# autonomousvision/LaRa

Measured on AMD Instinct MI355X. Metric: novel-view frames/sec @512x512 (4-view in, 2DGS fwd+bwd), higher is better.
Workload: dtype f32 raster + bf16-MFMA/f32-accumulate encoder (+ bf16-autocast coarse decoder MLP, as the reference's bf16-mixed)

## Files before the change

### include/lara2dgs.h

```cpp
#ifndef LARA2DGS_H
#define LARA2DGS_H

#include <stddef.h>
#include <stdint.h>

#ifdef __cplusplus
extern "C" {
#endif

#define LARA2DGS_ABI_VERSION 10

#define LARA2DGS_OK 0
#define LARA2DGS_E_INVALID (-1)
#define LARA2DGS_E_LAUNCH (-2)
#define LARA2DGS_E_UNSUPPORTED (-3)

typedef struct lara2dgs_view {
    int32_t P;
    int32_t sh_degree;
    int32_t sh_coeffs;
    int32_t image_height;
    int32_t image_width;
    float tanfovx;
    float tanfovy;
    float scale_modifier;
    int32_t prefiltered;
    int32_t debug;
    int32_t forward_only;
    int64_t capacity;
    const float *bg;
    const float *viewmatrix;
    const float *projmatrix;
    const float *campos;
    uint32_t *counts_out;
} lara2dgs_view;

typedef struct lara2dgs_state_layout {
    int64_t header;
    int64_t geom;
    int64_t cullbox;
    int64_t point_list;
    int64_t ranges;
    int64_t tile_order;
    int64_t pair_base;
    int64_t pair_pos;
    int64_t final_T;
    int64_t n_contrib;
    int64_t seg_base;
    int64_t seg_cnt;
    int64_t bwd_order;
    int64_t bwd_items;
    int64_t ckpt;
    int64_t pair_mask;
    int64_t tile_maxc;
    int64_t seg_cost;
    int64_t total;
} lara2dgs_state_layout;

int lara2dgs_abi_version(void);
const char *lara2dgs_error_string(int code);
int lara2dgs_last_hip_error(void);

int64_t lara2dgs_state_bytes(int32_t P, int32_t H, int32_t W, int64_t capacity, int32_t forward_only);
int64_t lara2dgs_scratch_bytes(int32_t P, int32_t H, int32_t W, int64_t capacity, int32_t forward_only);
int lara2dgs_get_state_layout(int32_t P, int32_t H, int32_t W, int64_t capacity, int32_t forward_only,
                              lara2dgs_state_layout *out);

int lara2dgs_forward(const lara2dgs_view *view, const float *means3D, const float *shs,
                     const float *colors_precomp, const float *opacities, const float *scales,
                     const float *rotations, const float *transmat_precomp, float *out_color,
                     float *out_allmap, int32_t *out_radii, void *state, void *scratch,
                     void *stream);

int lara2dgs_backward(const lara2dgs_view *view, const float *means3D, const float *shs,
                      const float *colors_precomp, const float *scales, const float *rotations,
                      const float *transmat_precomp, const int32_t *radii, const float *dL_dcolor,
                      const float *dL_dallmap, void *state, void *scratch,
                      float *dL_dmeans3D, float *dL_dmeans2D, float *dL_dshs, float *dL_dcolors,
                      float *dL_dopacities, float *dL_dscales, float *dL_drotations,
                      float *dL_dtransmat, void *stream);


int lara2dgs_forward_views(int32_t n_views, const lara2dgs_view *views, const float *means3D,
                           const float *shs, const float *colors_precomp, const float *opacities,
                           const float *scales, const float *rotations, const float *transmat_precomp,
                           float *out_color, float *out_allmap, int32_t *out_radii, void *state,
                           int64_t state_stride, void *scratch, int64_t scratch_stride, void *stream);

typedef struct lara2dgs_subset {
    const void *coarse_state;
    int64_t coarse_state_stride;
    int64_t coarse_capacity;
    int32_t coarse_P;
    int32_t coarse_forward_only;
    const int32_t *inv;
} lara2dgs_subset;
int lara2dgs_forward_views_subset(int32_t n_views, const lara2dgs_view *views, const float *means3D,
                                  const float *shs, const float *colors_precomp, const float *opacities,
                                  const float *scales, const float *rotations, const float *transmat_precomp,
                                  float *out_color, float *out_allmap, int32_t *out_radii, void *state,
                                  int64_t state_stride, void *scratch, int64_t scratch_stride,
                                  const lara2dgs_subset *subset, void *stream);

typedef struct lara2dgs_grad_layout {
    int64_t means3D, means2D, shs, colors, opacities, scales, rotations, transmat, total;
} lara2dgs_grad_layout;
int lara2dgs_get_grad_layout(int32_t P, int32_t sh_coeffs, int32_t has_shs, int32_t has_colors,
                             int32_t has_scale_rot, int32_t has_transmat, lara2dgs_grad_layout *out);

int lara2dgs_backward_views(int32_t n_views, const lara2dgs_view *views, const float *means3D,
                            const float *shs, const float *colors_precomp, const float *scales,
                            const float *rotations, const float *transmat_precomp, const int32_t *radii,
                            const float *dL_dcolor, const float *dL_dallmap, void *state,
                            int64_t state_stride, void *scratch, int64_t scratch_stride,
                            float *grad_out, void *stream);

int lara2dgs_mark_visible(int32_t P, const float *means3D, const float *viewmatrix,
                          const float *projmatrix, uint8_t *present, void *stream);

int lara2dgs_profile_enable(int on);
int lara2dgs_selftest(int which, const float *in, float *out, void *stream);
int lara2dgs_profile_collect(char *names, int names_len, float *ms, int max_entries);

#ifdef __cplusplus
}
#endif
#endif
```

### lara_amd/csrc/abi.hip

```cpp
#include <stdlib.h>
#include <string.h>

#include "common.h"

static thread_local int g_last_hip_error = 0;
void l2d_set_hip_error(hipError_t e) { g_last_hip_error = (int)e; }

#include <atomic>
#include <mutex>
#include <map>
#include <utility>
#include <vector>
namespace {
struct ProfRec { const char *name; hipEvent_t a, b; };
std::atomic<bool> g_prof_on{false};
std::mutex g_prof_mu;
std::vector<ProfRec> g_prof_log;
std::vector<hipEvent_t> g_prof_pool;
hipEvent_t prof_event() {
    if (!g_prof_pool.empty()) { hipEvent_t e = g_prof_pool.back(); g_prof_pool.pop_back(); return e; }
    hipEvent_t e = nullptr;
    (void)hipEventCreate(&e);
    return e;
}
}

L2dProfScope::L2dProfScope(const char *name, hipStream_t stream) : slot(-1), s(stream) {
    if (!g_prof_on.load(std::memory_order_relaxed)) return;
    std::lock_guard<std::mutex> lk(g_prof_mu);
    ProfRec r{name, prof_event(), prof_event()};
    (void)hipEventRecord(r.a, s);
    g_prof_log.push_back(r);
    slot = (int)g_prof_log.size() - 1;
}
L2dProfScope::~L2dProfScope() {
    if (slot < 0) return;
    std::lock_guard<std::mutex> lk(g_prof_mu);
    if (slot < (int)g_prof_log.size()) (void)hipEventRecord(g_prof_log[slot].b, s);
}

namespace {

bool make_view(const lara2dgs_view *view, ViewDev &v) {
    if (!view) return false;
    if (view->P < 0 || view->image_height <= 0 || view->image_width <= 0) return false;
    if (view->sh_degree < 0 || view->sh_degree > 3) return false;
    if (view->capacity < 0 || view->capacity > 0xffffffffll) return false;
    if (!view->bg || !view->viewmatrix || !view->projmatrix || !view->campos) return false;
    v.P = view->P;
    v.deg = view->sh_degree;
    v.M = view->sh_coeffs;
    v.H = view->image_height;
    v.W = view->image_width;
    v.gx = (v.W + TILE - 1) / TILE;
    v.gy = (v.H + TILE - 1) / TILE;
    v.tiles = v.gx * v.gy;
    if (v.gx > 65535 || v.gy > 65535) return false;
    v.scale_modifier = view->scale_modifier;
    v.cull_transparent = (view->prefiltered >> 1) & 1;
    v.cap = (unsigned)view->capacity;
    v.fwd_only = view->forward_only != 0;
    v.counts_out = view->counts_out;
    {
        static const unsigned dbg = getenv("LARA2DGS_DEBUG_FLAGS") ? (unsigned)strtoul(getenv("LARA2DGS_DEBUG_FLAGS"), nullptr, 0) : 0u;
        v.dbg = dbg;
    }
    v.bg = view->bg;
    v.viewmatrix = view->viewmatrix;
    v.projmatrix = view->projmatrix;
    v.campos = view->campos;
    return true;
}

StateView carve_state(const ViewDev &v, void *state) {
    lara2dgs_state_layout L;
    state_layout(v.P, v.H, v.W, v.cap, v.fwd_only, &L);
    char *b = (char *)state;
    StateView s;
    s.header = (uint32_t *)(b + L.header);
    s.geom = (float4 *)(b + L.geom);
    s.cullbox = (float4 *)(b + L.cullbox);
    s.point_list = (uint32_t *)(b + L.point_list);
    s.ranges = (uint2 *)(b + L.ranges);
    s.tile_order = (uint32_t *)(b + L.tile_order);
    s.pair_base = (uint32_t *)(b + L.pair_base);
    s.pair_pos = (uint32_t *)(b + L.pair_pos);
    s.final_T = (float *)(b + L.final_T);
    s.n_contrib = (uint32_t *)(b + L.n_contrib);
    s.seg_base = (uint32_t *)(b + L.seg_base);
    s.seg_cnt = (uint32_t *)(b + L.seg_cnt);
    s.bwd_order = (uint32_t *)(b + L.bwd_order);
    s.bwd_items = (uint2 *)(b + L.bwd_items);
    s.ckpt = (float *)(b + L.ckpt);
    s.pair_mask = (uint2 *)(b + L.pair_mask);
    s.tile_maxc = (uint32_t *)(b + L.tile_maxc);
    s.seg_cost = (uint32_t *)(b + L.seg_cost);
    return s;
}

ScratchView carve_scratch(const ViewDev &v, void *scratch, ScratchLayout &L) {
    scratch_layout(v.P, v.H, v.W, v.cap, v.fwd_only, &L);
    char *b = (char *)scratch;
    ScratchView s;
    s.tile_count = (uint32_t *)(b + L.tile_count);
    s.tile_fill = (uint32_t *)(b + L.tile_fill);
    s.sub_start = (uint32_t *)(b + L.sub_start);
    s.sort_parts = (uint32_t *)(b + L.sort_parts);
    s.sort_items = (uint2 *)(b + L.sort_items);
    s.rect = (uint4 *)(b + L.rect);
    s.keys = (uint64_t *)(b + L.keys);
    s.block_tot = (uint32_t *)(b + L.block_tot);
    s.pair_grad = (float4 *)(b + L.pair_grad);
    s.pair_valid = (uint32_t *)(b + L.pair_valid);
    return s;
}

}

extern "C" {

int lara2dgs_abi_version(void) { return LARA2DGS_ABI_VERSION; }

const char *lara2dgs_error_string(int code) {
    switch (code) {
    case LARA2DGS_OK: return "ok";
    case LARA2DGS_E_INVALID: return "invalid argument";
    case LARA2DGS_E_LAUNCH: return "HIP launch/API failure (see lara2dgs_last_hip_error)";
    case LARA2DGS_E_UNSUPPORTED: return "unsupported configuration";
    default: return "unknown error";
    }
}

int lara2dgs_last_hip_error(void) { return g_last_hip_error; }

int64_t lara2dgs_state_bytes(int32_t P, int32_t H, int32_t W, int64_t capacity, int32_t forward_only) {
    if (P < 0 || H <= 0 || W <= 0 || capacity < 0) return LARA2DGS_E_INVALID;
    lara2dgs_state_layout L;
    state_layout(P, H, W, capacity, forward_only != 0, &L);
    return L.total;
}

int64_t lara2dgs_scratch_bytes(int32_t P, int32_t H, int32_t W, int64_t capacity, int32_t forward_only) {
    if (P < 0 || H <= 0 || W <= 0 || capacity < 0) return LARA2DGS_E_INVALID;
    ScratchLayout L;
    scratch_layout(P, H, W, capacity, forward_only != 0, &L);
    return L.total;
}

int lara2dgs_get_state_layout(int32_t P, int32_t H, int32_t W, int64_t capacity, int32_t forward_only,
                              lara2dgs_state_layout *out) {
    if (!out || P < 0 || H <= 0 || W <= 0 || capacity < 0) return LARA2DGS_E_INVALID;
    state_layout(P, H, W, capacity, forward_only != 0, out);
    return LARA2DGS_OK;
}

int lara2dgs_mark_visible(int32_t P, const float *means3D, const float *viewmatrix,
                          const float *projmatrix, uint8_t *present, void *stream) {
    (void)projmatrix;
    if (P < 0 || (P > 0 && (!means3D || !viewmatrix || !present))) return LARA2DGS_E_INVALID;
    return launch_mark_visible(P, means3D, viewmatrix, present, (hipStream_t)stream);
}

int lara2dgs_selftest(int which, const float *in, float *out, void *stream) {
    if (which != 0 || !in || !out) return LARA2DGS_E_INVALID;
    return launch_selftest_butterfly(in, out, (hipStream_t)stream);
}

int lara2dgs_profile_enable(int on) {
    g_prof_on.store(on != 0);
    return LARA2DGS_OK;
}

int lara2dgs_profile_collect(char *names, int names_len, float *ms, int max_entries) {
    std::lock_guard<std::mutex> lk(g_prof_mu);
    int n = 0, pos = 0;
    for (size_t i = 0; i < g_prof_log.size(); i++) {
        ProfRec &r = g_prof_log[i];
        if (n < max_entries && names && ms) {
            const int len = (int)strlen(r.name) + 1;
            if (pos + len <= names_len) {
                float t = 0.f;
                (void)hipEventSynchronize(r.b);
                (void)hipEventElapsedTime(&t, r.a, r.b);
                memcpy(names + pos, r.name, len);
                pos += len;
                ms[n++] = t;
            }
        }
        g_prof_pool.push_back(r.a);
        g_prof_pool.push_back(r.b);
    }
    g_prof_log.clear();
    return n;
}

}

namespace {

bool views_agree(int n, const lara2dgs_view *views) {
    for (int i = 1; i < n; i++) {
        const lara2dgs_view &a = views[0], &b = views[i];
        if (a.P != b.P || a.sh_degree != b.sh_degree || a.sh_coeffs != b.sh_coeffs || a.image_height != b.image_height ||
            a.image_width != b.image_width || a.capacity != b.capacity || a.prefiltered != b.prefiltered ||
            a.scale_modifier != b.scale_modifier || a.debug != b.debug || a.forward_only != b.forward_only) return false;
        if (b.counts_out != (a.counts_out ? a.counts_out + 4 * i : nullptr)) return false;
    }
    return true;
}

void grad_layout(int64_t P, int M, bool sh, bool col, bool sr, bool tm, lara2dgs_grad_layout *L) {
    int64_t o = 0;
    auto sec = [&](bool on, int64_t n) { if (!on) return (int64_t)-1; const int64_t at = o; o = (o + n + 3) / 4 * 4; return at; };
    L->means3D = sec(true, P * 3);
    L->means2D = sec(true, P * 3);
    L->shs = sec(sh, P * M * 3);
    L->colors = sec(col, P * 3);
    L->opacities = sec(true, P);
    L->scales = sec(sr, P * 2);
    L->rotations = sec(sr, P * 4);
    L->transmat = sec(tm, P * 9);
    L->total = o;
}

__global__ void __launch_bounds__(256) zero_strided_kernel(char *__restrict__ base, const int64_t stride, const int64_t bytes) {
    uint4 *p = (uint4 *)(base + (int64_t)blockIdx.y * stride);
    const int64_t n = bytes / 16;
    for (int64_t i = (int64_t)blockIdx.x * 256 + threadIdx.x; i < n; i += (int64_t)gridDim.x * 256) p[i] = make_uint4(0u, 0u, 0u, 0u);
}

inline void zero_strided(void *base, int64_t stride, int64_t bytes, int n_views, hipStream_t s) {
    const int64_t n = (bytes + 15) / 16;
    const unsigned gx = (unsigned)(n < 256 * 64 ? (n + 255) / 256 : 64);
    hipLaunchKernelGGL(zero_strided_kernel, dim3(gx ? gx : 1, (unsigned)n_views), dim3(256), 0, s, (char *)base, stride, (bytes + 15) / 16 * 16);
}

bool strides_ok(const lara2dgs_view &v0, int64_t state_stride, int64_t scratch_stride) {
    return state_stride % 256 == 0 && scratch_stride % 256 == 0 &&
           state_stride >= lara2dgs_state_bytes(v0.P, v0.image_height, v0.image_width, v0.capacity, v0.forward_only) &&
           scratch_stride >= lara2dgs_scratch_bytes(v0.P, v0.image_height, v0.image_width, v0.capacity, v0.forward_only);
}

void one_view_strides(const lara2dgs_view &v, int64_t &state_stride, int64_t &scratch_stride) {
    state_stride = align_up(lara2dgs_state_bytes(v.P, v.image_height, v.image_width, v.capacity, v.forward_only), 256);
    scratch_stride = align_up(lara2dgs_scratch_bytes(v.P, v.image_height, v.image_width, v.capacity, v.forward_only), 256);
}
}

extern "C" {

int lara2dgs_get_grad_layout(int32_t P, int32_t sh_coeffs, int32_t has_shs, int32_t has_colors,
                             int32_t has_scale_rot, int32_t has_transmat, lara2dgs_grad_layout *out) {
    if (!out || P < 0 || sh_coeffs < 0) return LARA2DGS_E_INVALID;
    grad_layout(P, sh_coeffs, has_shs != 0, has_colors != 0, has_scale_rot != 0, has_transmat != 0, out);
    return LARA2DGS_OK;
}

static int forward_views_impl(int32_t n_views, const lara2dgs_view *views, const float *means3D,
                           const float *shs, const float *colors_precomp, const float *opacities,
                           const float *scales, const float *rotations, const float *transmat_precomp,
                           float *out_color, float *out_allmap, int32_t *out_radii, void *state,
                           int64_t state_stride, void *scratch, int64_t scratch_stride, void *stream,
                           const lara2dgs_subset *subset) {
    if (n_views <= 0 || !views || !state || !scratch) return LARA2DGS_E_INVALID;
    if (subset) {
        if (!subset->coarse_state || !subset->inv || subset->coarse_P < views[0].P || subset->coarse_capacity < 0 ||
            subset->coarse_capacity > 0xffffffffll || subset->coarse_state_stride % 256) return LARA2DGS_E_INVALID;
        if (!views[0].forward_only && subset->coarse_forward_only) return LARA2DGS_E_INVALID;
        if (subset->coarse_state_stride < lara2dgs_state_bytes(subset->coarse_P, views[0].image_height, views[0].image_width,
                                                                subset->coarse_capacity, subset->coarse_forward_only)) return LARA2DGS_E_INVALID;
    }
    if (!views_agree(n_views, views)) return LARA2DGS_E_INVALID;
    const lara2dgs_view &v0 = views[0];
    if (!strides_ok(v0, state_stride, scratch_stride)) return LARA2DGS_E_INVALID;
    hipStream_t caller = (hipStream_t)stream;
    const int64_t HW = (int64_t)v0.image_height * v0.image_width;
    if (!out_color || !out_allmap) return LARA2DGS_E_INVALID;
    if (v0.P > 0) {
        if (!means3D || !opacities || !out_radii) return LARA2DGS_E_INVALID;
        if ((shs == nullptr) == (colors_precomp == nullptr)) return LARA2DGS_E_INVALID;
        if ((scales && rotations) == (transmat_precomp != nullptr)) return LARA2DGS_E_INVALID;
    }
    std::vector<ViewDev> vd(n_views);
    std::vector<StateView> st(n_views);
    std::vector<ScratchView> sc(n_views);
    std::vector<int32_t *> rad(n_views);
    for (int i = 0; i < n_views; i++) {
        if (!make_view(&views[i], vd[i])) return LARA2DGS_E_INVALID;
        if (v0.P > 0 && shs && vd[i].M < (vd[i].deg + 1) * (vd[i].deg + 1)) return LARA2DGS_E_INVALID;
        st[i] = carve_state(vd[i], (char *)state + i * state_stride);
        ScratchLayout SL;
        sc[i] = carve_scratch(vd[i], (char *)scratch + i * scratch_stride, SL);
        rad[i] = out_radii + (int64_t)i * v0.P;
        if (i == 0)
            zero_strided(sc[0].tile_count, scratch_stride, SL.sub_start - SL.tile_count, n_views, caller);
    }
    int rc = LARA2DGS_OK;
    for (int i0 = 0; i0 < n_views && rc == LARA2DGS_OK; i0 += L2D_MAX_VIEWS) {
        ViewBatch vb{};
        vb.n = n_views - i0 < L2D_MAX_VIEWS ? n_views - i0 : L2D_MAX_VIEWS;
        vb.state_stride = state_stride; vb.scratch_stride = scratch_stride;
        for (int k = 0; k < vb.n; k++) vb.bg[k] = vd[i0 + k].bg;
        rc = launch_preprocess_fwd_views(vd[i0], vb.n, &vd[i0], n_views > 1, means3D, shs, colors_precomp, opacities, scales,
                                         rotations, transmat_precomp, &st[i0], &sc[i0], &rad[i0], caller);
        if (rc == LARA2DGS_OK && !subset) rc = launch_binning(vd[i0], st[i0], sc[i0], caller, vb);
        if (rc == LARA2DGS_OK && subset) {
            ViewDev cv = vd[i0];
            cv.P = subset->coarse_P; cv.cap = (unsigned)subset->coarse_capacity; cv.fwd_only = subset->coarse_forward_only != 0;
            const StateView cst = carve_state(cv, (char *)const_cast<void *>(subset->coarse_state) + (int64_t)i0 * subset->coarse_state_stride);
            rc = launch_binning_subset(vd[i0], st[i0], sc[i0], caller, vb, cst, subset->coarse_state_stride, subset->inv);
        }
        if (rc == LARA2DGS_OK)
            rc = launch_composite_fwd(vd[i0], st[i0], sc[i0], out_color + (int64_t)i0 * 3 * HW, out_allmap + (int64_t)i0 * 7 * HW,
                                      caller, vb);
    }
    return rc;
}

int lara2dgs_forward_views(int32_t n_views, const lara2dgs_view *views, const float *means3D,
                           const float *shs, const float *colors_precomp, const float *opacities,
                           const float *scales, const float *rotations, const float *transmat_precomp,
                           float *out_color, float *out_allmap, int32_t *out_radii, void *state,
                           int64_t state_stride, void *scratch, int64_t scratch_stride, void *stream) {
    return forward_views_impl(n_views, views, means3D, shs, colors_precomp, opacities, scales, rotations, transmat_precomp, out_color,
                              out_allmap, out_radii, state, state_stride, scratch, scratch_stride, stream, nullptr);
}

int lara2dgs_forward_views_subset(int32_t n_views, const lara2dgs_view *views, const float *means3D,
                                  const float *shs, const float *colors_precomp, const float *opacities,
                                  const float *scales, const float *rotations, const float *transmat_precomp,
                                  float *out_color, float *out_allmap, int32_t *out_radii, void *state,
                                  int64_t state_stride, void *scratch, int64_t scratch_stride,
                                  const lara2dgs_subset *subset, void *stream) {
    if (!subset) return LARA2DGS_E_INVALID;
    return forward_views_impl(n_views, views, means3D, shs, colors_precomp, opacities, scales, rotations, transmat_precomp, out_color,
                              out_allmap, out_radii, state, state_stride, scratch, scratch_stride, stream, subset);
}

static int backward_views_impl(int32_t n_views, const lara2dgs_view *views, const float *means3D, const float *shs,
                               const float *colors_precomp, const float *scales, const float *rotations,
                               const float *transmat_precomp, const int32_t *radii, const float *dL_dcolor,
                               const float *dL_dallmap, void *state, int64_t state_stride, void *scratch,
                               int64_t scratch_stride, float *dL_dmeans3D, float *dL_dmeans2D, float *dL_dshs,
                               float *dL_dcolors, float *dL_dopacities, float *dL_dscales, float *dL_drotations,
                               float *dL_dtransmat, void *stream) {
    const lara2dgs_view &v0 = views[0];
    hipStream_t caller = (hipStream_t)stream;
    const int64_t HW = (int64_t)v0.image_height * v0.image_width;
    std::vector<ViewDev> vd(n_views);
    std::vector<StateView> st(n_views);
    std::vector<ScratchView> sc(n_views);
    std::vector<const int32_t *> rad(n_views);
    std::vector<ScratchLayout> SL(n_views);
    for (int i = 0; i < n_views; i++) {
        if (!make_view(&views[i], vd[i])) return LARA2DGS_E_INVALID;
        st[i] = carve_state(vd[i], (char *)state + i * state_stride);
        sc[i] = carve_scratch(vd[i], (char *)scratch + i * scratch_stride, SL[i]);
        rad[i] = radii + (int64_t)i * v0.P;
    }
    int rc = LARA2DGS_OK;
    for (int i0 = 0; i0 < n_views && rc == LARA2DGS_OK; i0 += L2D_MAX_VIEWS) {
        ViewBatch vb{};
        vb.n = n_views - i0 < L2D_MAX_VIEWS ? n_views - i0 : L2D_MAX_VIEWS;
        vb.state_stride = state_stride; vb.scratch_stride = scratch_stride;
        for (int k = 0; k < vb.n; k++) vb.bg[k] = vd[i0 + k].bg;
        rc = launch_bwd_order(vd[i0], st[i0], sc[i0], caller, vb, sc[i0].pair_valid, SL[i0].total - SL[i0].pair_valid);
        if (rc == LARA2DGS_OK)
            rc = launch_composite_bwd(vd[i0], st[i0], sc[i0], dL_dcolor + (int64_t)i0 * 3 * HW, dL_dallmap ? dL_dallmap + (int64_t)i0 * 7 * HW : nullptr, caller, vb);
        if (rc == LARA2DGS_OK)
            rc = launch_preprocess_bwd_views(vd[i0], vb.n, &vd[i0], n_views > 1, i0 > 0, means3D, shs, colors_precomp, scales,
                                             rotations, transmat_precomp, &rad[i0], &st[i0], &sc[i0], dL_dmeans3D, dL_dmeans2D,
                                             dL_dshs, dL_dcolors, dL_dopacities, dL_dscales, dL_drotations, dL_dtransmat, caller);
    }
    return rc;
}

int lara2dgs_backward_views(int32_t n_views, const lara2dgs_view *views, const float *means3D,
                            const float *shs, const float *colors_precomp, const float *scales,
                            const float *rotations, const float *transmat_precomp, const int32_t *radii,
                            const float *dL_dcolor, const float *dL_dallmap, void *state,
                            int64_t state_stride, void *scratch, int64_t scratch_stride,
                            float *grad_out, void *stream) {
    if (n_views <= 0 || !views || !state || !scratch || !grad_out) return LARA2DGS_E_INVALID;
    if (!views_agree(n_views, views)) return LARA2DGS_E_INVALID;
    const lara2dgs_view &v0 = views[0];
    if (v0.forward_only) return LARA2DGS_E_INVALID;
    if (!strides_ok(v0, state_stride, scratch_stride)) return LARA2DGS_E_INVALID;
    if (!dL_dcolor) return LARA2DGS_E_INVALID;
    const bool has_sh = shs != nullptr, has_col = colors_precomp != nullptr, has_sr = scales && rotations,
               has_tm = transmat_precomp != nullptr;
    lara2dgs_grad_layout G;
    grad_layout(v0.P, v0.sh_coeffs, has_sh, has_col, has_sr, has_tm, &G);
    if (v0.P == 0 || G.total == 0) return LARA2DGS_OK;
    if (!means3D || !radii) return LARA2DGS_E_INVALID;
    if (has_sh == has_col || has_sr == has_tm) return LARA2DGS_E_INVALID;
    auto at = [&](int64_t off) { return off < 0 ? (float *)nullptr : grad_out + off; };
    return backward_views_impl(n_views, views, means3D, shs, colors_precomp, scales, rotations, transmat_precomp, radii,
                               dL_dcolor, dL_dallmap, state, state_stride, scratch, scratch_stride, at(G.means3D),
                               at(G.means2D), at(G.shs), at(G.colors), at(G.opacities), at(G.scales), at(G.rotations),
                               at(G.transmat), stream);
}

int lara2dgs_forward(const lara2dgs_view *view, const float *means3D, const float *shs,
                     const float *colors_precomp, const float *opacities, const float *scales,
                     const float *rotations, const float *transmat_precomp, float *out_color,
                     float *out_allmap, int32_t *out_radii, void *state, void *scratch,
                     void *stream) {
    ViewDev v;
    if (!make_view(view, v)) return LARA2DGS_E_INVALID;
    if (!out_color || !out_allmap || !state || !scratch) return LARA2DGS_E_INVALID;
    if (v.P > 0) {
        if (!means3D || !opacities || !out_radii) return LARA2DGS_E_INVALID;
        if ((shs == nullptr) == (colors_precomp == nullptr)) return LARA2DGS_E_INVALID;
        const bool has_sr = scales && rotations;
        if (has_sr == (transmat_precomp != nullptr)) return LARA2DGS_E_INVALID;
        if (shs && v.M < (v.deg + 1) * (v.deg + 1)) return LARA2DGS_E_INVALID;
    }
    int64_t sst, qst;
    one_view_strides(*view, sst, qst);
    return forward_views_impl(1, view, means3D, shs, colors_precomp, opacities, scales, rotations, transmat_precomp, out_color,
                              out_allmap, out_radii, state, sst, scratch, qst, stream, nullptr);
}

int lara2dgs_backward(const lara2dgs_view *view, const float *means3D, const float *shs,
                      const float *colors_precomp, const float *scales, const float *rotations,
                      const float *transmat_precomp, const int32_t *radii, const float *dL_dcolor,
                      const float *dL_dallmap, void *state, void *scratch,
                      float *dL_dmeans3D, float *dL_dmeans2D, float *dL_dshs, float *dL_dcolors,
                      float *dL_dopacities, float *dL_dscales, float *dL_drotations,
                      float *dL_dtransmat, void *stream) {
    ViewDev v;
    if (!make_view(view, v)) return LARA2DGS_E_INVALID;
    if (!dL_dcolor || !state || !scratch) return LARA2DGS_E_INVALID;
    if (v.fwd_only) return LARA2DGS_E_INVALID;
    if (v.P == 0) return LARA2DGS_OK;
    if (!means3D || !radii || !dL_dmeans3D || !dL_dmeans2D || !dL_dopacities) return LARA2DGS_E_INVALID;
    if ((shs == nullptr) == (colors_precomp == nullptr)) return LARA2DGS_E_INVALID;
    if (shs && !dL_dshs) return LARA2DGS_E_INVALID;
    if (colors_precomp && !dL_dcolors) return LARA2DGS_E_INVALID;
    const bool has_sr = scales && rotations;
    if (has_sr == (transmat_precomp != nullptr)) return LARA2DGS_E_INVALID;
    if (has_sr && (!dL_dscales || !dL_drotations)) return LARA2DGS_E_INVALID;
    if (transmat_precomp && !dL_dtransmat) return LARA2DGS_E_INVALID;
    int64_t sst, qst;
    one_view_strides(*view, sst, qst);
    return backward_views_impl(1, view, means3D, shs, colors_precomp, scales, rotations, transmat_precomp, radii, dL_dcolor,
                               dL_dallmap, state, sst, scratch, qst, dL_dmeans3D, dL_dmeans2D, dL_dshs, dL_dcolors,
                               dL_dopacities, dL_dscales, dL_drotations, dL_dtransmat, stream);
}

}
```

### lara_amd/csrc/binning.hip

```cpp
#include "common.h"

namespace {

template <typename Ptr>
__device__ __forceinline__ void bitonic_sort(Ptr a, const uint32_t n, const uint32_t m ) {
    for (uint32_t k = 2; k <= m; k <<= 1) {
        for (uint32_t j = k >> 1; j > 0; j >>= 1) {
            const bool flip = (j == (k >> 1));
            for (uint32_t t = threadIdx.x; t < (m >> 1); t += blockDim.x) {
                const uint32_t i = ((t & ~(j - 1)) << 1) | (t & (j - 1));
                const uint32_t p = flip ? (i ^ (k - 1)) : (i ^ j);
                if (p < n) {
                    const uint64_t x = a[i], y = a[p];
                    if (y < x) { a[i] = y; a[p] = x; }
                }
            }
            __syncthreads();
        }
    }
}

constexpr int L2D_SORT_PARTS = 2;
__device__ __forceinline__ uint32_t l2d_sort_parts(const uint32_t len) {
    return len <= 4096u || len > 8192u ? 1u : 2u;
}

__global__ void __launch_bounds__(1024)
tile_scan_kernel(ViewDev v, const uint32_t *__restrict__ tile_count, uint32_t *__restrict__ sub_start,
                 uint2 *__restrict__ ranges, uint32_t *__restrict__ header,
                 uint32_t *__restrict__ tile_order, uint32_t *__restrict__ block_tot,
                 uint32_t *__restrict__ seg_base, uint32_t *__restrict__ seg_cnt,
                 uint32_t *__restrict__ bwd_order, uint2 *__restrict__ bwd_items,
                 uint32_t *__restrict__ sort_parts, uint2 *__restrict__ sort_items, const long long sst, const long long qst) {
    tile_count = l2d_view_ptr(tile_count, qst); sub_start = l2d_view_ptr(sub_start, qst); block_tot = l2d_view_ptr(block_tot, qst);
    sort_parts = l2d_view_ptr(sort_parts, qst); sort_items = l2d_view_ptr(sort_items, qst);
    ranges = l2d_view_ptr(ranges, sst); header = l2d_view_ptr(header, sst); tile_order = l2d_view_ptr(tile_order, sst);
    seg_base = l2d_view_ptr(seg_base, sst); seg_cnt = l2d_view_ptr(seg_cnt, sst); bwd_order = l2d_view_ptr(bwd_order, sst);
    bwd_items = l2d_view_ptr(bwd_items, sst);
    __shared__ uint32_t wave_sums[16];
    __shared__ uint32_t carry_s, s_max;
    __shared__ uint32_t bcnt[64];
    const int tid = threadIdx.x, lane = tid & 63, wid = tid >> 6;
    if (blockIdx.x == 1) {
        if (tid == 0) carry_s = 0;
        __syncthreads();
        const int nblk = (v.P + 255) / 256;
        for (int base = 0; base < nblk; base += 1024) {
            const int i = base + tid;
            const uint32_t c = i < nblk ? block_tot[i] : 0u;
            uint32_t x = c;
#pragma unroll
            for (int d = 1; d < 64; d <<= 1) {
                const uint32_t y = __shfl_up(x, d, 64);
                if (lane >= d) x += y;
            }
            if (lane == 63) wave_sums[wid] = x;
            __syncthreads();
            uint32_t wave_off = 0;
            for (int w = 0; w < wid; w++) wave_off += wave_sums[w];
            const uint32_t incl = carry_s + wave_off + x;
            if (i < nblk) block_tot[i] = incl - c;
            __syncthreads();
            if (tid == 1023) carry_s = incl;
            __syncthreads();
        }
        return;
    }
    if (tid == 0) carry_s = 0;
    if (tid >= 4 && tid < 64) header[tid] = 0u;
    __syncthreads();
    uint32_t max_len = 0;
    for (int base = 0; base < v.tiles; base += 1024) {
        const int i = base + tid;
        uint32_t sub[L2D_SLICES];
        uint32_t c = 0;
        if (i < v.tiles) {
            const uint4 *tc = (const uint4 *)(tile_count + (size_t)i * L2D_SLICES);
#pragma unroll
            for (int q = 0; q < L2D_SLICES / 4; q++) {
                const uint4 w4 = tc[q];
                sub[4 * q] = w4.x; sub[4 * q + 1] = w4.y; sub[4 * q + 2] = w4.z; sub[4 * q + 3] = w4.w;
            }
#pragma unroll
            for (int q = 0; q < L2D_SLICES; q++) c += sub[q];
        }
        max_len = c > max_len ? c : max_len;
        uint32_t x = c;
#pragma unroll
        for (int d = 1; d < 64; d <<= 1) {
            const uint32_t y = __shfl_up(x, d, 64);
            if (lane >= d) x += y;
        }
        if (lane == 63) wave_sums[wid] = x;
        __syncthreads();
        uint32_t wave_off = 0;
        for (int w = 0; w < wid; w++) wave_off += wave_sums[w];
        const uint32_t carry = carry_s;
        const uint32_t incl = carry + wave_off + x;
        if (i < v.tiles) {
            ranges[i] = c ? make_uint2(incl - c, incl) : make_uint2(0u, 0u);
            uint32_t run = incl - c;
            uint4 *ss = (uint4 *)(sub_start + (size_t)i * L2D_SLICES);
#pragma unroll
            for (int q = 0; q < L2D_SLICES / 4; q++) {
                uint4 w4;
                w4.x = run; run += sub[4 * q];
                w4.y = run; run += sub[4 * q + 1];
                w4.z = run; run += sub[4 * q + 2];
                w4.w = run; run += sub[4 * q + 3];
                ss[q] = w4;
            }
        }
        __syncthreads();
        if (tid == 1023) carry_s = incl;
        __syncthreads();
    }
#pragma unroll
    for (int d = 32; d > 0; d >>= 1) {
        const uint32_t y = __shfl_xor(max_len, d, 64);
        max_len = y > max_len ? y : max_len;
    }
    __syncthreads();
    if (lane == 0) wave_sums[wid] = max_len;
    __syncthreads();
    if (tid == 0) {
        uint32_t m = 0;
        for (int w = 0; w < 16; w++) m = wave_sums[w] > m ? wave_sums[w] : m;
        const uint32_t total = carry_s;
        header[0] = total;
        header[1] = total > v.cap ? 1u : 0u;
        header[2] = m;
        s_max = m;
        if (v.counts_out) {
            uint32_t *c = v.counts_out + 4 * blockIdx.z;
            __hip_atomic_store(&c[0], total, __ATOMIC_RELAXED, __HIP_MEMORY_SCOPE_SYSTEM);
            __hip_atomic_store(&c[1], total > v.cap ? 1u : 0u, __ATOMIC_RELAXED, __HIP_MEMORY_SCOPE_SYSTEM);
            __hip_atomic_store(&c[2], m, __ATOMIC_RELAXED, __HIP_MEMORY_SCOPE_SYSTEM);
            __hip_atomic_store(&c[3], 1u, __ATOMIC_RELEASE, __HIP_MEMORY_SCOPE_SYSTEM);
        }
    }
    if (tid < 64) bcnt[tid] = 0;
    __syncthreads();
    const uint32_t denom = s_max + 1u;
    for (int i = tid; i < v.tiles; i += 1024) {
        const uint2 rg = ranges[i];
        const uint32_t b = 63u - (uint32_t)(((uint64_t)(rg.y - rg.x) * 64u) / denom);
        atomicAdd(&bcnt[b], 1u);
    }
    __syncthreads();
    if (tid < 64) {
        const uint32_t c = bcnt[tid];
        uint32_t x = c;
#pragma unroll
        for (int d = 1; d < 64; d <<= 1) {
            const uint32_t y = __shfl_up(x, d, 64);
            if (lane >= d) x += y;
        }
        bcnt[tid] = x - c;
    }
    __syncthreads();
    for (int i = tid; i < v.tiles; i += 1024) {
        const uint2 rg = ranges[i];
        const uint32_t b = 63u - (uint32_t)(((uint64_t)(rg.y - rg.x) * 64u) / denom);
        tile_order[atomicAdd(&bcnt[b], 1u)] = (uint32_t)i;
    }
    __syncthreads();
    if (!v.fwd_only) {
    if (tid == 0) carry_s = 0;
    if (tid < 64) bcnt[tid] = 0;
    __syncthreads();
    const bool overflow = header[1] != 0u;
    for (int base = 0; base < v.tiles; base += 1024) {
        const int i = base + tid;
        uint32_t len = 0;
        if (i < v.tiles) { const uint2 rg = ranges[i]; len = rg.y - rg.x; }
        const uint32_t nb = len ? (len - 1u) / L2D_SEG : 0u;
        uint32_t x = nb;
#pragma unroll
        for (int d = 1; d < 64; d <<= 1) {
            const uint32_t y = __shfl_up(x, d, 64);
            if (lane >= d) x += y;
        }
        if (lane == 63) wave_sums[wid] = x;
        __syncthreads();
        uint32_t wave_off = 0;
        for (int w = 0; w < wid; w++) wave_off += wave_sums[w];
        const uint32_t incl = carry_s + wave_off + x;
        if (i < v.tiles) {
            seg_base[i] = incl - nb;
            seg_cnt[i] = nb;
            if (!overflow)
                for (uint32_t q = 0; q < nb; q++) bwd_items[incl - nb + q] = make_uint2((uint32_t)i, q);
            const uint32_t pl = len - nb * L2D_SEG;
            atomicAdd(&bcnt[63u - (uint32_t)(((uint64_t)min(pl, (uint32_t)L2D_SEG) * 64u) / (L2D_SEG + 1u))], 1u);
        }
        __syncthreads();
        if (tid == 1023) carry_s = incl;
        __syncthreads();
    }
    if (tid == 0) { seg_base[v.tiles] = carry_s; header[3] = carry_s; }
    if (tid < 64) {
        const uint32_t c = bcnt[tid];
        uint32_t x = c;
#pragma unroll
        for (int d = 1; d < 64; d <<= 1) {
            const uint32_t y = __shfl_up(x, d, 64);
            if (lane >= d) x += y;
        }
        bcnt[tid] = x - c;
    }
    __syncthreads();
    for (int i = tid; i < v.tiles; i += 1024) {
        const uint2 rg = ranges[i];
        const uint32_t len = rg.y - rg.x;
        const uint32_t pl = len - seg_cnt[i] * L2D_SEG;
        bwd_order[atomicAdd(&bcnt[63u - (uint32_t)(((uint64_t)min(pl, (uint32_t)L2D_SEG) * 64u) / (L2D_SEG + 1u))], 1u)] = (uint32_t)i;
    }
    }
    __syncthreads();
    if (tid == 0) carry_s = 0;
    __syncthreads();
    for (int base = 0; base < v.tiles; base += 1024) {
        const int i = base + tid;
        uint32_t len = 0;
        if (i < v.tiles) { const uint2 rg = ranges[i]; len = rg.y - rg.x; }
        const uint32_t want = l2d_sort_parts(len) - 1u;
        uint32_t x = want;
#pragma unroll
        for (int d = 1; d < 64; d <<= 1) {
            const uint32_t y = __shfl_up(x, d, 64);
            if (lane >= d) x += y;
        }
        if (lane == 63) wave_sums[wid] = x;
        __syncthreads();
        uint32_t wave_off = 0;
        for (int w = 0; w < wid; w++) wave_off += wave_sums[w];
        const uint32_t incl = carry_s + wave_off + x, first = incl - want;
        if (i < v.tiles) {
            const uint32_t room = first < (uint32_t)v.tiles ? (uint32_t)v.tiles - first : 0u;
            const uint32_t got = want < room ? want : room;
            sort_parts[i] = 1u + got;
            for (uint32_t q = 0; q < got; q++) sort_items[first + q] = make_uint2((uint32_t)i, q + 1u);
        }
        __syncthreads();
        if (tid == 1023) carry_s = incl;
        __syncthreads();
    }
    if (tid == 0) sort_parts[v.tiles] = carry_s < (uint32_t)v.tiles ? carry_s : (uint32_t)v.tiles;
}

__global__ void __launch_bounds__(256)
scatter_kernel(ViewDev v, const uint4 *__restrict__ rect, const uint32_t *__restrict__ sub_start,
               const uint32_t *__restrict__ block_base, uint32_t *__restrict__ pair_base,
               uint32_t *__restrict__ tile_fill, uint64_t *__restrict__ keys, const int use_lds, const long long sst,
               const long long qst) {
    rect = l2d_view_ptr(rect, qst); sub_start = l2d_view_ptr(sub_start, qst); block_base = l2d_view_ptr(block_base, qst);
    tile_fill = l2d_view_ptr(tile_fill, qst); keys = l2d_view_ptr(keys, qst); pair_base = l2d_view_ptr(pair_base, sst);
    extern __shared__ __attribute__((aligned(16))) uint32_t hist[];
    const int idx = blockIdx.x * blockDim.x + threadIdx.x;
    const int slice = blockIdx.x % L2D_SLICES;
    int rx0 = 0, ry0 = 0, rx1 = 0, ry1 = 0;
    uint64_t word = 0;
    if (idx < v.P) {
        const uint4 r = rect[idx];
        rx0 = r.x & 0xffff; ry0 = r.x >> 16; rx1 = r.y & 0xffff; ry1 = r.y >> 16;
        word = ((uint64_t)r.z << 32) | (uint32_t)idx;
        if (!v.fwd_only) {
            const uint32_t pb = block_base[blockIdx.x] + r.w;
            pair_base[idx] = pb;
            if (idx == v.P - 1) pair_base[v.P] = pb + (uint32_t)(rx1 - rx0) * (uint32_t)(ry1 - ry0);
        }
    }
    if (use_lds) {
        for (int t = threadIdx.x; t < v.tiles; t += blockDim.x) hist[t] = 0;
        __syncthreads();
        for (int y = ry0; y < ry1; y++)
            for (int x = rx0; x < rx1; x++) atomicAdd(&hist[y * v.gx + x], 1u);
        __syncthreads();
        for (int t = threadIdx.x; t < v.tiles; t += blockDim.x) {
            const uint32_t c = hist[t];
            if (c) hist[t] = sub_start[t * L2D_SLICES + slice] +
                             __hip_atomic_fetch_add(&tile_fill[t * L2D_SLICES + slice], c, __ATOMIC_RELAXED,
                                                    __HIP_MEMORY_SCOPE_AGENT);
        }
        __syncthreads();
        for (int y = ry0; y < ry1; y++)
            for (int x = rx0; x < rx1; x++) {
                const uint32_t slot = atomicAdd(&hist[y * v.gx + x], 1u);
                if (slot < v.cap) keys[slot] = word;
            }
    } else {
        for (int y = ry0; y < ry1; y++)
            for (int x = rx0; x < rx1; x++) {
                const int t = (y * v.gx + x) * L2D_SLICES + slice;
                const uint32_t slot = sub_start[t] + __hip_atomic_fetch_add(&tile_fill[t], 1u, __ATOMIC_RELAXED,
                                                                          __HIP_MEMORY_SCOPE_AGENT);
                if (slot < v.cap) keys[slot] = word;
            }
    }
}

__device__ __forceinline__ uint32_t next_pow2(uint32_t n) {
    return n <= 1 ? 1u : 1u << (32 - __clz(n - 1));
}

__device__ __forceinline__ void ce(uint64_t &a, uint64_t &b) {
    const bool sw = b < a;
    const uint64_t lo = sw ? b : a, hi = sw ? a : b;
    a = lo; b = hi;
}
__device__ __forceinline__ uint64_t shfl64(uint64_t x, int src_lane) {
    const uint32_t lo = __shfl((uint32_t)x, src_lane, 64), hi = __shfl((uint32_t)(x >> 32), src_lane, 64);
    return ((uint64_t)hi << 32) | lo;
}

template <int E, int NT, bool REVERSED>
__device__ __forceinline__ void xchg(uint64_t (&x)[E], const int t, const int pt, uint64_t *lds) {
    uint64_t o[E];
    if ((t ^ pt) < 64) {
#pragma unroll
        for (int e = 0; e < E; e++) o[e] = shfl64(x[REVERSED ? E - 1 - e : e], pt & 63);
    } else {
#pragma unroll
        for (int e = 0; e < E; e++) lds[e * NT + t] = x[e];
        __syncthreads();
#pragma unroll
        for (int e = 0; e < E; e++) o[e] = lds[(REVERSED ? E - 1 - e : e) * NT + pt];
        __syncthreads();
    }
    const bool keep_min = t < pt;
#pragma unroll
    for (int e = 0; e < E; e++) {
        const bool take = keep_min ? (o[e] < x[e]) : (x[e] < o[e]);
        x[e] = take ? o[e] : x[e];
    }
}

template <int E, int NT>
__device__ __forceinline__ void block_sort(uint64_t (&x)[E], uint64_t *lds) {
    const int t = threadIdx.x;
#pragma unroll
    for (int k = 2; k <= E; k <<= 1) {
#pragma unroll
        for (int e = 0; e < E; e++) {
            const int p = e ^ (k - 1);
            if (p > e) ce(x[e], x[p]);
        }
#pragma unroll
        for (int j = k >> 2; j >= 1; j >>= 1)
#pragma unroll
            for (int e = 0; e < E; e++)
                if ((e & j) == 0) ce(x[e], x[e | j]);
    }
#pragma unroll 1
    for (int kt = 2; kt <= NT; kt <<= 1) {
        xchg<E, NT, true>(x, t, t ^ (kt - 1), lds);
#pragma unroll 1
        for (int jt = kt >> 2; jt >= 1; jt >>= 1) xchg<E, NT, false>(x, t, t ^ jt, lds);
#pragma unroll
        for (int j = E >> 1; j >= 1; j >>= 1)
#pragma unroll
            for (int e = 0; e < E; e++)
                if ((e & j) == 0) ce(x[e], x[e | j]);
    }
}

struct PairMap {
    const uint4 *rect;
    const uint32_t *pair_base;
    uint32_t *pair_pos;
    int tx, ty;
    uint32_t first;
    __device__ __forceinline__ void put(const uint32_t id, const uint32_t i) const {
        if (!pair_pos) return;
        const uint4 r = rect[id];
        const int rx0 = r.x & 0xffff, ry0 = r.x >> 16, rx1 = r.y & 0xffff;
        pair_pos[first + i] = pair_base[id] + (uint32_t)((ty - ry0) * (rx1 - rx0) + (tx - rx0));
    }
};

template <int E, int NT>
__device__ __forceinline__ void sort_tile(const uint64_t *__restrict__ seg, const uint32_t n,
                                          uint32_t *__restrict__ out, uint64_t *lds, const PairMap &pm) {
    uint64_t x[E];
    const uint32_t i0 = threadIdx.x * E;
#pragma unroll
    for (int e = 0; e < E; e++) x[e] = (i0 + e < n) ? seg[i0 + e] : ~0ull;
    block_sort<E, NT>(x, lds);
#pragma unroll
    for (int e = 0; e < E; e++)
        if (i0 + e < n) {
            out[i0 + e] = (uint32_t)x[e];
            pm.put((uint32_t)x[e], i0 + e);
        }
}

constexpr uint32_t L2D_SORT_LDS_KEYS = 4096;

constexpr int L2D_SORT_BUCKETS = 1024, L2D_SORT_BUCKET_MAX = 48;

template <int E>
__device__ __forceinline__ void sort_keys(const uint64_t *src, const uint32_t m, uint32_t *__restrict__ out,
                                          const uint32_t off, uint64_t *lds, uint32_t *bkt, uint32_t *sh, const PairMap &pm) {
    const int t = threadIdx.x, lane = t & 63;
    uint64_t x[E];
#pragma unroll
    for (int e = 0; e < E; e++) x[e] = (t + e * 512 < (int)m) ? src[t + e * 512] : ~0ull;
    if (t == 0) { sh[0] = ~0u; sh[1] = 0u; sh[2] = 0u; }
    const uint32_t B = m <= 256u ? 64u : (m <= 1024u ? 256u : (uint32_t)L2D_SORT_BUCKETS);
    for (uint32_t b = t; b < B; b += 512) bkt[b] = 0u;
    __syncthreads();
    uint32_t lo = ~0u, hi = 0u;
#pragma unroll
    for (int e = 0; e < E; e++)
        if (t + e * 512 < (int)m) {
            const uint32_t d = (uint32_t)(x[e] >> 32);
            lo = d < lo ? d : lo;
            hi = d > hi ? d : hi;
        }
#pragma unroll
    for (int k = 32; k > 0; k >>= 1) {
        const uint32_t a = __shfl_xor(lo, k, 64), b = __shfl_xor(hi, k, 64);
        lo = a < lo ? a : lo;
        hi = b > hi ? b : hi;
    }
    if (lane == 0) { atomicMin(&sh[0], lo); atomicMax(&sh[1], hi); }
    __syncthreads();
    const uint32_t dmin = sh[0];
    const uint64_t scale = ((uint64_t)B << 32) / ((uint64_t)(sh[1] - dmin) + 1ull);
    uint32_t bk[E], slot[E];
#pragma unroll
    for (int e = 0; e < E; e++) {
        bk[e] = 0u; slot[e] = 0u;
        if (t + e * 512 < (int)m) {
            const uint64_t q = (uint64_t)((uint32_t)(x[e] >> 32) - dmin) * scale;
            bk[e] = (uint32_t)(q >> 32);
            bk[e] = bk[e] < B ? bk[e] : B - 1u;
            slot[e] = atomicAdd(&bkt[bk[e]], 1u);
        }
    }
    __syncthreads();
    {
        const uint32_t c0 = 2 * t < (int)B ? bkt[2 * t] : 0u, c1 = 2 * t + 1 < (int)B ? bkt[2 * t + 1] : 0u;
        uint32_t incl = c0 + c1, big = c0 > c1 ? c0 : c1;
#pragma unroll
        for (int d = 1; d < 64; d <<= 1) {
            const uint32_t y = __shfl_up(incl, d, 64);
            if (lane >= d) incl += y;
        }
#pragma unroll
        for (int k = 32; k > 0; k >>= 1) { const uint32_t y = __shfl_xor(big, k, 64); big = y > big ? y : big; }
        if (lane == 63) sh[4 + (t >> 6)] = incl;
        if (lane == 0) atomicMax(&sh[2], big);
        __syncthreads();
        uint32_t wave_off = 0;
        for (int w = 0; w < (t >> 6); w++) wave_off += sh[4 + w];
        __syncthreads();
        if (2 * t < (int)B) bkt[2 * t] = wave_off + incl - c0 - c1;
        if (2 * t + 1 < (int)B) bkt[2 * t + 1] = wave_off + incl - c1;
        if (t == 511) bkt[B] = wave_off + incl;
    }
    __syncthreads();
    if (sh[2] > (uint32_t)L2D_SORT_BUCKET_MAX) {
        __syncthreads();
        block_sort<E, 512>(x, lds);
#pragma unroll
        for (int e = 0; e < E; e++)
            if ((uint32_t)(t * E + e) < m) {
                out[off + t * E + e] = (uint32_t)x[e];
                pm.put((uint32_t)x[e], off + t * E + e);
            }
        return;
    }
#pragma unroll
    for (int e = 0; e < E; e++)
        if (t + e * 512 < (int)m) lds[bkt[bk[e]] + slot[e]] = x[e];
    __syncthreads();
    for (uint32_t b = t; b < B; b += 512) {
        const uint32_t s0 = bkt[b], s1 = bkt[b + 1];
        for (uint32_t i = s0 + 1; i < s1; i++) {
            const uint64_t key = lds[i];
            uint32_t j = i;
            while (j > s0 && lds[j - 1] > key) { lds[j] = lds[j - 1]; j--; }
            lds[j] = key;
        }
    }
    __syncthreads();
    for (uint32_t i = t; i < m; i += 512) {
        const uint32_t id = (uint32_t)lds[i];
        out[off + i] = id;
        pm.put(id, off + i);
    }
}

template <int DUMMY = 0>
__device__ __forceinline__ void sort_dispatch(const uint64_t *src, const uint32_t m, uint32_t *__restrict__ out,
                                              const uint32_t off, uint64_t *lds, uint32_t *bkt, uint32_t *sh, const PairMap &pm) {
    if (m <= 512u) sort_keys<1>(src, m, out, off, lds, bkt, sh, pm);
    else if (m <= 1024u) sort_keys<2>(src, m, out, off, lds, bkt, sh, pm);
    else if (m <= 2048u) sort_keys<4>(src, m, out, off, lds, bkt, sh, pm);
    else sort_keys<8>(src, m, out, off, lds, bkt, sh, pm);
}

__global__ void __launch_bounds__(512)
tile_sort_kernel(ViewDev v, const uint2 *__restrict__ ranges, const uint32_t *__restrict__ header,
                 const uint32_t *__restrict__ tile_order, uint64_t *__restrict__ keys,
                 uint32_t *__restrict__ point_list, const uint4 *__restrict__ rect,
                 const uint32_t *__restrict__ pair_base, uint32_t *__restrict__ pair_pos,
                 uint32_t *__restrict__ sort_parts, const uint2 *__restrict__ sort_items, const long long sst, const long long qst) {
    ranges = l2d_view_ptr(ranges, sst); header = l2d_view_ptr(header, sst); tile_order = l2d_view_ptr(tile_order, sst);
    point_list = l2d_view_ptr(point_list, sst); pair_base = l2d_view_ptr(pair_base, sst); pair_pos = l2d_view_ptr(pair_pos, sst);
    keys = l2d_view_ptr(keys, qst); rect = l2d_view_ptr(rect, qst); sort_parts = l2d_view_ptr(sort_parts, qst);
    sort_items = l2d_view_ptr(sort_items, qst);
    __shared__ uint64_t lds[L2D_SORT_LDS_KEYS];
    __shared__ uint32_t bkt[L2D_SORT_BUCKETS + 1], sh[16];
    __shared__ uint32_t s_min, s_max, s_mine, s_ticket, s_hist[L2D_SORT_PARTS];
    int part = 0, tile;
    if ((int)blockIdx.x < v.tiles) {
        if (blockIdx.x >= sort_parts[v.tiles]) return;
        const uint2 it = sort_items[blockIdx.x];
        tile = (int)it.x; part = (int)it.y;
    } else {
        tile = (int)tile_order[(int)blockIdx.x - v.tiles];
    }
    const uint2 rg = ranges[tile];
    const uint32_t n = rg.y - rg.x;
    if (header[1]) return;
    if (n == 0) return;
    const int S = (int)(sort_parts[tile] & 0xffffu);
    uint64_t *seg = keys + rg.x;
    uint32_t *out = point_list + rg.x;
    const PairMap pm{rect, pair_base, v.fwd_only ? nullptr : pair_pos, tile % v.gx, tile / v.gx, rg.x};
    bool whole_list_in_place = S == 1 && n > L2D_SORT_LDS_KEYS;
    if (S == 1 && !whole_list_in_place) {
        sort_dispatch(seg, n, out, 0u, lds, bkt, sh, pm);
        return;
    }
    if (S > 1) {
        if (threadIdx.x == 0) { s_min = ~0u; s_max = 0u; s_mine = 0u; }
        if (threadIdx.x < L2D_SORT_PARTS) s_hist[threadIdx.x] = 0u;
        __syncthreads();
        uint32_t lo = ~0u, hi = 0u;
        for (uint32_t i = threadIdx.x; i < n; i += 512) {
            const uint32_t d = (uint32_t)(seg[i] >> 32);
            lo = d < lo ? d : lo;
            hi = d > hi ? d : hi;
        }
#pragma unroll
        for (int k = 32; k > 0; k >>= 1) {
            const uint32_t a = __shfl_xor(lo, k, 64), b = __shfl_xor(hi, k, 64);
            lo = a < lo ? a : lo;
            hi = b > hi ? b : hi;
        }
        if ((threadIdx.x & 63) == 0) { atomicMin(&s_min, lo); atomicMax(&s_max, hi); }
        __syncthreads();
        const uint32_t dmin = s_min;
        const uint64_t width = (uint64_t)(s_max - dmin) + 1ull;
        uint32_t cnt[L2D_SORT_PARTS];
#pragma unroll
        for (int b = 0; b < L2D_SORT_PARTS; b++) cnt[b] = 0u;
        for (uint32_t i = threadIdx.x; i < n; i += 512) {
            const int bin = (int)(((uint64_t)((uint32_t)(seg[i] >> 32) - dmin) * (uint64_t)S) / width);
#pragma unroll
            for (int b = 0; b < L2D_SORT_PARTS; b++) cnt[b] += bin == b ? 1u : 0u;
        }
#pragma unroll
        for (int b = 0; b < L2D_SORT_PARTS; b++) {
#pragma unroll
            for (int k = 32; k > 0; k >>= 1) cnt[b] += __shfl_xor(cnt[b], k, 64);
            if ((threadIdx.x & 63) == 0 && cnt[b]) atomicAdd(&s_hist[b], cnt[b]);
        }
        __syncthreads();
        uint32_t off = 0, biggest = 0;
        for (int b = 0; b < S; b++) {
            off += b < part ? s_hist[b] : 0u;
            biggest = s_hist[b] > biggest ? s_hist[b] : biggest;
        }
        if (biggest > L2D_SORT_LDS_KEYS) {
            if (threadIdx.x == 0) {
                __threadfence();
                s_ticket = __hip_atomic_fetch_add(&sort_parts[tile], 0x10000u, __ATOMIC_ACQ_REL, __HIP_MEMORY_SCOPE_AGENT) >> 16;
            }
            __syncthreads();
            if (s_ticket != (uint32_t)S - 1u) return;
            whole_list_in_place = true;
        } else {
            const uint32_t m = s_hist[part];
            if (m == 0) return;
            for (uint32_t i0 = 0; i0 < n; i0 += 512) {
                const uint32_t i = i0 + threadIdx.x;
                const uint64_t key = i < n ? seg[i] : 0ull;
                const int bin = i < n ? (int)(((uint64_t)((uint32_t)(key >> 32) - dmin) * (uint64_t)S) / width) : -1;
                const unsigned long long mine = __ballot(bin == part);
                uint32_t base = 0;
                if ((threadIdx.x & 63) == 0 && mine) base = atomicAdd(&s_mine, (uint32_t)__builtin_popcountll(mine));
                base = (uint32_t)__builtin_amdgcn_readfirstlane((int)base);
                if (bin == part) lds[base + (uint32_t)__builtin_popcountll(mine & ((1ull << (threadIdx.x & 63)) - 1ull))] = key;
            }
            __syncthreads();
            sort_dispatch(lds, m, out, off, lds, bkt, sh, pm);
            return;
        }
    }
    bitonic_sort(seg, n, next_pow2(n));
    for (uint32_t i = threadIdx.x; i < n; i += blockDim.x) {
        out[i] = (uint32_t)seg[i];
        pm.put((uint32_t)seg[i], i);
    }
}

__global__ void __launch_bounds__(256)
pair_base_kernel(ViewDev v, const uint4 *__restrict__ rect, const uint32_t *__restrict__ block_base, uint32_t *__restrict__ pair_base,
                 const long long sst, const long long qst) {
    rect = l2d_view_ptr(rect, qst); block_base = l2d_view_ptr(block_base, qst); pair_base = l2d_view_ptr(pair_base, sst);
    const int idx = blockIdx.x * 256 + threadIdx.x;
    if (idx >= v.P) return;
    const uint4 r = rect[idx];
    const uint32_t pb = block_base[blockIdx.x] + r.w;
    pair_base[idx] = pb;
    if (idx == v.P - 1) {
        const int rx0 = r.x & 0xffff, ry0 = r.x >> 16, rx1 = r.y & 0xffff, ry1 = r.y >> 16;
        pair_base[v.P] = pb + (uint32_t)(rx1 - rx0) * (uint32_t)(ry1 - ry0);
    }
}

__global__ void __launch_bounds__(256)
subset_compact_kernel(ViewDev v, const uint32_t *__restrict__ header, const uint2 *__restrict__ ranges, uint32_t *__restrict__ point_list,
                      const uint32_t *__restrict__ pair_base, uint32_t *__restrict__ pair_pos, const long long sst,
                      const uint2 *__restrict__ c_ranges, const uint32_t *__restrict__ c_point_list, const uint32_t *__restrict__ c_pair_base,
                      const uint32_t *__restrict__ c_pair_pos, const long long csst, const int32_t *__restrict__ inv) {
    header = l2d_view_ptr(header, sst); ranges = l2d_view_ptr(ranges, sst); point_list = l2d_view_ptr(point_list, sst);
    pair_base = l2d_view_ptr(pair_base, sst); pair_pos = l2d_view_ptr(pair_pos, sst);
    c_ranges = l2d_view_ptr(c_ranges, csst); c_point_list = l2d_view_ptr(c_point_list, csst);
    c_pair_base = l2d_view_ptr(c_pair_base, csst); c_pair_pos = l2d_view_ptr(c_pair_pos, csst);
    __shared__ uint32_t wtot[2][4];
    if (header[1]) return;
    const int tile = blockIdx.x, tid = threadIdx.x, lane = tid & 63, wave = tid >> 6;
    const uint2 cr = c_ranges[tile];
    const uint32_t n = cr.y - cr.x;
    uint32_t out = ranges[tile].x;
    uint32_t id_n = tid < n ? c_point_list[cr.x + tid] : 0u;
    int fid_n = tid < n ? inv[id_n] : -1;
    int buf = 0;
    for (uint32_t base = 0; base < n; base += 256, buf ^= 1) {
        const uint32_t i = base + tid, id = id_n;
        const int fid = fid_n;
        uint32_t off = 0, pbf = 0;
        if (fid >= 0 && !v.fwd_only) { off = c_pair_pos[cr.x + i] - c_pair_base[id]; pbf = pair_base[fid]; }
        if (base + 256 < n) {
            id_n = i + 256 < n ? c_point_list[cr.x + i + 256] : 0u;
            fid_n = i + 256 < n ? inv[id_n] : -1;
        }
        const unsigned long long kept = __ballot(fid >= 0);
        if (lane == 0) wtot[buf][wave] = (uint32_t)__builtin_popcountll(kept);
        __syncthreads();
        uint32_t before = 0, all = 0;
#pragma unroll
        for (int w = 0; w < 4; w++) { before += w < wave ? wtot[buf][w] : 0u; all += wtot[buf][w]; }
        if (fid >= 0) {
            const uint32_t pos = out + before + (uint32_t)__builtin_popcountll(kept & ((1ull << lane) - 1ull));
            point_list[pos] = (uint32_t)fid;
            if (!v.fwd_only) pair_pos[pos] = pbf + off;
        }
        out += all;
    }
}

}

int launch_binning_subset(const ViewDev &v, StateView st, ScratchView sc, hipStream_t s, const ViewBatch &vb, StateView cst,
                          long long coarse_stride, const int32_t *inv) {
    const unsigned nz = (unsigned)vb.n;
    const long long sst = vb.state_stride, qst = vb.scratch_stride;
    {
        L2D_PROF("tile_scan", s);
        hipLaunchKernelGGL(tile_scan_kernel, dim3(v.P > 0 ? 2 : 1, 1, nz), dim3(1024), 0, s, v, sc.tile_count, sc.sub_start,
                           st.ranges, st.header, st.tile_order, sc.block_tot, st.seg_base, st.seg_cnt, st.bwd_order,
                           st.bwd_items, sc.sort_parts, sc.sort_items, sst, qst);
    }
    L2D_CHECK_LAUNCH();
    if (v.P == 0) return LARA2DGS_OK;
    if (!v.fwd_only) {
        L2D_PROF("subset_pair_base", s);
        hipLaunchKernelGGL(pair_base_kernel, dim3((v.P + 255) / 256, 1, nz), dim3(256), 0, s, v, sc.rect, sc.block_tot, st.pair_base, sst, qst);
    }
    {
        L2D_PROF("subset_compact", s);
        hipLaunchKernelGGL(subset_compact_kernel, dim3(v.tiles, 1, nz), dim3(256), 0, s, v, st.header, st.ranges, st.point_list,
                           st.pair_base, st.pair_pos, sst, cst.ranges, cst.point_list, cst.pair_base, cst.pair_pos, coarse_stride, inv);
    }
    L2D_CHECK_LAUNCH();
    return LARA2DGS_OK;
}

int launch_binning(const ViewDev &v, StateView st, ScratchView sc, hipStream_t s, const ViewBatch &vb) {
    const unsigned nz = (unsigned)vb.n;
    const long long sst = vb.state_stride, qst = vb.scratch_stride;
    {
        L2D_PROF("tile_scan", s);
        hipLaunchKernelGGL(tile_scan_kernel, dim3(v.P > 0 ? 2 : 1, 1, nz), dim3(1024), 0, s, v, sc.tile_count, sc.sub_start,
                           st.ranges, st.header, st.tile_order, sc.block_tot, st.seg_base, st.seg_cnt, st.bwd_order,
                           st.bwd_items, sc.sort_parts, sc.sort_items, sst, qst);
    }
    L2D_CHECK_LAUNCH();
    if (v.P == 0) return LARA2DGS_OK;
    {
        L2D_PROF("scatter", s);
        const int use_lds = v.tiles <= L2D_LDS_HIST_TILES;
        hipLaunchKernelGGL(scatter_kernel, dim3((v.P + 255) / 256, 1, nz), dim3(256),
                           use_lds ? (size_t)v.tiles * 4 : 0, s, v, sc.rect, sc.sub_start, sc.block_tot,
                           st.pair_base, sc.tile_fill, sc.keys, use_lds, sst, qst);
    }
    L2D_CHECK_LAUNCH();
    {
        L2D_PROF("tile_sort", s);
        hipLaunchKernelGGL(tile_sort_kernel, dim3(v.tiles * 2, 1, nz), dim3(512), 0, s, v, st.ranges, st.header, st.tile_order,
                           sc.keys, st.point_list, sc.rect, st.pair_base, st.pair_pos, sc.sort_parts, sc.sort_items, sst, qst);
    }
    L2D_CHECK_LAUNCH();
    return LARA2DGS_OK;
}
```

### lara_amd/csrc/common.h

```cpp
#pragma once
#include <hip/hip_runtime.h>
#include <stdint.h>

#include "../../include/lara2dgs.h"

#define TILE 16
#define NEAR_N 0.2f
#define FAR_N 100.0f
#define FILTER_SIZE 0.707106f
#define FILTER_INV_SQUARE 2.0f
#define CUTOFF 3.0f
#define GEOM_F 20
#define L2D_SLICES 16
#define L2D_LDS_HIST_TILES 8192
#define GRAD_F 20
#ifndef L2D_SEG
#define L2D_SEG 512
#endif
#define L2D_CKPT_F 10
#define L2D_MAX_VIEWS 8

struct ViewDev {
    int P, deg, M, H, W, gx, gy, tiles;
    float scale_modifier;
    unsigned cap;
    unsigned dbg;
    int cull_transparent;
    int fwd_only;
    const float *bg, *viewmatrix, *projmatrix, *campos;
    uint32_t *counts_out;
};

struct ViewBatch {
    int n;
    long long state_stride, scratch_stride;
    const float *bg[L2D_MAX_VIEWS];
};
#ifdef __HIPCC__
template <class T>
__device__ __forceinline__ T *l2d_view_ptr(T *p, const long long stride_bytes) {
    return (T *)((const char *)p + (long long)blockIdx.z * stride_bytes);
}
#endif

struct StateView {
    uint32_t *header;
    float4 *geom;
    float4 *cullbox;
    uint32_t *point_list;
    uint2 *ranges;
    uint32_t *tile_order;
    uint32_t *pair_base;
    uint32_t *pair_pos;
    float *final_T;
    uint32_t *n_contrib;
    uint32_t *seg_base;
    uint32_t *seg_cnt;
    uint32_t *bwd_order;
    uint2 *bwd_items;
    float *ckpt;
    uint2 *pair_mask;
    uint32_t *tile_maxc;
    uint32_t *seg_cost;
};

struct ScratchView {
    uint32_t *tile_count;
    uint32_t *tile_fill;
    uint32_t *sub_start;
    uint32_t *sort_parts;
    uint2 *sort_items;
    uint4 *rect;
    uint64_t *keys;
    uint32_t *block_tot;
    float4 *pair_grad;
    uint32_t *pair_valid;
};

static inline int64_t align_up(int64_t x, int64_t a) { return (x + a - 1) / a * a; }

__host__ __device__ static inline int64_t l2d_ckpt_slots(int64_t cap) { return cap / L2D_SEG + 1; }

static inline void state_layout(int P, int H, int W, int64_t cap, int fwd_only, lara2dgs_state_layout *L) {
    const int64_t tiles = (int64_t)((W + TILE - 1) / TILE) * ((H + TILE - 1) / TILE);
    const int64_t HW = (int64_t)H * W;
    const int64_t k = fwd_only ? 0 : 1;
    int64_t o = 0;
    L->header = o;      o = align_up(o + 256, 256);
    L->geom = o;        o = align_up(o + (int64_t)P * GEOM_F * 4, 256);
    L->cullbox = o;     o = align_up(o + (int64_t)P * 16, 256);
    L->point_list = o;  o = align_up(o + cap * 4, 256);
    L->ranges = o;      o = align_up(o + tiles * 8, 256);
    L->tile_order = o;  o = align_up(o + tiles * 4, 256);
    L->pair_base = o;   o = align_up(o + k * ((int64_t)P + 1) * 4, 256);
    L->pair_pos = o;    o = align_up(o + k * cap * 4, 256);
    L->final_T = o;     o = align_up(o + k * L2D_CKPT_F * HW * 4, 256);
    L->n_contrib = o;   o = align_up(o + k * 2 * HW * 4, 256);
    const int64_t nseg = cap / L2D_SEG + 1;
    L->seg_base = o;    o = align_up(o + k * (tiles + 1) * 4, 256);
    L->seg_cnt = o;     o = align_up(o + k * tiles * 4, 256);
    L->bwd_order = o;   o = align_up(o + k * tiles * 4, 256);
    L->bwd_items = o;   o = align_up(o + k * (nseg + tiles) * 8, 256);
    L->ckpt = o;        o = align_up(o + k * l2d_ckpt_slots(cap) * L2D_CKPT_F * 256 * 4, 256);
    L->pair_mask = o;   o = align_up(o + k * cap * 8, 256);
    L->tile_maxc = o;   o = align_up(o + k * tiles * 4, 256);
    L->seg_cost = o;    o = align_up(o + k * (nseg + tiles) * 4, 256);
    L->total = o;
}

struct ScratchLayout { int64_t tile_count, tile_fill, sub_start, sort_parts, sort_items, rect, keys, block_tot, pair_grad, pair_valid, total; };
static inline void scratch_layout(int P, int H, int W, int64_t cap, int fwd_only, ScratchLayout *L) {
    const int64_t tiles = (int64_t)((W + TILE - 1) / TILE) * ((H + TILE - 1) / TILE);
    int64_t o = 0;
    L->tile_count = o;  o = align_up(o + tiles * 4 * L2D_SLICES, 256);
    L->tile_fill = o;   o = align_up(o + tiles * 4 * L2D_SLICES, 256);
    L->sub_start = o;   o = align_up(o + tiles * 4 * L2D_SLICES, 256);
    L->sort_parts = o;  o = align_up(o + (tiles + 1) * 4, 256);
    L->sort_items = o;  o = align_up(o + tiles * 8, 256);
    const int64_t fwd0 = o;
    L->rect = o;        o = align_up(o + (int64_t)P * 16, 256);
    L->keys = o;        o = align_up(o + cap * 8, 256);
    L->block_tot = o;   o = align_up(o + (((int64_t)P + 255) / 256 + 1) * 4, 256);
    const int64_t fwd_end = o;
    L->pair_grad = fwd0;
    L->pair_valid = align_up(fwd0 + cap * GRAD_F * 4, 256);
    const int64_t bwd_end = align_up(L->pair_valid + cap + 256, 256);
    L->total = (fwd_only || fwd_end > bwd_end) ? fwd_end : bwd_end;
}

int launch_preprocess_fwd_views(const ViewDev &v, int n, const ViewDev *views, bool multi, const float *means3D, const float *shs,
                                const float *colors_precomp, const float *opacities, const float *scales,
                                const float *rotations, const float *transmat_precomp, const StateView *st,
                                const ScratchView *sc, int32_t *const *radii, hipStream_t s);
int launch_binning(const ViewDev &v, StateView st, ScratchView sc, hipStream_t s, const ViewBatch &vb);
int launch_binning_subset(const ViewDev &v, StateView st, ScratchView sc, hipStream_t s, const ViewBatch &vb, StateView cst,
                          long long coarse_stride, const int32_t *inv);
int launch_composite_fwd(const ViewDev &v, StateView st, ScratchView sc, float *out_color, float *out_allmap,
                         hipStream_t s, const ViewBatch &vb);
int launch_bwd_order(const ViewDev &v, StateView st, ScratchView sc, hipStream_t s, const ViewBatch &vb, void *zero_base, int64_t zero_bytes);
int launch_composite_bwd(const ViewDev &v, StateView st, ScratchView sc, const float *dL_dcolor,
                         const float *dL_dallmap, hipStream_t s, const ViewBatch &vb);
int launch_preprocess_bwd_views(const ViewDev &v, int n, const ViewDev *views, bool multi, int accumulate, const float *means3D,
                                const float *shs, const float *colors_precomp, const float *scales, const float *rotations,
                                const float *transmat_precomp, const int32_t *const *radii, const StateView *st,
                                const ScratchView *sc, float *dL_dmeans3D, float *dL_dmeans2D, float *dL_dshs,
                                float *dL_dcolors, float *dL_dopacities, float *dL_dscales, float *dL_drotations,
                                float *dL_dtransmat, hipStream_t s);
int launch_selftest_butterfly(const float *in, float *out, hipStream_t s);
int launch_mark_visible(int P, const float *means3D, const float *viewmatrix, uint8_t *present,
                        hipStream_t s);

void l2d_set_hip_error(hipError_t e);

struct L2dProfScope {
    int slot;
    hipStream_t s;
    L2dProfScope(const char *name, hipStream_t stream);
    ~L2dProfScope();
};
#define L2D_PROF(name, stream) L2dProfScope prof_scope__(name, stream)
#define L2D_CHECK_LAUNCH()                                  \
    do {                                                    \
        hipError_t e__ = hipGetLastError();                 \
        if (e__ != hipSuccess) {                            \
            l2d_set_hip_error(e__);                         \
            return LARA2DGS_E_LAUNCH;                       \
        }                                                   \
    } while (0)
```

### lara_amd/csrc/composite.hip

```cpp
#include "common.h"

namespace {

constexpr int FWD_CHUNK = 512;
constexpr int REC4 = 6;

__device__ __forceinline__ void cross3(const float a[3], const float b[3], float o[3]) {
    o[0] = a[1] * b[2] - a[2] * b[1];
    o[1] = a[2] * b[0] - a[0] * b[2];
    o[2] = a[0] * b[1] - a[1] * b[0];
}

template <int CHUNK>
__device__ __forceinline__ uint32_t stage_entry(const float4 *__restrict__ geom, const uint32_t id,
                                                const float4 cb, const bool valid, const float X0,
                                                const float Y0, float4 *rec, uint32_t *ids,
                                                const int e = threadIdx.x, uint2 *mask_out = nullptr) {
    float4 r0 = make_float4(0.f, 0.f, 0.f, 0.f), r1 = r0, r2 = r0, r3 = r0, r4 = r0, r5 = r0;
    uint32_t mask_lo = 0, mask_hi = 0, rectpack = 0;
    int gx0 = 0, gx1 = -1, gy0 = 0, gy1 = -1;
    if (valid) {
        gx0 = (int)ceilf(fminf(fmaxf((cb.x - X0 - 1.f) * 0.5f, 0.f), 8.f));
        gx1 = (int)floorf(fminf(fmaxf((cb.y - X0) * 0.5f, -1.f), 7.f));
        gy0 = (int)ceilf(fminf(fmaxf((cb.z - Y0 - 1.f) * 0.5f, 0.f), 8.f));
        gy1 = (int)floorf(fminf(fmaxf((cb.w - Y0) * 0.5f, -1.f), 7.f));
    }
    if (gx0 <= gx1 && gy0 <= gy1) {
        const float4 *g = geom + (size_t)id * 5;
        const float4 g0 = g[0], g1 = g[1], g2 = g[2], g3 = g[3], g4 = g[4];
        const float Tu[3] = {g0.x, g0.y, g0.z}, Tv[3] = {g0.w, g1.x, g1.y}, Tw[3] = {g1.z, g1.w, g2.x};
        const float k0[3] = {X0 * Tw[0] - Tu[0], X0 * Tw[1] - Tu[1], X0 * Tw[2] - Tu[2]};
        const float l0[3] = {Y0 * Tw[0] - Tv[0], Y0 * Tw[1] - Tv[1], Y0 * Tw[2] - Tv[2]};
        float A[3], B[3], C[3];
        cross3(k0, l0, A);
        cross3(Tw, l0, B);
        cross3(k0, Tw, C);
        const float cx = g2.y - X0, cy = g2.z - Y0, opa = g2.w;
        const float tau = 2.0f * __logf(255.0f * opa) * 1.001f + 0.01f;
        const float nb = B[0] * B[0] + B[1] * B[1], qa = nb - tau * B[2] * B[2];
        const bool ellipse = qa > 1e-5f * (nb + tau * B[2] * B[2]);
        const float inv_qa = ellipse ? __builtin_amdgcn_rcpf(qa) : 0.f;
        const float bx0 = (float)(2 * gx0), bx1 = (float)(2 * gx1 + 1);
        uint32_t colsum = 0;
        for (int by = gy0; by <= gy1; by++) {
            float lo = 1e9f, hi = -1e9f;
#pragma unroll
            for (int q = 0; q < 2; q++) {
                const float y = (float)(2 * by + q);
                const float u0 = A[0] + y * C[0], u1 = A[1] + y * C[1], u2 = A[2] + y * C[2];
                const float qb = u0 * B[0] + u1 * B[1] - tau * (u2 * B[2]);
                const float qc = u0 * u0 + u1 * u1 - tau * (u2 * u2);
                const float disc = qb * qb - qa * qc + 4e-6f * (qb * qb);
                if (!ellipse) {
                    lo = bx0; hi = bx1;
                } else if (disc >= 0.f) {
                    const float sq = __builtin_amdgcn_sqrtf(disc);
                    lo = fminf(lo, (-qb - sq) * inv_qa);
                    hi = fmaxf(hi, (-qb + sq) * inv_qa);
                }
                const float h = 0.5f * tau - (y - cy) * (y - cy);
                if (h >= 0.f) {
                    const float sh = __builtin_amdgcn_sqrtf(h);
                    lo = fminf(lo, cx - sh);
                    hi = fmaxf(hi, cx + sh);
                }
            }
            const int ilo = (int)ceilf(fmaxf(lo - 0.02f, bx0)), ihi = (int)floorf(fminf(hi + 0.02f, bx1));
            if (ilo <= ihi) {
                const uint32_t cols = ((2u << (ihi >> 1)) - 1u) & ~((1u << (ilo >> 1)) - 1u);
                colsum |= cols;
                if (by < 4) mask_lo |= cols << (8 * by);
                else mask_hi |= cols << (8 * (by - 4));
            }
        }
        if (colsum) {
            const int rx0 = __builtin_ctz(colsum), rx1 = 31 - __builtin_clz(colsum);
            const int ry0 = mask_lo ? (__builtin_ctz(mask_lo) >> 3) : 4 + (__builtin_ctz(mask_hi) >> 3);
            const int ry1 = mask_hi ? 4 + ((31 - __builtin_clz(mask_hi)) >> 3) : ((31 - __builtin_clz(mask_lo)) >> 3);
            rectpack = (uint32_t)rx0 | ((uint32_t)rx1 << 4) | ((uint32_t)ry0 << 8) | ((uint32_t)ry1 << 12) | (1u << 16);
            r0 = make_float4(A[0], A[1], A[2], B[0]);
            r1 = make_float4(B[1], B[2], C[0], C[1]);
            r2 = make_float4(C[2], cx, cy, Tw[0]);
            r3 = make_float4(Tw[1], Tw[2], opa, __uint_as_float(mask_lo));
            r4 = make_float4(g3.x, g3.y, g3.z, g4.x);
            r5 = make_float4(g4.y, g4.z, __uint_as_float(mask_hi), 0.f);
        }
    }
    rec[0 * CHUNK + e] = r0; rec[1 * CHUNK + e] = r1; rec[2 * CHUNK + e] = r2;
    rec[3 * CHUNK + e] = r3; rec[4 * CHUNK + e] = r4; rec[5 * CHUNK + e] = r5;
    if (ids) ids[e] = valid ? id : 0u;
    if (mask_out && valid) *mask_out = make_uint2(mask_lo, mask_hi);
    return rectpack;
}

template <int CHUNK>
__device__ __forceinline__ void stage_entry_masked(const float4 *__restrict__ geom, const uint32_t id, const uint2 mask,
                                                   const bool valid, const float X0, const float Y0, float4 *rec,
                                                   uint32_t *ids, const int e) {
    float4 r0 = make_float4(0.f, 0.f, 0.f, 0.f), r1 = r0, r2 = r0, r3 = r0, r4 = r0, r5 = r0;
    if (valid && (mask.x | mask.y)) {
        const float4 *g = geom + (size_t)id * 5;
        const float4 g0 = g[0], g1 = g[1], g2 = g[2], g3 = g[3], g4 = g[4];
        const float Tu[3] = {g0.x, g0.y, g0.z}, Tv[3] = {g0.w, g1.x, g1.y}, Tw[3] = {g1.z, g1.w, g2.x};
        const float k0[3] = {X0 * Tw[0] - Tu[0], X0 * Tw[1] - Tu[1], X0 * Tw[2] - Tu[2]};
        const float l0[3] = {Y0 * Tw[0] - Tv[0], Y0 * Tw[1] - Tv[1], Y0 * Tw[2] - Tv[2]};
        float A[3], B[3], C[3];
        cross3(k0, l0, A);
        cross3(Tw, l0, B);
        cross3(k0, Tw, C);
        r0 = make_float4(A[0], A[1], A[2], B[0]);
        r1 = make_float4(B[1], B[2], C[0], C[1]);
        r2 = make_float4(C[2], g2.y - X0, g2.z - Y0, Tw[0]);
        r3 = make_float4(Tw[1], Tw[2], g2.w, __uint_as_float(mask.x));
        r4 = make_float4(g3.x, g3.y, g3.z, g4.x);
        r5 = make_float4(g4.y, g4.z, __uint_as_float(mask.y), 0.f);
    }
    rec[0 * CHUNK + e] = r0; rec[1 * CHUNK + e] = r1; rec[2 * CHUNK + e] = r2;
    rec[3 * CHUNK + e] = r3; rec[4 * CHUNK + e] = r4; rec[5 * CHUNK + e] = r5;
    ids[e] = valid ? id : 0u;
}

struct Hit {
    float sx, sy, rz, depth, G, alpha, ddx, ddy;
    bool use3d;
};

struct EntryRec { float4 r0, r1, r2, r3; };
template <int CHUNK>
__device__ __forceinline__ EntryRec load_entry(const float4 *rec, const int j) {
    EntryRec e;
    e.r0 = rec[0 * CHUNK + j]; e.r1 = rec[1 * CHUNK + j]; e.r2 = rec[2 * CHUNK + j]; e.r3 = rec[3 * CHUNK + j];
    return e;
}

__device__ __forceinline__ bool eval_rec(const EntryRec &e, const float lx, const float ly, Hit &h,
                                         float Tw[3], float &opa) {
    const float4 r0 = e.r0, r1 = e.r1, r2 = e.r2, r3 = e.r3;
    const float px = r0.x + lx * r0.w + ly * r1.z;
    const float py = r0.y + lx * r1.x + ly * r1.w;
    const float pz = r0.z + lx * r1.y + ly * r2.x;
    Tw[0] = r2.w; Tw[1] = r3.x; Tw[2] = r3.y; opa = r3.z;
    h.rz = __builtin_amdgcn_rcpf(pz);
    h.sx = px * h.rz; h.sy = py * h.rz;
    const float rho3d = h.sx * h.sx + h.sy * h.sy;
    h.ddx = r2.y - lx; h.ddy = r2.z - ly;
    const float rho2d = FILTER_INV_SQUARE * (h.ddx * h.ddx + h.ddy * h.ddy);
    h.use3d = rho3d <= rho2d;
    const float rho = fminf(rho3d, rho2d);
    h.depth = h.use3d ? (h.sx * Tw[0] + h.sy * Tw[1]) + Tw[2] : Tw[2];
    const float power = -0.5f * rho;
    h.G = __expf(power);
    h.alpha = fminf(0.99f, opa * h.G);
    return (pz != 0.0f) & (h.depth >= NEAR_N) & !(power > 0.0f) & !(h.alpha < 1.0f / 255.0f);
}

__device__ __forceinline__ unsigned long long quad_masks(const uint32_t bm, const int qx4, const int grp) {
    unsigned long long m = 0ull;
#pragma unroll
    for (int g = 0; g < 16; g++) {
        const int bit = (g >> 2) * 8 + qx4 + (g & 3);
        const unsigned long long b = __ballot((bm >> bit) & 1u);
        m = (grp == g) ? b : m;
    }
    return m;
}

struct FwdPixel {
    float T = 1.0f, C0 = 0.f, C1 = 0.f, C2 = 0.f, N0 = 0.f, N1 = 0.f, N2 = 0.f;
    float Dd = 0.f, M1 = 0.f, M2 = 0.f, distortion = 0.f, median_depth = 0.f;
    uint32_t last_contributor = 0, median_contributor = 0;
    bool done = false;

    template <int CHUNK>
    __device__ __forceinline__ void blend(const float4 *rec, const int j, const int base, bool valid,
                                          const Hit &h) {
        valid = valid && !done;
        const float test_T = T * (1.0f - h.alpha);
        const bool kill = valid && test_T < 0.0001f;
        done = done || kill;
        valid = valid && !kill;
        if (__ballot(valid) == 0ull) return;
        const float4 r4 = rec[4 * CHUNK + j], r5 = rec[5 * CHUNK + j];
        const float a = valid ? h.alpha : 0.f;
        const float depth = valid ? h.depth : 1.0f;
        const float w = a * T;
        const float A = 1.0f - T;
        const float mm = FAR_N / (FAR_N - NEAR_N) * (1.0f - NEAR_N * __builtin_amdgcn_rcpf(depth));
        distortion += (mm * mm * A + M2 - 2.0f * mm * M1) * w;
        Dd += depth * w;
        M1 += mm * w;
        M2 += mm * mm * w;
        const bool med = valid && T > 0.5f;
        median_depth = med ? depth : median_depth;
        median_contributor = med ? (uint32_t)(base + j + 1) : median_contributor;
        N0 += r4.x * w; N1 += r4.y * w; N2 += r4.z * w;
        C0 += r4.w * w; C1 += r5.x * w; C2 += r5.y * w;
        T = valid ? test_T : T;
        last_contributor = valid ? (uint32_t)(base + j + 1) : last_contributor;
    }

};

template <bool KEEP>
__global__ void __launch_bounds__(256)
composite_fwd_kernel(ViewDev v, const uint32_t *__restrict__ header, const uint2 *__restrict__ ranges,
                     const uint32_t *__restrict__ point_list, const float4 *__restrict__ geom,
                     const uint32_t *__restrict__ tile_order, const float4 *__restrict__ cullbox,
                     float *__restrict__ final_T, uint32_t *__restrict__ n_contrib,
                     const uint32_t *__restrict__ seg_base, const uint32_t *__restrict__ seg_cnt,
                     float *__restrict__ ckpt, uint2 *__restrict__ pair_mask, uint32_t *__restrict__ tile_maxc,
                     uint32_t *__restrict__ seg_cost,
                     float *__restrict__ out_color, float *__restrict__ out_allmap, const ViewBatch vb) {
    {
        const long long sst = vb.state_stride, HWb = (long long)v.H * v.W * 4;
        header = l2d_view_ptr(header, sst); ranges = l2d_view_ptr(ranges, sst); point_list = l2d_view_ptr(point_list, sst);
        geom = l2d_view_ptr(geom, sst); tile_order = l2d_view_ptr(tile_order, sst); cullbox = l2d_view_ptr(cullbox, sst);
        final_T = l2d_view_ptr(final_T, sst); n_contrib = l2d_view_ptr(n_contrib, sst); seg_base = l2d_view_ptr(seg_base, sst);
        seg_cnt = l2d_view_ptr(seg_cnt, sst); ckpt = l2d_view_ptr(ckpt, sst); pair_mask = l2d_view_ptr(pair_mask, sst);
        tile_maxc = l2d_view_ptr(tile_maxc, sst); seg_cost = l2d_view_ptr(seg_cost, sst);
        out_color = l2d_view_ptr(out_color, 3 * HWb); out_allmap = l2d_view_ptr(out_allmap, 7 * HWb);
        v.bg = vb.bg[blockIdx.z];
    }
    constexpr int CHUNK = FWD_CHUNK;
    static_assert(L2D_SEG % FWD_CHUNK == 0, "segment boundaries must fall on round boundaries");
    __shared__ float4 rec[REC4 * CHUNK];
    __shared__ unsigned long long qmask[4][16][CHUNK / 64];
    uint32_t &s_cost = *(uint32_t *)&rec[5 * CHUNK + 0].w;
    uint32_t &s_tmax = *(uint32_t *)&rec[5 * CHUNK + 1].w;
    uint32_t &s_ndone = *(uint32_t *)&rec[5 * CHUNK + 2].w;
    const int tile = (v.dbg & 8u) ? (int)blockIdx.x : (int)tile_order[blockIdx.x];
    const int tx = tile % v.gx, ty = tile / v.gx;
    const int wave = threadIdx.x >> 6, lane = threadIdx.x & 63;
    const int grp = lane >> 2;
    const int lxi = (wave & 1) * 8 + (grp & 3) * 2 + (lane & 1);
    const int lyi = (wave >> 1) * 8 + (grp >> 2) * 2 + ((lane >> 1) & 1);
    const int pxi = tx * TILE + lxi, pyi = ty * TILE + lyi;
    const bool inside = pxi < v.W && pyi < v.H;
    const size_t HW = (size_t)v.H * v.W;
    const size_t pix = (size_t)pyi * v.W + pxi;
    const float lx = (float)lxi, ly = (float)lyi;
    const float X0 = (float)(tx * TILE), Y0 = (float)(ty * TILE);

    if (header[1]) {
        if (inside) {
            const float qnan = __uint_as_float(0x7fc00000u);
            for (int ch = 0; ch < 3; ch++) out_color[ch * HW + pix] = qnan;
            for (int ch = 0; ch < 7; ch++) out_allmap[ch * HW + pix] = qnan;
            if (KEEP) {
                for (int ch = 0; ch < L2D_CKPT_F; ch++) final_T[pix + ch * HW] = qnan;
                n_contrib[pix] = 0; n_contrib[pix + HW] = 0;
            }
        }
        return;
    }

    const uint2 range = ranges[tile];
    const int total = (int)(range.y - range.x);
    const int lo = 0, hi = total;
    FwdPixel px;
    px.done = !inside;
    uint32_t *dbg_hdr = const_cast<uint32_t *>(header);
    const long long dbg_t0 = (v.dbg & 32u) ? (long long)__builtin_readcyclecounter() : 0ll;
    int dbg_rounds = 0;

    const int tid = threadIdx.x;
    const uint32_t cost_nb = KEEP ? seg_cnt[tile] : 0u;
    uint32_t *const cost_full = KEEP ? seg_cost + seg_base[tile] : nullptr,
             *const cost_last = KEEP ? seg_cost + (v.cap / L2D_SEG + 1u) + tile : nullptr;
    if (KEEP)
        for (uint32_t q = tid; q <= cost_nb; q += 256) *(q < cost_nb ? cost_full + q : cost_last) = 0u;
    int cost_round = -1;
    constexpr int SPT = CHUNK / 256;
    uint32_t id1[SPT], id2[SPT];
    float4 cb1[SPT];
#pragma unroll
    for (int q = 0; q < SPT; q++) {
        const int o = lo + q * 256 + tid;
        id1[q] = o < hi ? point_list[range.x + o] : 0u;
        id2[q] = CHUNK + o < hi ? point_list[range.x + CHUNK + o] : 0u;
    }
#pragma unroll
    for (int q = 0; q < SPT; q++) cb1[q] = lo + q * 256 + tid < hi ? cullbox[id1[q]] : make_float4(0.f, 0.f, 0.f, 0.f);
    if (threadIdx.x < 3) *(uint32_t *)&rec[5 * CHUNK + threadIdx.x].w = 0u;
    __syncthreads();
    for (int base = lo; base < hi; base += CHUNK) {
        {
            const bool wave_done = __ballot(px.done) == ~0ull;
            if (wave_done && lane == 0) atomicAdd(&s_ndone, 1u);
            __syncthreads();
            if (s_ndone == 4u) break;
        }
        if (KEEP && tid == 0) {
            if (cost_round >= 0) { if ((uint32_t)cost_round < cost_nb) cost_full[cost_round] = s_cost; else *cost_last += s_cost; }
            s_cost = 0u;
        }
        cost_round = (base - lo) / CHUNK;
        dbg_rounds++;
        if (KEEP && base && base % L2D_SEG == 0 && !px.done) {
            float *ck = ckpt + ((size_t)seg_base[tile] + (size_t)(base / L2D_SEG - 1)) * (L2D_CKPT_F * 256) + tid;
            ck[0 * 256] = px.T; ck[1 * 256] = px.M1; ck[2 * 256] = px.M2;
            ck[3 * 256] = px.C0; ck[4 * 256] = px.C1; ck[5 * 256] = px.C2;
            ck[6 * 256] = px.Dd; ck[7 * 256] = px.N0; ck[8 * 256] = px.N1; ck[9 * 256] = px.N2;
        }
#pragma unroll
        for (int q = 0; q < SPT; q++) {
            const int o = q * 256 + tid;
            const uint32_t id0 = id1[q];
            const float4 cb0 = cb1[q];
            id1[q] = id2[q];
            id2[q] = base + 2 * CHUNK + o < hi ? point_list[range.x + base + 2 * CHUNK + o] : 0u;
            cb1[q] = base + CHUNK + o < hi ? cullbox[id1[q]] : make_float4(0.f, 0.f, 0.f, 0.f);
            stage_entry<CHUNK>(geom, id0, cb0, base + o < hi, X0, Y0, rec, nullptr, o,
                               KEEP && base + o < hi ? pair_mask + range.x + base + o : nullptr);
        }
        __syncthreads();
        if (__ballot(!px.done) == 0ull) continue;
        const int nw = (min(CHUNK, hi - base) + 63) >> 6;
        unsigned long long *qm = &qmask[wave][grp][0];
#pragma unroll 1
        for (int w = 0; w < nw; w++) {
            const float4 *mrec = rec + ((wave >> 1) ? 5 : 3) * CHUNK + w * 64 + lane;
            const uint32_t bm = __float_as_uint((wave >> 1) ? mrec->z : mrec->w);
            unsigned long long m = 0ull;
            if (__ballot((bm & (0x0f0f0f0fu << ((wave & 1) * 4))) != 0u) != 0ull) m = quad_masks(bm, (wave & 1) * 4, grp);
            if ((lane & 3) == 0) qm[w] = m;
        }
        int w = 0;
        unsigned long long mm = qm[0];
        if (((__ballot(px.done) >> (lane & ~3)) & 0xfull) == 0xfull) { mm = 0ull; w = nw; }
        auto next = [&](bool &has, int &j) {
            while (mm == 0ull && w + 1 < nw) { w++; mm = qm[w]; }
            has = mm != 0ull;
            j = has ? 64 * w + __builtin_ctzll(mm) : 0;
            mm &= mm - 1ull;
        };
        bool hA0, hA1, hB0 = false, hB1 = false;
        int jA0, jA1, jB0 = 0, jB1 = 0;
        next(hA0, jA0);
        next(hA1, jA1);
        EntryRec rA0 = load_entry<CHUNK>(rec, jA0), rA1 = load_entry<CHUNK>(rec, jA1), rB0, rB1;
        auto trip = [&](const EntryRec &c0, const EntryRec &c1, const int j0, const int j1, const bool has0, const bool has1,
                        EntryRec &x0, EntryRec &x1, int &k0, int &k1, bool &n0, bool &n1) {
            next(n0, k0);
            next(n1, k1);
            x0 = load_entry<CHUNK>(rec, k0);
            x1 = load_entry<CHUNK>(rec, k1);
            Hit h0, h1;
            float Tw0[3], Tw1[3], opa0, opa1;
            const bool e0 = eval_rec(c0, lx, ly, h0, Tw0, opa0) && has0;
            const bool e1 = eval_rec(c1, lx, ly, h1, Tw1, opa1) && has1;
            if (v.dbg & 4u) {
                atomicAdd(&dbg_hdr[4], ((lane & 3) == 0) ? (unsigned)has0 + (unsigned)has1 : 0u);
                atomicAdd(&dbg_hdr[5], (unsigned)e0 + (unsigned)e1);
                if (lane == 0) atomicAdd(&dbg_hdr[6], 1u);
            }
            px.blend<CHUNK>(rec, j0, base, e0, h0);
            px.blend<CHUNK>(rec, j1, base, e1, h1);
            if (((__ballot(px.done) >> (lane & ~3)) & 0xfull) == 0xfull) { mm = 0ull; w = nw; n0 = false; n1 = false; }
        };
        uint32_t ntrips = 0;
        while (true) {
            if (__ballot(hA0) == 0ull) break;
            trip(rA0, rA1, jA0, jA1, hA0, hA1, rB0, rB1, jB0, jB1, hB0, hB1);
            ntrips++;
            if (__ballot(hB0) == 0ull) break;
            trip(rB0, rB1, jB0, jB1, hB0, hB1, rA0, rA1, jA0, jA1, hA0, hA1);
            ntrips++;
        }
        if (KEEP && lane == 0 && ntrips) atomicAdd(&s_cost, ntrips);
    }
    const float T = px.T;
    if (KEEP) {
        if (threadIdx.x == 0) s_tmax = 0u;
        __syncthreads();
        uint32_t m = px.last_contributor;
#pragma unroll
        for (int d = 1; d < 64; d <<= 1) m = max(m, (uint32_t)__shfl_xor((int)m, d, 64));
        if (lane == 0) atomicMax(&s_tmax, m);
        __syncthreads();
        if (threadIdx.x == 0) {
            tile_maxc[tile] = s_tmax;
            if (cost_round >= 0) { if ((uint32_t)cost_round < cost_nb) cost_full[cost_round] = s_cost; else *cost_last += s_cost; }
        }
    }
    if (inside) {
        if (KEEP) {
            final_T[pix] = T;
            final_T[pix + HW] = px.M1;
            final_T[pix + 2 * HW] = px.M2;
            final_T[pix + 3 * HW] = px.C0; final_T[pix + 4 * HW] = px.C1; final_T[pix + 5 * HW] = px.C2;
            final_T[pix + 6 * HW] = px.Dd;
            final_T[pix + 7 * HW] = px.N0; final_T[pix + 8 * HW] = px.N1; final_T[pix + 9 * HW] = px.N2;
            n_contrib[pix] = px.last_contributor;
            n_contrib[pix + HW] = px.median_contributor;
        }
        out_color[0 * HW + pix] = px.C0 + T * v.bg[0];
        out_color[1 * HW + pix] = px.C1 + T * v.bg[1];
        out_color[2 * HW + pix] = px.C2 + T * v.bg[2];
        out_allmap[0 * HW + pix] = px.Dd;
        out_allmap[1 * HW + pix] = 1.0f - T;
        out_allmap[2 * HW + pix] = px.N0;
        out_allmap[3 * HW + pix] = px.N1;
        out_allmap[4 * HW + pix] = px.N2;
        out_allmap[5 * HW + pix] = px.median_depth;
        out_allmap[6 * HW + pix] = px.distortion;
        if ((v.dbg & 32u) && lane == 0) {
            out_allmap[6 * HW + pix] = (float)((long long)__builtin_readcyclecounter() - dbg_t0);
            out_allmap[5 * HW + pix] = (float)dbg_rounds;
        }
    }
}

__device__ __forceinline__ float mul_legacy(const float a, const float b) {
    float r;
    asm("v_mul_legacy_f32 %0, %1, %2" : "=v"(r) : "v"(a), "v"(b));
    return r;
}

template <int CTRL>
__device__ __forceinline__ float dpp_full(float x) {
    return __int_as_float(__builtin_amdgcn_update_dpp(0, __float_as_int(x), CTRL, 0xf, 0xf, false));
}
struct QuadCoef { float a1, a2, a3, b1, b2, b3; };
__device__ __forceinline__ QuadCoef quad_coef(const int lane, const float lx, const float ly) {
    QuadCoef k;
    const int l = lane & 3;
    k.a1 = l == 0 ? 1.f : (l == 1 ? lx - 1.f : (l == 2 ? ly : 0.f));
    k.a2 = l == 1 ? 1.f : 0.f;
    k.a3 = l == 3 ? 1.f : 0.f;
    k.b1 = l == 0 ? ly : (l == 2 ? 1.f : (l == 3 ? lx - 1.f : 0.f));
    k.b2 = l == 3 ? 1.f : 0.f;
    k.b3 = l == 1 ? 1.f : 0.f;
    return k;
}
__device__ __forceinline__ void quad_reduce_scatter(const float dp[3], const float q[3], const float h[10], const QuadCoef &k,
                                                    float r[6], const int lane) {
    const bool b0 = lane & 1, b1 = lane & 2;
#pragma unroll
    for (int c = 0; c < 3; c++) {
        float d = dp[c];
        asm volatile("" : "+v"(d));
        const float t = d + dpp_full<0xB1>(d);
        const float tq = q[c] + dpp_full<0xB1>(q[c]);
        const float mine = k.a1 * t + (k.a2 * d + k.a3 * tq);
        const float send = k.b1 * t + (k.b2 * d + k.b3 * tq);
        r[c] = mine + dpp_full<0x4E>(send);
    }
    float v1[5];
#pragma unroll
    for (int i = 0; i < 5; i++) {
        const float mine = b0 ? h[2 * i + 1] : h[2 * i];
        const float send = b0 ? h[2 * i] : h[2 * i + 1];
        v1[i] = mine + dpp_full<0xB1>(send);
    }
#pragma unroll
    for (int i = 0; i < 2; i++) {
        const float mine = b1 ? v1[2 * i + 1] : v1[2 * i];
        const float send = b1 ? v1[2 * i] : v1[2 * i + 1];
        r[3 + i] = mine + dpp_full<0x4E>(send);
    }
    r[5] = v1[4] + dpp_full<0x4E>(v1[4]);
}
__device__ __forceinline__ void quad_reduce_scatter16(const float dp[3], const float q[3], const float h[4], const QuadCoef &k,
                                                      float r[4], const int lane) {
    const bool b0 = lane & 1, b1 = lane & 2;
#pragma unroll
    for (int c = 0; c < 3; c++) {
        float d = dp[c], qq = q[c];
        asm volatile("" : "+v"(d));
        asm volatile("" : "+v"(qq));
        const float t = d + dpp_full<0xB1>(d);
        const float tq = qq + dpp_full<0xB1>(qq);
        const float mine = k.a1 * t + (k.a2 * d + k.a3 * tq);
        const float send = k.b1 * t + (k.b2 * d + k.b3 * tq);
        r[c] = mine + dpp_full<0x4E>(send);
    }
    float v1[2];
#pragma unroll
    for (int i = 0; i < 2; i++) {
        const float mine = b0 ? h[2 * i + 1] : h[2 * i];
        const float send = b0 ? h[2 * i] : h[2 * i + 1];
        v1[i] = mine + dpp_full<0xB1>(send);
    }
    const float mine = b1 ? v1[1] : v1[0];
    const float send = b1 ? v1[0] : v1[1];
    r[3] = mine + dpp_full<0x4E>(send);
}

constexpr int SLAB_WIN = 128;
constexpr int SLAB_CHUNK = 128;
#ifndef L2D_SLAB_POOL
#define L2D_SLAB_POOL 374
#endif
constexpr int SLAB_POOL = L2D_SLAB_POOL;
constexpr int SLAB_F = 24;
constexpr int SLAB_F_COLOR = 16;
#ifdef L2D_COLOR_OCC4
constexpr int SLAB_POOL_COLOR = SLAB_POOL;
#else
constexpr int SLAB_POOL_COLOR = SLAB_POOL * SLAB_F / SLAB_F_COLOR;
#endif

template <bool MAPS>
#ifdef L2D_BWD_WAVES
__global__ void __launch_bounds__(256, L2D_BWD_WAVES)
#elif defined(L2D_COLOR_OCC4)
__global__ void __launch_bounds__(256, MAPS ? 1 : 4)
#else
__global__ void __launch_bounds__(256)
#endif
composite_bwd_kernel(ViewDev v, const uint32_t *__restrict__ header, const uint2 *__restrict__ ranges,
                     const uint32_t *__restrict__ point_list, const float4 *__restrict__ geom,
                     const uint32_t *__restrict__ tile_order, const float4 *__restrict__ cullbox,
                     const float *__restrict__ final_T, const uint32_t *__restrict__ n_contrib,
                     const uint32_t *__restrict__ seg_base, const uint32_t *__restrict__ seg_cnt,
                     const uint32_t *__restrict__ bwd_order,
                     const uint2 *__restrict__ bwd_items, const float *__restrict__ ckpt,
                     const uint2 *__restrict__ pair_mask, const uint32_t *__restrict__ tile_maxc,
                     const float *__restrict__ dL_dcolor, const float *__restrict__ dL_dallmap,
                     const uint32_t *__restrict__ pair_pos,
                     float4 *__restrict__ pair_grad, uint8_t *__restrict__ pair_valid, const ViewBatch vb) {
    {
        const long long sst = vb.state_stride, qst = vb.scratch_stride, HWb = (long long)v.H * v.W * 4;
        header = l2d_view_ptr(header, sst); ranges = l2d_view_ptr(ranges, sst); point_list = l2d_view_ptr(point_list, sst);
        geom = l2d_view_ptr(geom, sst); tile_order = l2d_view_ptr(tile_order, sst); cullbox = l2d_view_ptr(cullbox, sst);
        final_T = l2d_view_ptr(final_T, sst); n_contrib = l2d_view_ptr(n_contrib, sst); seg_base = l2d_view_ptr(seg_base, sst);
        seg_cnt = l2d_view_ptr(seg_cnt, sst); bwd_order = l2d_view_ptr(bwd_order, sst); bwd_items = l2d_view_ptr(bwd_items, sst);
        ckpt = l2d_view_ptr(ckpt, sst); pair_mask = l2d_view_ptr(pair_mask, sst); pair_pos = l2d_view_ptr(pair_pos, sst);
        tile_maxc = l2d_view_ptr(tile_maxc, sst);
        pair_grad = l2d_view_ptr(pair_grad, qst); pair_valid = l2d_view_ptr(pair_valid, qst);
        dL_dcolor = l2d_view_ptr(dL_dcolor, 3 * HWb); dL_dallmap = l2d_view_ptr(dL_dallmap, 7 * HWb);
        v.bg = vb.bg[blockIdx.z];
    }
    constexpr int WIN = SLAB_WIN;
    constexpr int POOL = MAPS ? SLAB_POOL : SLAB_POOL_COLOR, SF = MAPS ? SLAB_F : SLAB_F_COLOR;
    __shared__ float4 rec[REC4 * WIN];
    __shared__ __attribute__((aligned(16))) float pool[(POOL + 1) * SF];
    __shared__ uint16_t s_base_[2][SLAB_CHUNK];
    __shared__ unsigned long long s_live_[2][SLAB_CHUNK];
    __shared__ uint32_t s_ql[64];
    __shared__ uint32_t s_id_[2][WIN];
    __shared__ uint2 s_mask[WIN];
    __shared__ int s_nfit_[2];
    __shared__ uint32_t s_total_[2];
    if (header[1]) return;
    const unsigned long long dbg_t0 = (v.dbg & 32u) ? wall_clock64() : 0ull;
    int dbg_rounds = 0;
    uint32_t dbg_windows = 0, dbg_trips = 0, dbg_entries = 0, dbg_slots = 0, dbg_rows = 0;
    unsigned long long dbg_tp = 0ull;
    uint32_t dbg_ph[5] = {0u, 0u, 0u, 0u, 0u};
#define DBG_PHASE(k) do { if (v.dbg & 64u) { const unsigned long long t__ = __builtin_readcyclecounter(); dbg_ph[k] += (uint32_t)(t__ - dbg_tp); dbg_tp = t__; } } while (0)
    if (v.dbg & 64u) dbg_tp = __builtin_readcyclecounter();
    const uint32_t n_full = header[3];
    int tile, seg;
    if (header[22]) {
        if (blockIdx.x >= n_full + (uint32_t)v.tiles) return;
        const uint2 it = bwd_items[blockIdx.x];
        tile = (int)it.x; seg = (int)it.y;
    } else if (blockIdx.x < n_full) {
        const uint2 it = bwd_items[blockIdx.x];
        tile = (int)it.x; seg = (int)it.y;
    } else if (blockIdx.x - n_full < (uint32_t)v.tiles) {
        tile = (int)bwd_order[blockIdx.x - n_full];
        seg = (int)seg_cnt[tile];
    } else {
        return;
    }
    const uint2 range = ranges[tile];
    const int seg_lo = seg * L2D_SEG;
    const int seg_hi = seg == (int)seg_cnt[tile] ? (int)(range.y - range.x) : seg_lo + L2D_SEG;
    const int total = min((int)tile_maxc[tile], seg_hi);
    const int lo = seg_lo;
    if (total <= lo) return;
    const int tx = tile % v.gx, ty = tile / v.gx;
    const int tid = threadIdx.x, wave = tid >> 6, lane = tid & 63;
    const int grp = lane >> 2;
    const int lxi = (wave & 1) * 8 + (grp & 3) * 2 + (lane & 1);
    const int lyi = (wave >> 1) * 8 + (grp >> 2) * 2 + ((lane >> 1) & 1);
    const int pxi = tx * TILE + lxi, pyi = ty * TILE + lyi;
    const bool inside = pxi < v.W && pyi < v.H;
    const size_t HW = (size_t)v.H * v.W;
    const size_t pix = inside ? (size_t)pyi * v.W + pxi : 0;
    const float lx = (float)lxi, ly = (float)lyi;
    const float X0 = (float)(tx * TILE), Y0 = (float)(ty * TILE);

    const float T_final = inside ? final_T[pix] : 0.f;
    float T = T_final;
    const uint32_t last_contributor = inside ? n_contrib[pix] : 0u;
    const uint32_t median_contributor = (MAPS && inside) ? n_contrib[pix + HW] : 0u;
    float dpix[3] = {0.f, 0.f, 0.f}, dnrm[3] = {0.f, 0.f, 0.f};
    float dL_ddepth = 0.f, dL_daccum = 0.f, dL_dmedian = 0.f, dL_dreg = 0.f;
    float final_D = 0.f, final_D2 = 0.f;
    if (inside) {
        for (int ch = 0; ch < 3; ch++) dpix[ch] = dL_dcolor[ch * HW + pix];
        if constexpr (MAPS) {
            dL_ddepth = dL_dallmap[0 * HW + pix];
            dL_daccum = dL_dallmap[1 * HW + pix];
            for (int ch = 0; ch < 3; ch++) dnrm[ch] = dL_dallmap[(2 + ch) * HW + pix];
            dL_dmedian = dL_dallmap[5 * HW + pix];
            dL_dreg = dL_dallmap[6 * HW + pix];
            final_D = final_T[pix + HW];
            final_D2 = final_T[pix + 2 * HW];
        }
    }
    const float final_A = 1.0f - T_final;
    const float bg_dot_dpixel = v.bg[0] * dpix[0] + v.bg[1] * dpix[1] + v.bg[2] * dpix[2];

    float accum_g = 0.f, last_g = 0.f, last_alpha = 0.f;
    float last_dL_dT = 0.f;

    const int my_blk = (lyi >> 1) * 8 + (lxi >> 1);
    const uint32_t below_lo = my_blk >= 32 ? 0xffffffffu : (1u << my_blk) - 1u;
    const uint32_t below_hi = my_blk >= 32 ? (1u << (my_blk - 32)) - 1u : 0u;
    const QuadCoef qcoef = quad_coef(lane, lx, ly);
    uint32_t quad_last = last_contributor;
    quad_last = max(quad_last, (uint32_t)__builtin_amdgcn_update_dpp(0, (int)quad_last, 0xB1, 0xf, 0xf, false));
    quad_last = max(quad_last, (uint32_t)__builtin_amdgcn_update_dpp(0, (int)quad_last, 0x4E, 0xf, 0xf, false));
    if ((lane & 3) == 0) s_ql[my_blk] = quad_last;
    if (tid < SF) pool[POOL * SF + tid] = 0.f;

    if ((int)last_contributor > seg_hi) {
        const float *ck = ckpt + ((size_t)seg_base[tile] + (size_t)seg) * (L2D_CKPT_F * 256) + tid;
        const float Tb = ck[0], inv_Tb = 1.0f / Tb;
        T = Tb;
        const float s_alpha = (Tb - T_final) * inv_Tb;
        if constexpr (MAPS) {
            const float s_m1 = (final_D - ck[1 * 256]) * inv_Tb, s_m2 = (final_D2 - ck[2 * 256]) * inv_Tb;
            float sg = (Tb - T_final) * dL_daccum + (final_T[pix + 6 * HW] - ck[6 * 256]) * dL_ddepth;
            for (int ch = 0; ch < 3; ch++)
                sg += (final_T[pix + (3 + ch) * HW] - ck[(3 + ch) * 256]) * dpix[ch] +
                      (final_T[pix + (7 + ch) * HW] - ck[(7 + ch) * 256]) * dnrm[ch];
            accum_g = sg * inv_Tb;
            last_dL_dT = (final_D2 * s_alpha + final_A * s_m2 - 2.0f * final_D * s_m1) * dL_dreg;
        } else {
            (void)s_alpha;
            float sg = 0.f;
            for (int ch = 0; ch < 3; ch++) {
                float p = (final_T[pix + (3 + ch) * HW] - ck[(3 + ch) * 256]) * dpix[ch];
                asm volatile("" : "+v"(p));
                sg += p;
            }
            accum_g = sg * inv_Tb;
        }
    }

    const int se = tid - 128;
    const bool stager = se >= 0;
    uint32_t id1 = 0u, id2 = 0u;
    uint2 mk1 = make_uint2(0u, 0u), mk2 = mk1;
    auto size_round = [&](const int whi_, const int wcnt_, const int s0_, const int buf, const bool side) {
        unsigned long long *const live_ = s_live_[buf];
        uint16_t *const base_ = s_base_[buf];
                const int jm = max(whi_ - s0_ - (int)s_ql[lane], 0);
                unsigned long long la = ~0ull, lb = ~0ull;
                if (__ballot(jm > 0) != 0ull) {
                    volatile unsigned long long *vlive = live_;
                    vlive[2 * lane] = 0ull;
                    vlive[2 * lane + 1] = 0ull;
                    if (jm < SLAB_CHUNK) atomicOr(&live_[jm], 1ull << lane);
                    __builtin_amdgcn_wave_barrier();
                    la = vlive[2 * lane];
                    lb = la | vlive[2 * lane + 1];
                    unsigned long long ex = lb;
#pragma unroll
                    for (int d = 1; d < 64; d <<= 1) {
                        const uint32_t ylo = __shfl_up((uint32_t)ex, d, 64), yhi = __shfl_up((uint32_t)(ex >> 32), d, 64);
                        if (lane >= d) ex |= ((unsigned long long)yhi << 32) | ylo;
                    }
                    const uint32_t plo = __shfl_up((uint32_t)ex, 1, 64), phi = __shfl_up((uint32_t)(ex >> 32), 1, 64);
                    const unsigned long long before = lane ? (((unsigned long long)phi << 32) | plo) : 0ull;
                    la |= before; lb |= before;
                }
                uint32_t c[2];
#pragma unroll
                for (int q = 0; q < 2; q++) {
                    const int slot = s0_ + 2 * lane + q;
                    unsigned long long mk = 0ull;
                    if (slot < wcnt_) {
                        const uint2 mw = side ? s_mask[slot] : make_uint2(__float_as_uint(rec[3 * WIN + slot].w), __float_as_uint(rec[5 * WIN + slot].z));
                        mk = (((unsigned long long)mw.y << 32) | mw.x) & (q ? lb : la);
                    }
                    live_[2 * lane + q] = mk;
                    c[q] = (uint32_t)__builtin_popcountll(mk);
                }
                uint32_t incl = c[0] + c[1];
#pragma unroll
                for (int d = 1; d < 64; d <<= 1) {
                    const uint32_t y = __shfl_up(incl, d, 64);
                    if (lane >= d) incl += y;
                }
                const uint32_t b0 = incl - c[0] - c[1], b1 = incl - c[1];
                const unsigned long long f0 = __ballot(s0_ + 2 * lane < wcnt_ && b1 <= (uint32_t)POOL);
                const unsigned long long f1 = __ballot(s0_ + 2 * lane + 1 < wcnt_ && incl <= (uint32_t)POOL);
                const int L = f1 == ~0ull ? 64 : __builtin_ctzll(~f1);
                if (lane == 0) s_nfit_[buf] = L == 64 ? 128 : 2 * L + (int)((f0 >> L) & 1ull);
                base_[2 * lane] = (uint16_t)b0;
                base_[2 * lane + 1] = (uint16_t)b1;
                if (lane == 63) s_total_[buf] = incl;
    };
    {
        const int wcnt = min(WIN, total - lo);
        if (stager) {
            const uint32_t id0 = total - 1 - se >= lo ? point_list[range.x + total - 1 - se] : 0u;
            const uint2 mk0 = total - 1 - se >= lo ? pair_mask[range.x + total - 1 - se] : make_uint2(0u, 0u);
            id1 = total - WIN - 1 - se >= lo ? point_list[range.x + total - WIN - 1 - se] : 0u;
            mk1 = total - WIN - 1 - se >= lo ? pair_mask[range.x + total - WIN - 1 - se] : make_uint2(0u, 0u);
            id2 = total - 2 * WIN - 1 - se >= lo ? point_list[range.x + total - 2 * WIN - 1 - se] : 0u;
            mk2 = total - 2 * WIN - 1 - se >= lo ? pair_mask[range.x + total - 2 * WIN - 1 - se] : make_uint2(0u, 0u);
            stage_entry_masked<WIN>(geom, id0, mk0, se < wcnt, X0, Y0, rec, s_id_[0], se);
        }
        __syncthreads();
        if (wave == 3) size_round(total, wcnt, 0, 0, false);
        __syncthreads();
        DBG_PHASE(0);
    }
    int cur = 0, wb = 0;
    for (int whi = total; whi > lo; whi -= WIN) {
        const int wcnt = min(WIN, whi - lo);
        const bool more_windows = whi - WIN > lo;
        dbg_windows++;
        if (stager) s_mask[se] = mk1;
        unsigned long long wm0 = 0ull, wm1 = 0ull;

        for (int s0 = 0; s0 < wcnt;) {
            dbg_rounds++;
            const unsigned long long *const s_live = s_live_[cur];
            const uint16_t *const s_base = s_base_[cur];
            const uint32_t *const s_id = s_id_[wb];
            const int nfit = s_nfit_[cur];
            if (v.dbg & 512u) { dbg_entries += (uint32_t)nfit; dbg_slots += nfit < SLAB_CHUNK ? (uint32_t)s_base[nfit] : min(s_total_[cur], (uint32_t)POOL); }

            {
                if (s0 == 0) {
#pragma unroll
                    for (int k = 0; k < 2; k++) {
                        const float4 *mrec = rec + ((wave >> 1) ? 5 : 3) * WIN + 64 * k + lane;
                        const uint32_t bm = __float_as_uint((wave >> 1) ? mrec->z : mrec->w);
                        unsigned long long m = 0ull;
                        if (__ballot((bm & (0x0f0f0f0fu << ((wave & 1) * 4))) != 0u) != 0ull) m = quad_masks(bm, (wave & 1) * 4, grp);
                        if (k == 0) wm0 = m; else wm1 = m;
                    }
                }
                unsigned long long m0 = wm0, m1 = wm1;
                {
                    int sh = s0;
                    if (sh >= 64) { m0 = m1; m1 = 0ull; sh -= 64; }
                    if (sh) { m0 = (m0 >> sh) | (m1 << (64 - sh)); m1 >>= sh; }
                    if (nfit < 64) { m0 &= (1ull << nfit) - 1ull; m1 = 0ull; }
                    else if (nfit < 128) m1 &= (1ull << (nfit - 64)) - 1ull;
                }
                const int jmin = whi - s0 - (int)quad_last;
                if (jmin > 0) {
                    m0 = jmin >= 64 ? 0ull : m0 & (~0ull << jmin);
                    m1 = jmin >= 128 ? 0ull : (jmin > 64 ? m1 & (~0ull << (jmin - 64)) : m1);
                }
                uint32_t mm = (uint32_t)m0, q1 = (uint32_t)(m0 >> 32), q2 = (uint32_t)m1, q3 = (uint32_t)(m1 >> 32);
                int jb = 0;
                auto trip = [&]() __attribute__((always_inline)) {
                    dbg_trips++;
                    while (mm == 0u && (q1 | q2 | q3) != 0u) { mm = q1; q1 = q2; q2 = q3; q3 = 0u; jb += 32; }
                    const bool has = mm != 0u;
                    const int j = jb + (has ? __builtin_ctz(mm) : 0);
                    mm &= mm - 1u;
                    const int ws = s0 + j;
                    const uint32_t contributor = (uint32_t)(whi - 1 - ws);
                    const EntryRec ent = load_entry<WIN>(rec, ws);
                    Hit h;
                    float Tw[3], opa;
                    const bool active = eval_rec(ent, lx, ly, h, Tw, opa) && has && contributor < last_contributor;
                    const float4 r4 = rec[4 * WIN + ws], r5 = rec[5 * WIN + ws];
                    const float nrm[3] = {r4.x, r4.y, r4.z}, rgb[3] = {r4.w, r5.x, r5.y};
                    if constexpr (!MAPS) {
                        (void)nrm;
                        const float alpha = active ? h.alpha : 0.f;
                        const float inv_1ma = __builtin_amdgcn_rcpf(1.f - alpha);
                        const float T_new = T * inv_1ma;
                        const float w = alpha * T_new;
                        const float gval = __builtin_fmaf(rgb[2], dpix[2], __builtin_fmaf(rgb[0], dpix[0], rgb[1] * dpix[1]));
                        const float accum_new = mul_legacy(last_alpha, last_g) + (1.f - last_alpha) * accum_g;
                        float dL_dalpha = gval - accum_new;
                        dL_dalpha = __builtin_fmaf(T_new, dL_dalpha, -((T_final * inv_1ma) * bg_dot_dpixel));
                        T = T_new;
                        accum_g = accum_new;
                        last_g = gval;
                        last_alpha = alpha;
                        const float da = active ? dL_dalpha : 0.f;
                        const float sx = h.sx, sy = h.sy;
                        const float rz3 = (active && h.use3d) ? h.rz : 0.f;
                        const float qG = opa * da * h.G;
                        const float dL_dsx = -mul_legacy(qG, sx), dL_dsy = -mul_legacy(qG, sy);
                        const float dpx = dL_dsx * rz3, dpy = dL_dsy * rz3;
                        const float dpv[3] = {dpx, dpy, -(mul_legacy(dpx, sx) + mul_legacy(dpy, sy))};
                        const float qG2 = h.use3d ? 0.f : -FILTER_INV_SQUARE * qG;
                        const float q3[3] = {h.G * da, qG2 * h.ddx, qG2 * h.ddy};
                        const float h4[4] = {w * dpix[0], w * dpix[1], w * dpix[2], w};
                        float r[4];
                        quad_reduce_scatter16(dpv, q3, h4, qcoef, r, lane);
#pragma unroll
                        for (int i = 0; i < 4; i++) asm volatile("" : "+v"(r[i]));
                        const unsigned long long lv = s_live[has ? j : 0];
                        const int rank = __builtin_popcount((uint32_t)lv & below_lo) + __builtin_popcount((uint32_t)(lv >> 32) & below_hi);
                        float4 *ps = (float4 *)(pool + ((int)s_base[has ? j : 0] + rank) * SF) + (lane & 3);
                        if (has) *ps = make_float4(r[0], r[1], r[2], r[3]);
                    } else {
                    const float alpha = active ? h.alpha : 0.f, c_d = h.depth;
                    const float inv_1ma = __builtin_amdgcn_rcpf(1.f - alpha);
                    const float T_new = T * inv_1ma;
                    const float w = alpha * T_new;
                    const float gval = rgb[0] * dpix[0] + rgb[1] * dpix[1] + rgb[2] * dpix[2] +
                                       nrm[0] * dnrm[0] + nrm[1] * dnrm[1] + nrm[2] * dnrm[2] +
                                       c_d * dL_ddepth + dL_daccum;
                    const float accum_new = mul_legacy(last_alpha, last_g) + (1.f - last_alpha) * accum_g;
                    float dL_dalpha = gval - accum_new;
                    float dL_dz = 0.0f;
                    const float inv_cd = __builtin_amdgcn_rcpf(c_d);
                    const float m_d = FAR_N / (FAR_N - NEAR_N) * (1.f - NEAR_N * inv_cd);
                    const float dmd_dd = (FAR_N * NEAR_N) / (FAR_N - NEAR_N) * inv_cd * inv_cd;
                    if (contributor + 1 == median_contributor) dL_dz += dL_dmedian;
                    const float dL_dweight = (final_D2 + m_d * m_d * final_A - 2.f * m_d * final_D) * dL_dreg;
                    dL_dalpha += dL_dweight - last_dL_dT;
                    const float dLdT_new = mul_legacy(alpha, dL_dweight) + (1.f - alpha) * last_dL_dT;
                    const float dL_dmd = 2.0f * (T_new * alpha) * (m_d * final_A - final_D) * dL_dreg;
                    dL_dz += dL_dmd * dmd_dd;
                    dL_dalpha *= T_new;
                    dL_dalpha += (-T_final * inv_1ma) * bg_dot_dpixel;
                    dL_dz += w * dL_ddepth;
                    T = T_new;
                    accum_g = accum_new;
                    last_g = gval;
                    last_alpha = alpha;
                    last_dL_dT = dLdT_new;
                    const float ww = w, da = active ? dL_dalpha : 0.f, dz = active ? dL_dz : 0.f;
                    const float sx = h.sx, sy = h.sy;
                    const float rz3 = (active && h.use3d) ? h.rz : 0.f;
                    const float qv[3] = {mul_legacy(dz, sx), mul_legacy(dz, sy), dz};
                    const float qG = opa * da * h.G;
                    const float dL_dsx = dz * Tw[0] - mul_legacy(qG, sx);
                    const float dL_dsy = dz * Tw[1] - mul_legacy(qG, sy);
                    const float dpx = dL_dsx * rz3, dpy = dL_dsy * rz3;
                    const float dpv[3] = {dpx, dpy, -(mul_legacy(dpx, sx) + mul_legacy(dpy, sy))};
                    const float qG2 = h.use3d ? 0.f : -FILTER_INV_SQUARE * qG;
                    const float hv[10] = {qG2 * h.ddx, qG2 * h.ddy, ww * dnrm[0], ww * dnrm[1], ww * dnrm[2], h.G * da,
                                          ww * dpix[0], ww * dpix[1], ww * dpix[2], ww};
                    float r[6];
                    quad_reduce_scatter(dpv, qv, hv, qcoef, r, lane);
#pragma unroll
                    for (int i = 0; i < 6; i++) asm volatile("" : "+v"(r[i]));
                    const unsigned long long lv = s_live[has ? j : 0];
                    const int rank = __builtin_popcount((uint32_t)lv & below_lo) + __builtin_popcount((uint32_t)(lv >> 32) & below_hi);
                    float *ps = pool + ((int)s_base[has ? j : 0] + rank) * SLAB_F + (lane & 3);
                    if (has) {
                        ps[0] = r[0]; ps[4] = r[1]; ps[8] = r[2]; ps[12] = r[3]; ps[16] = r[4];
                        if (!(lane & 2)) ps[20] = r[5];
                    }
                    }
                };
                while (__ballot((mm | q1 | q2 | q3) != 0u) != 0ull) {
                    trip();
#ifndef L2D_WALK_NO_UNROLL
                    if (__ballot((mm | q1 | q2 | q3) != 0u) == 0ull) break;
                    trip();
#endif
                }
            }
            __syncthreads();
            DBG_PHASE(3);

            if ((wave << 5) < nfit && !(v.dbg & 2u)) {
                const int e = tid >> 1, part = tid & 1;
                const int ws = min(s0 + e, WIN - 1);
                const bool has = e < nfit;
                const int cnt = has ? __builtin_popcountll(s_live[e]) : 0;
                float4 gq0 = make_float4(0.f, 0.f, 0.f, 0.f), gq1 = gq0, gq2 = gq0;
                if (cnt && part == 0) {
                    const float4 *gm = geom + (size_t)s_id[ws] * 5;
                    gq0 = gm[0]; gq1 = gm[1]; gq2 = gm[2];
                }
                constexpr int NG = MAPS ? 22 : 16;
                float g[NG];
                const float4 *ps = (const float4 *)(pool + (int)s_base[e] * SF);
                {
                    const float4 *p0 = part < cnt ? ps + part * (SF / 4) : (const float4 *)(pool + POOL * SF);
#pragma unroll
                    for (int q = 0; q < NG / 4; q++) {
                        const float4 t = p0[q];
                        g[4 * q] = t.x; g[4 * q + 1] = t.y; g[4 * q + 2] = t.z; g[4 * q + 3] = t.w;
                    }
                    if constexpr (MAPS) {
                        const float2 t2 = *(const float2 *)(p0 + 5);
                        g[20] = t2.x; g[21] = t2.y;
                    }
                }
                for (int i = part + 2; i < cnt; i += 2) {
#pragma unroll
                    for (int q = 0; q < NG / 4; q++) {
                        const float4 t = ps[i * (SF / 4) + q];
                        g[4 * q] += t.x; g[4 * q + 1] += t.y; g[4 * q + 2] += t.z; g[4 * q + 3] += t.w;
                    }
                    if constexpr (MAPS) {
                        const float2 t2 = *(const float2 *)(ps + i * (SF / 4) + 5);
                        g[20] += t2.x; g[21] += t2.y;
                    }
                }
#pragma unroll
                for (int k = 0; k < NG; k++) g[k] += dpp_full<0xB1>(g[k]);
                const bool touched = (MAPS ? g[21] : g[15]) > 0.f;
                if (part == 0 && touched) {
                    const uint32_t p = range.x + (uint32_t)(whi - 1 - ws);
                    const float4 g0 = gq0, g1 = gq1, g2 = gq2;
                    const float Tu[3] = {g0.x, g0.y, g0.z}, Tv[3] = {g0.w, g1.x, g1.y}, Tw[3] = {g1.z, g1.w, g2.x};
                    const float k0[3] = {X0 * Tw[0] - Tu[0], X0 * Tw[1] - Tu[1], X0 * Tw[2] - Tu[2]};
                    const float l0[3] = {Y0 * Tw[0] - Tv[0], Y0 * Tw[1] - Tv[1], Y0 * Tw[2] - Tv[2]};
                    const float a[3] = {g[0], MAPS ? g[4] : g[1], MAPS ? g[8] : g[2]};
                    const float b[3] = {MAPS ? g[1] : g[4], g[5], MAPS ? g[9] : g[6]};
                    const float cc[3] = {MAPS ? g[2] : g[8], MAPS ? g[6] : g[9], g[10]};
                    const float qd[3] = {MAPS ? g[3] : 0.f, MAPS ? g[7] : 0.f, MAPS ? g[11] : 0.f};
                    float t1[3], t2[3], dk0[3], dl0[3], dTw[3];
                    cross3(l0, a, t1); cross3(Tw, cc, t2);
                    for (int i = 0; i < 3; i++) dk0[i] = t1[i] + t2[i];
                    cross3(a, k0, t1); cross3(b, Tw, t2);
                    for (int i = 0; i < 3; i++) dl0[i] = t1[i] + t2[i];
                    cross3(l0, b, t1); cross3(cc, k0, t2);
                    for (int i = 0; i < 3; i++) {
                        dTw[i] = t1[i] + t2[i] + X0 * dk0[i] + Y0 * dl0[i];
                        if constexpr (MAPS) dTw[i] += qd[i];
                    }
                    const uint32_t q = pair_pos[p];
                    float4 *row = pair_grad + (size_t)q * (GRAD_F / 4);
                    row[0] = make_float4(-dk0[0], -dk0[1], -dk0[2], -dl0[0]);
                    row[1] = make_float4(-dl0[1], -dl0[2], dTw[0], dTw[1]);
                    if constexpr (MAPS) {
                        row[2] = make_float4(dTw[2], g[12], g[13], g[14]);
                        row[3] = make_float4(g[15], g[16], g[17], g[18]);
                        row[4] = make_float4(g[19], g[20], 0.f, 0.f);
                    } else {
                        row[2] = make_float4(dTw[2], g[13], g[14], 0.f);
                        row[3] = make_float4(0.f, 0.f, g[12], g[3]);
                        row[4] = make_float4(g[7], g[11], 0.f, 0.f);
                    }
                    pair_valid[q] = 1;
                    dbg_rows++;
                }
            }
            const bool last_round = s0 + nfit >= wcnt;
            if (stager && last_round && more_windows) {
                stage_entry_masked<WIN>(geom, id1, mk1, se < min(WIN, whi - WIN - lo), X0, Y0, rec, s_id_[wb ^ 1], se);
                id1 = id2;
                mk1 = mk2;
                id2 = whi - 3 * WIN - 1 - se >= lo ? point_list[range.x + whi - 3 * WIN - 1 - se] : 0u;
                mk2 = whi - 3 * WIN - 1 - se >= lo ? pair_mask[range.x + whi - 3 * WIN - 1 - se] : make_uint2(0u, 0u);
            }
            if (wave == 3) {
                if (!last_round) size_round(whi, wcnt, s0 + nfit, cur ^ 1, false);
                else if (more_windows) size_round(whi - WIN, min(WIN, whi - WIN - lo), 0, cur ^ 1, true);
            }
            __syncthreads();
            DBG_PHASE(4);
            s0 += nfit;
            cur ^= 1;
        }
        wb ^= 1;
    }
    if ((v.dbg & 64u) && tid == 0) {
        DBG_PHASE(4);
        uint32_t *h = const_cast<uint32_t *>(header);
        for (int k = 0; k < 5; k++) atomicAdd(&h[16 + k], dbg_ph[k] >> 6);
    }
    if (v.dbg & 512u) {
        uint32_t *h = const_cast<uint32_t *>(header);
        if (tid == 0) {
            atomicAdd(&h[24], 1u); atomicAdd(&h[25], dbg_windows); atomicAdd(&h[26], (uint32_t)dbg_rounds);
            atomicAdd(&h[28], dbg_entries); atomicAdd(&h[29], dbg_slots);
        }
        if (lane == 0) atomicAdd(&h[27], dbg_trips);
        if (dbg_rows) atomicAdd(&h[30], dbg_rows);
    }
    if ((v.dbg & 32u) && tid == 0) {
        uint32_t *h = const_cast<uint32_t *>(header);
        const unsigned long long t1 = wall_clock64();
        atomicMax(&h[8], (uint32_t)(t1 - dbg_t0));
        atomicMax((unsigned long long *)&h[12], ((unsigned long long)(uint32_t)(t1 - dbg_t0) << 32) |
                                                    ((unsigned long long)dbg_rounds << 16) | (unsigned long long)blockIdx.x);
        atomicAdd(&h[9], (uint32_t)(t1 - dbg_t0));
        atomicMax(&h[10], ~(uint32_t)dbg_t0);
        atomicMax(&h[11], (uint32_t)t1);
    }
}

__global__ void __launch_bounds__(64)
selftest_butterfly_kernel(const float *__restrict__ in, float *__restrict__ out) {
    const int lane = threadIdx.x, q4 = lane & 3, grp = lane >> 2;
    const float lx = (float)((grp & 3) * 2 + (lane & 1)), ly = (float)((grp >> 2) * 2 + ((lane >> 1) & 1));
    float dp[3], q[3], h[10], r[6];
    for (int k = 0; k < 3; k++) { dp[k] = in[lane * 16 + k]; q[k] = in[lane * 16 + 3 + k]; }
    for (int k = 0; k < 10; k++) h[k] = in[lane * 16 + 6 + k];
    quad_reduce_scatter(dp, q, h, quad_coef(lane, lx, ly), r, lane);
    float *dst = out + (lane >> 2) * 24 + q4;
    for (int i = 0; i < 5; i++) dst[4 * i] = r[i];
    if (q4 < 2) dst[20] = r[5];
}

constexpr int BO_PER_THREAD = 17;
__global__ void __launch_bounds__(1024)
bwd_order_kernel(ViewDev v, uint32_t *__restrict__ header, uint2 *__restrict__ bwd_items, const uint32_t *__restrict__ seg_cnt,
                 const uint32_t *__restrict__ seg_cost, const long long sst, char *__restrict__ zero_base, const long long zero_bytes,
                 const long long qst) {
    if (blockIdx.x >= 1) {
        uint4 *z = (uint4 *)l2d_view_ptr(zero_base, qst);
        const long long n16 = zero_bytes / 16;
        for (long long i = (long long)(blockIdx.x - 1) * 1024 + threadIdx.x; i < n16; i += (long long)(gridDim.x - 1) * 1024)
            z[i] = make_uint4(0u, 0u, 0u, 0u);
        return;
    }
    header = l2d_view_ptr(header, sst); bwd_items = l2d_view_ptr(bwd_items, sst); seg_cnt = l2d_view_ptr(seg_cnt, sst);
    seg_cost = l2d_view_ptr(seg_cost, sst);
    __shared__ uint32_t bcnt[64];
    if (header[1] || (v.dbg & 256u)) return;
    const int tid = threadIdx.x, lane = tid & 63;
    if (header[22]) return;
    const uint32_t n_full = header[3], n = n_full + (uint32_t)v.tiles;
    if (n > (uint32_t)(BO_PER_THREAD * 1024)) return;
    const uint32_t *cost_last = seg_cost + (v.cap / L2D_SEG + 1u);
    if (tid < 64) bcnt[tid] = 0u;
    __syncthreads();
    uint2 item[BO_PER_THREAD];
    uint32_t bkt[BO_PER_THREAD];
#pragma unroll
    for (int k = 0; k < BO_PER_THREAD; k++) {
        const uint32_t i = (uint32_t)tid + 1024u * k;
        bkt[k] = 64u;
        if (i < n) {
            uint32_t c;
            if (i < n_full) { item[k] = bwd_items[i]; c = seg_cost[i]; }
            else { const uint32_t t = i - n_full; item[k] = make_uint2(t, seg_cnt[t]); c = cost_last[t]; }
            bkt[k] = 63u - min(63u, c >> 2);
            atomicAdd(&bcnt[bkt[k]], 1u);
        }
    }
    __syncthreads();
    if (tid < 64) {
        const uint32_t c = bcnt[tid];
        uint32_t x = c;
#pragma unroll
        for (int d = 1; d < 64; d <<= 1) {
            const uint32_t y = __shfl_up(x, d, 64);
            if (lane >= d) x += y;
        }
        bcnt[tid] = x - c;
    }
    __syncthreads();
#pragma unroll
    for (int k = 0; k < BO_PER_THREAD; k++)
        if (bkt[k] < 64u) bwd_items[atomicAdd(&bcnt[bkt[k]], 1u)] = item[k];
    if (tid == 0) header[22] = 1u;
}

}

int launch_composite_fwd(const ViewDev &v, StateView st, ScratchView sc, float *out_color, float *out_allmap,
                         hipStream_t s, const ViewBatch &vb) {
    (void)sc;
    const unsigned nz = (unsigned)vb.n;
    {
        L2D_PROF(v.fwd_only ? "composite_fwd_only" : "composite_fwd", s);
        auto kern = v.fwd_only ? composite_fwd_kernel<false> : composite_fwd_kernel<true>;
        hipLaunchKernelGGL(kern, dim3(v.tiles, 1, nz), dim3(256), 0, s, v, st.header, st.ranges, st.point_list,
                           (const float4 *)st.geom, st.tile_order, (const float4 *)st.cullbox, st.final_T, st.n_contrib, st.seg_base,
                           st.seg_cnt, st.ckpt, st.pair_mask, st.tile_maxc, st.seg_cost, out_color, out_allmap, vb);
    }
    L2D_CHECK_LAUNCH();
    return LARA2DGS_OK;
}

int launch_bwd_order(const ViewDev &v, StateView st, ScratchView sc, hipStream_t s, const ViewBatch &vb, void *zero_base, int64_t zero_bytes) {
    (void)sc;
    L2D_PROF("bwd_order", s);
    const int64_t zb = (zero_bytes + 15) / 16 * 16;
    const unsigned zw = zb > 0 ? (unsigned)((zb / 16 + 8191) / 8192 < 128 ? (zb / 16 + 8191) / 8192 : 128) : 0u;
    hipLaunchKernelGGL(bwd_order_kernel, dim3(1 + zw, 1, (unsigned)vb.n), dim3(1024), 0, s, v, st.header, st.bwd_items, st.seg_cnt,
                       st.seg_cost, vb.state_stride, (char *)zero_base, (long long)zb, vb.scratch_stride);
    L2D_CHECK_LAUNCH();
    return LARA2DGS_OK;
}

int launch_composite_bwd(const ViewDev &v, StateView st, ScratchView sc, const float *dL_dcolor,
                         const float *dL_dallmap, hipStream_t s, const ViewBatch &vb) {
    {
        L2D_PROF(dL_dallmap ? "composite_bwd" : "composite_bwd_color", s);
        const unsigned grid = (unsigned)v.tiles + v.cap / L2D_SEG;
        auto kern = dL_dallmap ? composite_bwd_kernel<true> : composite_bwd_kernel<false>;
        hipLaunchKernelGGL(kern, dim3(grid, 1, (unsigned)vb.n), dim3(256), 0, s, v, st.header, st.ranges,
                           st.point_list, (const float4 *)st.geom, st.tile_order,
                           (const float4 *)st.cullbox, st.final_T, st.n_contrib, st.seg_base, st.seg_cnt, st.bwd_order,
                           st.bwd_items, st.ckpt, st.pair_mask, st.tile_maxc, dL_dcolor, dL_dallmap, st.pair_pos, sc.pair_grad,
                           (uint8_t *)sc.pair_valid, vb);
    }
    L2D_CHECK_LAUNCH();
    return LARA2DGS_OK;
}

int launch_selftest_butterfly(const float *in, float *out, hipStream_t s) {
    hipLaunchKernelGGL(selftest_butterfly_kernel, dim3(1), dim3(64), 0, s, in, out);
    L2D_CHECK_LAUNCH();
    return LARA2DGS_OK;
}
```

### lara_amd/rasterizer.py

```python
from __future__ import annotations

import collections
import ctypes
import os
import threading
import time
import warnings
from typing import NamedTuple, Optional

import torch
from torch import nn

_HERE = os.path.dirname(os.path.abspath(__file__))
LIB_PATH = os.environ.get("LARA2DGS_LIB") or os.path.join(_HERE, "liblara2dgs.so")
ABI_VERSION = 10


class _View(ctypes.Structure):
    _fields_ = [
        ("P", ctypes.c_int32), ("sh_degree", ctypes.c_int32), ("sh_coeffs", ctypes.c_int32),
        ("image_height", ctypes.c_int32), ("image_width", ctypes.c_int32),
        ("tanfovx", ctypes.c_float), ("tanfovy", ctypes.c_float), ("scale_modifier", ctypes.c_float),
        ("prefiltered", ctypes.c_int32), ("debug", ctypes.c_int32), ("forward_only", ctypes.c_int32),
        ("capacity", ctypes.c_int64),
        ("bg", ctypes.c_void_p), ("viewmatrix", ctypes.c_void_p),
        ("projmatrix", ctypes.c_void_p), ("campos", ctypes.c_void_p),
        ("counts_out", ctypes.c_void_p),
    ]


class _Subset(ctypes.Structure):
    _fields_ = [("coarse_state", ctypes.c_void_p), ("coarse_state_stride", ctypes.c_int64), ("coarse_capacity", ctypes.c_int64),
                ("coarse_P", ctypes.c_int32), ("coarse_forward_only", ctypes.c_int32), ("inv", ctypes.c_void_p)]


class GradLayout(ctypes.Structure):
    _fields_ = [(n, ctypes.c_int64) for n in
                ("means3D", "means2D", "shs", "colors", "opacities", "scales", "rotations", "transmat", "total")]


class StateLayout(ctypes.Structure):
    _fields_ = [(n, ctypes.c_int64) for n in
                ("header", "geom", "cullbox", "point_list", "ranges", "tile_order", "pair_base", "pair_pos", "final_T", "n_contrib",
                 "seg_base", "seg_cnt", "bwd_order", "bwd_items", "ckpt", "pair_mask", "tile_maxc", "seg_cost", "total")]


_lib = None


def load_library():
    global _lib
    if _lib is not None:
        return _lib
    if not os.path.exists(LIB_PATH):
        raise RuntimeError(
            f"lara_amd: HIP library not found at {LIB_PATH}. Build it with "
            "`python -c 'import __graft_entry__ as g; g.build()'` or `make -C lara_amd/csrc`. "
            "There is no CPU fallback.")
    lib = ctypes.CDLL(LIB_PATH)
    vp, i32, i64 = ctypes.c_void_p, ctypes.c_int32, ctypes.c_int64
    lib.lara2dgs_abi_version.restype = ctypes.c_int
    lib.lara2dgs_error_string.restype = ctypes.c_char_p
    lib.lara2dgs_error_string.argtypes = [ctypes.c_int]
    lib.lara2dgs_last_hip_error.restype = ctypes.c_int
    lib.lara2dgs_state_bytes.restype = i64
    lib.lara2dgs_state_bytes.argtypes = [i32, i32, i32, i64, i32]
    lib.lara2dgs_scratch_bytes.restype = i64
    lib.lara2dgs_scratch_bytes.argtypes = [i32, i32, i32, i64, i32]
    lib.lara2dgs_get_state_layout.restype = ctypes.c_int
    lib.lara2dgs_get_state_layout.argtypes = [i32, i32, i32, i64, i32, ctypes.POINTER(StateLayout)]
    lib.lara2dgs_forward.restype = ctypes.c_int
    lib.lara2dgs_forward.argtypes = [ctypes.POINTER(_View)] + [vp] * 13
    lib.lara2dgs_backward.restype = ctypes.c_int
    lib.lara2dgs_backward.argtypes = [ctypes.POINTER(_View)] + [vp] * 20
    lib.lara2dgs_forward_views.restype = ctypes.c_int
    lib.lara2dgs_forward_views.argtypes = [i32, ctypes.POINTER(_View)] + [vp] * 11 + [i64, vp, i64, vp]
    lib.lara2dgs_forward_views_subset.restype = ctypes.c_int
    lib.lara2dgs_forward_views_subset.argtypes = [i32, ctypes.POINTER(_View)] + [vp] * 11 + [i64, vp, i64, ctypes.POINTER(_Subset), vp]
    lib.lara2dgs_backward_views.restype = ctypes.c_int
    lib.lara2dgs_backward_views.argtypes = [i32, ctypes.POINTER(_View)] + [vp] * 10 + [i64, vp, i64, vp, vp]
    lib.lara2dgs_get_grad_layout.restype = ctypes.c_int
    lib.lara2dgs_get_grad_layout.argtypes = [i32, i32, i32, i32, i32, i32, ctypes.POINTER(GradLayout)]
    lib.lara2dgs_mark_visible.restype = ctypes.c_int
    lib.lara2dgs_mark_visible.argtypes = [i32, vp, vp, vp, vp, vp]
    lib.lara2dgs_profile_enable.restype = ctypes.c_int
    lib.lara2dgs_profile_enable.argtypes = [ctypes.c_int]
    lib.lara2dgs_profile_collect.restype = ctypes.c_int
    lib.lara2dgs_profile_collect.argtypes = [ctypes.c_char_p, ctypes.c_int, ctypes.POINTER(ctypes.c_float), ctypes.c_int]
    lib.lara2dgs_selftest.restype = ctypes.c_int
    lib.lara2dgs_selftest.argtypes = [ctypes.c_int, vp, vp, vp]
    if lib.lara2dgs_abi_version() != ABI_VERSION:
        raise RuntimeError("lara_amd: liblara2dgs.so ABI version mismatch; rebuild the library")
    _lib = lib
    return lib


def _check(rc: int, what: str):
    if rc != 0:
        lib = load_library()
        raise RuntimeError(f"lara_amd: {what} failed: {lib.lara2dgs_error_string(rc).decode()} "
                           f"(hipError {lib.lara2dgs_last_hip_error()})")


_cull_transparent = os.environ.get("LARA2DGS_CULL_TRANSPARENT", "0") == "1"


def set_cull_transparent(on: bool) -> bool:
    global _cull_transparent
    prev, _cull_transparent = _cull_transparent, bool(on)
    return prev


def _dup_factor() -> int:
    return int(os.environ.get("LARA2DGS_DUP_FACTOR", "4"))


def _sizing_P(P: int) -> int:
    if P <= 32768:
        return max(-(-P // 1024) * 1024, 1024)
    return (P + 32767) // 65536 * 65536 + 32768


_HISTORY = 256
_hist = {}
_reruns = 0


def _bucket(device: torch.device, P: int, H: int, W: int):
    return (device.index, _sizing_P(P), int(H), int(W))


def _cap_grid(n: int) -> int:
    n = max(int(n), 1 << 20)
    k = 1 << (n - 1).bit_length()
    if k // 4 * 3 >= n:
        k = k // 4 * 3
    return min(k, 0xFFFFFFFF)


def note_pair_count(bucket, D: int):
    h = _hist.get(bucket)
    if h is None:
        h = _hist[bucket] = collections.deque(maxlen=_HISTORY)
    h.append(int(D))


def _recent_max(bucket) -> int:
    h = _hist.get(bucket)
    return max(h) if h else 0


def _next_capacity(bucket) -> int:
    return _cap_grid(max(bucket[1] * _dup_factor(), 2 * _recent_max(bucket)))


def binning_capacity(P: int, H: int = 0, W: int = 0, device: Optional[torch.device] = None) -> int:
    if device is None:
        return _cap_grid(_sizing_P(P) * _dup_factor())
    return _next_capacity(_bucket(device, P, H, W))


_longest = {}


def capacity_report() -> dict:
    rep = {b: {"D_max": max(h), "calls": len(h), "capacity": _cap_grid(max(b[1] * _dup_factor(), 2 * max(h))),
               "longest_list": _longest.get(b, 0)}
           for b, h in _hist.items() if h}
    rep["reruns"] = _reruns
    return rep


def reset_capacity_history():
    _hist.clear()
    _longest.clear()


_tls = threading.local()
_COUNT_SPINS = 4000
_counts_fallbacks = 0


class _Counts:

    def __init__(self, n):
        self.t = torch.zeros((max(n, 16), 4), dtype=torch.int32).pin_memory()
        self.np = self.t.numpy().view("uint32")
        self.ptr = self.t.data_ptr()


def _counts(n) -> _Counts:
    c = getattr(_tls, "counts", None)
    if c is None or c.np.shape[0] < n:
        c = _tls.counts = _Counts(n)
    return c


def _wait_counts(c: _Counts, n: int, done: torch.cuda.Event, headers):
    global _counts_fallbacks
    ready = c.np[:n, 3]
    spins = 0
    while not ready.all():
        spins += 1
        if spins > _COUNT_SPINS:
            if done.query() and not ready.all():
                _counts_fallbacks += 1
                h = headers().cpu().numpy().view("uint32").reshape(n, -1)
                return int(h[:, 0].max()), bool(h[:, 1].any())
            time.sleep(0)
    return int(c.np[:n, 0].max()), bool(c.np[:n, 1].any())


def _run_forward(bucket, n, enqueue, debug=False):
    global _reruns
    cap = _next_capacity(bucket)
    c = _counts(n)
    while True:
        c.np[:n, 3] = 0
        state, headers, extra = enqueue(cap, c.ptr)
        done = torch.cuda.Event()
        done.record()
        D, overflow = _wait_counts(c, n, done, headers)
        note_pair_count(bucket, D)
        if bool(c.np[:n, 3].all()):
            _longest[bucket] = max(_longest.get(bucket, 0), int(c.np[:n, 2].max()))
        if not overflow:
            break
        new_cap = _cap_grid(max(2 * D, bucket[1] * _dup_factor()))
        if new_cap <= cap:
            raise RuntimeError(
                f"lara_amd: a view produced {D} (tile, surfel) pairs, beyond the 32-bit pair index the buffers use "
                f"(capacity {cap}); its outputs were poisoned with NaN.")
        _reruns += 1
        state = headers = None
        cap = new_cap
    if debug:
        torch.cuda.current_stream().synchronize()
    return state, cap, extra, D


_scratch = {}


_GUARD = 1 << 16
_guards = []


def _poison_mode() -> bool:
    return os.environ.get("LARA2DGS_POISON_BUFFERS") == "1"


def _alloc_bytes(n: int, device: torch.device) -> torch.Tensor:
    if not _poison_mode():
        return torch.empty(n, dtype=torch.uint8, device=device)
    whole = torch.empty(n + 2 * _GUARD, dtype=torch.uint8, device=device)
    whole.fill_(255)
    _guards.append((whole, n))
    return whole[_GUARD:_GUARD + n]


def check_poison_guards() -> list:
    torch.cuda.synchronize()
    bad = [n for whole, n in _guards
           if not bool((whole[:_GUARD] == 255).all()) or not bool((whole[_GUARD + n:] == 255).all())]
    _guards.clear()
    return bad


def _get_scratch(device: torch.device, nbytes: int) -> torch.Tensor:
    if _poison_mode():
        return _alloc_bytes(nbytes, device)
    key = (device.index, torch.cuda.current_stream(device).cuda_stream)
    buf = _scratch.get(key)
    if buf is None or buf.numel() < nbytes:
        buf = torch.empty(int(nbytes * 1.25) + 256, dtype=torch.uint8, device=device)
        _scratch[key] = buf
    return buf


def _prep(t: Optional[torch.Tensor], name: str, device) -> Optional[torch.Tensor]:
    if t is None or t.numel() == 0:
        return None
    if t.device != device:
        raise RuntimeError(f"lara_amd: `{name}` is on {t.device}, expected {device}")
    if t.dtype != torch.float32:
        if not t.is_floating_point():
            raise RuntimeError(f"lara_amd: `{name}` must be a floating-point tensor, got {t.dtype}")
        t = t.float()
    if not t.is_contiguous():
        t = t.contiguous()
    if t.data_ptr() % 16:
        t = t.clone()
    return t


def _ptr(t: Optional[torch.Tensor]):
    return None if t is None else t.data_ptr()


class GaussianRasterizationSettings(NamedTuple):
    image_height: int
    image_width: int
    tanfovx: float
    tanfovy: float
    bg: torch.Tensor
    scale_modifier: float
    viewmatrix: torch.Tensor
    projmatrix: torch.Tensor
    sh_degree: int
    campos: torch.Tensor
    prefiltered: bool
    debug: bool


def _make_view(rs: GaussianRasterizationSettings, P: int, M: int, cap: int, device):
    bg = _prep(rs.bg, "bg", device)
    vm = _prep(rs.viewmatrix, "viewmatrix", device)
    pm = _prep(rs.projmatrix, "projmatrix", device)
    cp = _prep(rs.campos, "campos", device)
    if bg is None or vm is None or pm is None or cp is None:
        raise RuntimeError("lara_amd: bg / viewmatrix / projmatrix / campos must be non-empty tensors")
    if bg.numel() != 3 or vm.numel() != 16 or pm.numel() != 16 or cp.numel() != 3:
        raise RuntimeError("lara_amd: bg[3], viewmatrix[4,4], projmatrix[4,4], campos[3] expected")
    v = _View(P, int(rs.sh_degree), M, int(rs.image_height), int(rs.image_width),
              float(rs.tanfovx), float(rs.tanfovy), float(rs.scale_modifier),
              int(bool(rs.prefiltered)) | (2 if _cull_transparent else 0), int(bool(rs.debug)), 0, cap,
              bg.data_ptr(), vm.data_ptr(), pm.data_ptr(), cp.data_ptr(), None)
    return v, (bg, vm, pm, cp)


def _validate(means3D, sh, colors_precomp, opacities, scales, rotations, cov3Ds_precomp, sh_degree):
    if means3D.dim() != 2 or means3D.shape[1] != 3:
        raise RuntimeError("means3D must have dimensions (num_points, 3)")
    if not means3D.is_cuda:
        raise RuntimeError("lara_amd: tensors must live on an MI355X (HIP) device; there is no CPU path")
    device = means3D.device
    P = means3D.shape[0]
    means3D_c = _prep(means3D, "means3D", device)
    if means3D_c is None:
        means3D_c = means3D.contiguous()
    sh_c = _prep(sh, "shs", device)
    col_c = _prep(colors_precomp, "colors_precomp", device)
    opa_c = _prep(opacities, "opacities", device)
    sc_c = _prep(scales, "scales", device)
    rot_c = _prep(rotations, "rotations", device)
    tm_c = _prep(cov3Ds_precomp, "cov3D_precomp", device)
    M = 0
    if sh_c is not None:
        if sh_c.dim() != 3 or sh_c.shape[0] != P or sh_c.shape[2] != 3:
            raise RuntimeError("shs must have dimensions (num_points, num_coeffs, 3)")
        M = sh_c.shape[1]
        if M < (int(sh_degree) + 1) ** 2:
            raise RuntimeError("shs holds fewer coefficients than sh_degree needs")
    for t, n, k in ((opa_c, "opacities", 1), (sc_c, "scales", 2), (rot_c, "rotations", 4),
                    (tm_c, "cov3D_precomp", 9), (col_c, "colors_precomp", 3)):
        if t is not None and t.numel() != P * k:
            raise RuntimeError(f"{n} must hold {k} value(s) per point")
    return device, P, M, (means3D_c, sh_c, col_c, opa_c, sc_c, rot_c, tm_c)


def _needs_state(*tensors) -> bool:
    return torch.is_grad_enabled() and any(t is not None and t.requires_grad for t in tensors)


def _views_array(settings, P, M, cap, device, prefiltered_bits=None):
    arr = (_View * len(settings))()
    keep = []
    for i, rs in enumerate(settings):
        v, k = _make_view(rs, P, M, cap, device)
        if prefiltered_bits is not None:
            v.prefiltered = prefiltered_bits
        arr[i] = v
        keep.extend(k)
    return arr, keep


def _forward_views_impl(means3D, sh, colors_precomp, opacities, scales, rotations, cov3Ds_precomp, settings, forward_only=False,
                        subset=None, batched=True):
    lib = load_library()
    rs0 = settings[0]
    n = len(settings)
    for rs in settings[1:]:
        if (rs.image_height, rs.image_width, rs.sh_degree, bool(rs.prefiltered), float(rs.scale_modifier), bool(rs.debug)) != \
                (rs0.image_height, rs0.image_width, rs0.sh_degree, bool(rs0.prefiltered), float(rs0.scale_modifier), bool(rs0.debug)):
            raise RuntimeError("lara_amd: the views of one multi-view call must agree in image size, sh_degree, prefiltered, "
                               "scale_modifier and debug")
    device, P, M, (means3D_c, sh_c, col_c, opa_c, sc_c, rot_c, tm_c) = _validate(
        means3D, sh, colors_precomp, opacities, scales, rotations, cov3Ds_precomp, rs0.sh_degree)
    H, W = int(rs0.image_height), int(rs0.image_width)
    fo = int(bool(forward_only))
    with torch.cuda.device(device):
        views, keep = _views_array(settings, P, M, 0, device)
        lead = (n,) if batched else ()
        color = torch.empty(lead + (3, H, W), dtype=torch.float32, device=device)
        allmap = torch.empty(lead + (7, H, W), dtype=torch.float32, device=device)
        radii = torch.empty(lead + (P,), dtype=torch.int32, device=device)
        sub = None
        if subset is not None and P > 0:
            c_state, c_sb, c_cap, c_P, idx = subset
            if idx.numel() != P or idx.device != device or c_P < P:
                raise RuntimeError("lara_amd: `subset_of` needs one index per surfel of this call, on its device")
            inv = torch.full((c_P,), -1, dtype=torch.int32, device=device)
            inv[idx] = torch.arange(P, dtype=torch.int32, device=device)
            sub = _Subset(c_state.data_ptr(), c_sb, c_cap, c_P, 0, inv.data_ptr())

        def enqueue(cap, counts_ptr):
            for i in range(n):
                views[i].capacity = cap
                views[i].forward_only = fo
                views[i].counts_out = counts_ptr + 16 * i
            sb = (lib.lara2dgs_state_bytes(_sizing_P(P), H, W, cap, fo) + 255) // 256 * 256
            qb = (lib.lara2dgs_scratch_bytes(_sizing_P(P), H, W, cap, fo) + 255) // 256 * 256
            state = _alloc_bytes(n * sb, device)
            scratch = _get_scratch(device, n * qb)
            args = (n, views, _ptr(means3D_c), _ptr(sh_c), _ptr(col_c), _ptr(opa_c), _ptr(sc_c), _ptr(rot_c), _ptr(tm_c),
                    color.data_ptr(), allmap.data_ptr(), radii.data_ptr(), state.data_ptr(), sb, scratch.data_ptr(), qb)
            if sub is None:
                rc = lib.lara2dgs_forward_views(*args, torch.cuda.current_stream(device).cuda_stream)
            else:
                rc = lib.lara2dgs_forward_views_subset(*args, ctypes.byref(sub), torch.cuda.current_stream(device).cuda_stream)
            _check(rc, "lara2dgs_forward_views")
            return state, (lambda: state.view(n, sb)[:, :64].contiguous().view(torch.int32)), (sb, qb)

        state, cap, (sb, qb), D = _run_forward(_bucket(device, P, H, W), n, enqueue, any(rs.debug for rs in settings))
    return dict(color=color, radii=radii, allmap=allmap, state=state, cap=cap, strides=(sb, qb), D=D, M=M, keep=keep,
                inputs=(means3D_c, sh_c, col_c, sc_c, rot_c, tm_c))


class _RasterizeViews(torch.autograd.Function):

    @staticmethod
    def forward(ctx, means3D, means2D, sh, colors_precomp, opacities, scales, rotations, cov3Ds_precomp, settings, subset=None,
                batched=True):
        settings = tuple(settings)
        rs0 = settings[0]
        r = _forward_views_impl(means3D, sh, colors_precomp, opacities, scales, rotations, cov3Ds_precomp, settings, subset=subset,
                                batched=batched)
        color, radii, allmap, M, keep = r["color"], r["radii"], r["allmap"], r["M"], r["keep"]
        means3D_c, sh_c, col_c, sc_c, rot_c, tm_c = r["inputs"]
        ctx.state, ctx.cap, ctx.strides, ctx.D = r["state"], r["cap"], r["strides"], r["D"]
        ctx.settings = settings
        ctx.M = M
        ctx.prefiltered_bits = int(bool(rs0.prefiltered)) | (2 if _cull_transparent else 0)
        ctx.flags = (sh_c is not None, col_c is not None, sc_c is not None, tm_c is not None)
        ctx.shapes = (sh.shape if sh_c is not None else None, opacities.shape)
        empty = means3D_c.new_empty(0)
        ctx.save_for_backward(means3D_c, sh_c if sh_c is not None else empty, col_c if col_c is not None else empty,
                              sc_c if sc_c is not None else empty, rot_c if rot_c is not None else empty,
                              tm_c if tm_c is not None else empty, radii, *keep)
        ctx.mark_non_differentiable(radii)
        ctx.set_materialize_grads(False)
        return color, radii, allmap

    @staticmethod
    def backward(ctx, grad_color, grad_radii, grad_allmap):
        lib = load_library()
        means3D, sh, col, sc, rot, tm, radii = ctx.saved_tensors[:7]
        cams = ctx.saved_tensors[7:]
        has_sh, has_col, has_sr, has_tm = ctx.flags
        settings = ctx.settings
        n = len(settings)
        rs0 = settings[0]
        device = means3D.device
        P = means3D.shape[0]
        H, W = int(rs0.image_height), int(rs0.image_width)
        state, cap, (sb, qb) = ctx.state, ctx.cap, ctx.strides
        G = GradLayout()
        _check(lib.lara2dgs_get_grad_layout(P, ctx.M, int(has_sh), int(has_col), int(has_sr), int(has_tm), ctypes.byref(G)),
               "lara2dgs_get_grad_layout")
        with torch.cuda.device(device):
            if grad_color is None:
                grad_color = torch.zeros((n, 3, H, W), dtype=torch.float32, device=device)
            grad_color = _prep(grad_color, "grad_color", device)
            if grad_allmap is not None:
                grad_allmap = _prep(grad_allmap, "grad_allmap", device)
            views = (_View * n)()
            for i, rs in enumerate(settings):
                bg, vm, pm, cp = cams[4 * i:4 * i + 4]
                views[i] = _View(P, int(rs.sh_degree), ctx.M, H, W, float(rs.tanfovx), float(rs.tanfovy),
                                 float(rs.scale_modifier), ctx.prefiltered_bits, int(bool(rs.debug)), 0, cap,
                                 bg.data_ptr(), vm.data_ptr(), pm.data_ptr(), cp.data_ptr(), None)
            out = torch.empty((max(G.total, 4),), dtype=torch.float32, device=device)
            scratch = _get_scratch(device, n * qb)
            stream = torch.cuda.current_stream(device).cuda_stream
            rc = lib.lara2dgs_backward_views(
                n, views, _ptr(means3D), _ptr(sh if has_sh else None), _ptr(col if has_col else None),
                _ptr(sc if has_sr else None), _ptr(rot if has_sr else None), _ptr(tm if has_tm else None),
                radii.data_ptr(), grad_color.data_ptr(), _ptr(grad_allmap), state.data_ptr(), sb,
                scratch.data_ptr(), qb, out.data_ptr(), stream)
            _check(rc, "lara2dgs_backward_views")

        def sec(off, k, shape):
            return None if off < 0 else out[off:off + P * k].view(shape)
        g_sh = sec(G.shs, ctx.M * 3, (P, ctx.M, 3)) if has_sh else None
        if g_sh is not None and ctx.shapes[0] is not None:
            g_sh = g_sh.view(ctx.shapes[0])
        g_opac = sec(G.opacities, 1, (P, 1)).view(ctx.shapes[1])
        return (sec(G.means3D, 3, (P, 3)), sec(G.means2D, 3, (P, 3)) if ctx.needs_input_grad[1] else None, g_sh,
                sec(G.colors, 3, (P, 3)) if has_col else None, g_opac,
                sec(G.scales, 2, (P, 2)) if has_sr else None, sec(G.rotations, 4, (P, 4)) if has_sr else None,
                sec(G.transmat, 9, (P, 9)) if has_tm else None, None, None, None)


def rasterize_gaussians_views(settings, means3D, means2D, opacities, shs=None, colors_precomp=None, scales=None,
                              rotations=None, cov3D_precomp=None, subset_of=None):
    if len(settings) == 0:
        raise RuntimeError("lara_amd: rasterize_gaussians_views needs at least one view")
    if (shs is None and colors_precomp is None) or (shs is not None and colors_precomp is not None):
        raise Exception('Please provide excatly one of either SHs or precomputed colors!')
    if ((scales is None or rotations is None) and cov3D_precomp is None) or \
            ((scales is not None or rotations is not None) and cov3D_precomp is not None):
        raise Exception('Please provide exactly one of either scale/rotation pair or precomputed 3D covariance!')
    means3D, means2D, shs, colors_precomp, opacities, scales, rotations, cov3D_precomp = (
        _as_f32(t) for t in (means3D, means2D, shs, colors_precomp, opacities, scales, rotations, cov3D_precomp))
    if not _needs_state(means3D, means2D, shs, colors_precomp, opacities, scales, rotations, cov3D_precomp):
        r = _forward_views_impl(means3D, shs, colors_precomp, opacities, scales, rotations, cov3D_precomp, tuple(settings), True)
        return r["color"], r["radii"], r["allmap"]
    subset = None
    if subset_of is not None:
        coarse_color, idx = subset_of
        node = getattr(coarse_color, "grad_fn", None)
        if node is not None and hasattr(node, "strides") and hasattr(node, "state") and len(node.settings) == len(settings):
            for a, b in zip(node.settings, settings):
                if (a.image_height, a.image_width, a.tanfovx, a.tanfovy, float(a.scale_modifier)) != \
                        (b.image_height, b.image_width, b.tanfovx, b.tanfovy, float(b.scale_modifier)) or \
                        a.viewmatrix.data_ptr() != b.viewmatrix.data_ptr() or a.projmatrix.data_ptr() != b.projmatrix.data_ptr():
                    raise RuntimeError("lara_amd: `subset_of` names a call with other cameras")
            subset = (node.state, node.strides[0], node.cap, node.saved_tensors[0].shape[0], idx.contiguous())
    return _RasterizeViews.apply(means3D, means2D, shs, colors_precomp, opacities, scales, rotations, cov3D_precomp,
                                 tuple(settings), subset)


def _as_f32(t):
    return t.float() if (t is not None and t.is_floating_point() and t.dtype != torch.float32) else t


def rasterize_gaussians(means3D, means2D, sh, colors_precomp, opacities, scales, rotations,
                        cov3Ds_precomp, raster_settings):
    means3D, means2D, sh, colors_precomp, opacities, scales, rotations, cov3Ds_precomp = (
        _as_f32(t) for t in (means3D, means2D, sh, colors_precomp, opacities, scales, rotations, cov3Ds_precomp))
    if not _needs_state(means3D, means2D, sh, colors_precomp, opacities, scales, rotations, cov3Ds_precomp):
        r = _forward_views_impl(means3D, sh, colors_precomp, opacities, scales, rotations, cov3Ds_precomp, (raster_settings,), True,
                                batched=False)
        return r["color"], r["radii"], r["allmap"]
    return _RasterizeViews.apply(means3D, means2D, sh, colors_precomp, opacities, scales, rotations, cov3Ds_precomp,
                                 (raster_settings,), None, False)


class GaussianRasterizer(nn.Module):

    def __init__(self, raster_settings: GaussianRasterizationSettings):
        super().__init__()
        self.raster_settings = raster_settings

    def markVisible(self, positions: torch.Tensor) -> torch.Tensor:
        lib = load_library()
        rs = self.raster_settings
        with torch.no_grad():
            if not positions.is_cuda:
                raise RuntimeError("lara_amd: tensors must live on an MI355X (HIP) device")
            device = positions.device
            pos = _prep(positions, "positions", device)
            P = positions.shape[0]
            present = torch.zeros((P,), dtype=torch.uint8, device=device)
            vm = _prep(rs.viewmatrix, "viewmatrix", device)
            pm = _prep(rs.projmatrix, "projmatrix", device)
            with torch.cuda.device(device):
                rc = lib.lara2dgs_mark_visible(P, _ptr(pos), vm.data_ptr(), pm.data_ptr(),
                                               present.data_ptr(),
                                               torch.cuda.current_stream(device).cuda_stream)
            _check(rc, "lara2dgs_mark_visible")
        return present.bool()

    def forward(self, means3D, means2D, opacities, shs=None, colors_precomp=None, scales=None,
                rotations=None, cov3D_precomp=None):
        raster_settings = self.raster_settings
        if (shs is None and colors_precomp is None) or (shs is not None and colors_precomp is not None):
            raise Exception('Please provide excatly one of either SHs or precomputed colors!')
        if ((scales is None or rotations is None) and cov3D_precomp is None) or \
                ((scales is not None or rotations is not None) and cov3D_precomp is not None):
            raise Exception('Please provide exactly one of either scale/rotation pair or precomputed 3D covariance!')
        return rasterize_gaussians(means3D, means2D, shs, colors_precomp, opacities, scales,
                                   rotations, cov3D_precomp, raster_settings)


def state_views(state: torch.Tensor, P: int, H: int, W: int, cap: int, forward_only: bool = False) -> dict:
    lib = load_library()
    L = StateLayout()
    _check(lib.lara2dgs_get_state_layout(P, H, W, cap, int(forward_only), ctypes.byref(L)), "lara2dgs_get_state_layout")
    tiles = ((W + 15) // 16) * ((H + 15) // 16)

    def sec(off, nbytes, dtype, shape):
        return state[off:off + nbytes].view(dtype).view(shape)

    hdr = sec(L.header, 256, torch.int32, (64,))
    common = dict(
        header=hdr,
        geom=sec(L.geom, P * 80, torch.float32, (P, 20)),
        cullbox=sec(L.cullbox, P * 16, torch.float32, (P, 4)),
        point_list=sec(L.point_list, cap * 4, torch.int32, (cap,)),
        ranges=sec(L.ranges, tiles * 8, torch.int32, (tiles, 2)),
        tile_order=sec(L.tile_order, tiles * 4, torch.int32, (tiles,)))
    if forward_only:
        return common
    return dict(
        common,
        pair_base=sec(L.pair_base, (P + 1) * 4, torch.int32, (P + 1,)),
        pair_pos=sec(L.pair_pos, cap * 4, torch.int32, (cap,)),
        final_T=sec(L.final_T, 10 * H * W * 4, torch.float32, (10, H, W)),
        n_contrib=sec(L.n_contrib, 2 * H * W * 4, torch.int32, (2, H, W)),
        seg_base=sec(L.seg_base, (tiles + 1) * 4, torch.int32, (tiles + 1,)),
        seg_cnt=sec(L.seg_cnt, tiles * 4, torch.int32, (tiles,)),
        bwd_order=sec(L.bwd_order, tiles * 4, torch.int32, (tiles,)),
        bwd_items=sec(L.bwd_items, (cap // 512 + 1 + tiles) * 8, torch.int32, (cap // 512 + 1 + tiles, 2)),
        pair_mask=sec(L.pair_mask, cap * 8, torch.int64, (cap,)),
        tile_maxc=sec(L.tile_maxc, tiles * 4, torch.int32, (tiles,)),
        seg_cost=sec(L.seg_cost, (cap // 512 + 1 + tiles) * 4, torch.int32, (cap // 512 + 1 + tiles,)),
    )


def forward_with_state(raster_settings, means3D, opacities, shs=None, colors_precomp=None,
                       scales=None, rotations=None, cov3D_precomp=None, forward_only=False) -> dict:
    with torch.no_grad():
        r = _forward_views_impl(means3D, shs, colors_precomp, opacities, scales, rotations, cov3D_precomp, (raster_settings,),
                                forward_only, batched=False)
    P = means3D.shape[0]
    r["views"] = state_views(r["state"], P, int(raster_settings.image_height),
                             int(raster_settings.image_width), r["cap"], forward_only)
    return r


def profile_enable(on: bool = True):
    load_library().lara2dgs_profile_enable(int(on))


def profile_collect(max_entries: int = 65536) -> list:
    lib = load_library()
    names = ctypes.create_string_buffer(max_entries * 24)
    ms = (ctypes.c_float * max_entries)()
    n = lib.lara2dgs_profile_collect(names, len(names), ms, max_entries)
    parts = names.raw.split(b"\0")
    return [(parts[i].decode(), float(ms[i])) for i in range(n)]
```

Before: 920.1.

## Verify subset rows on device and reuse coarse pair masks in subset binning

```diff
diff --git a/include/lara2dgs.h b/include/lara2dgs.h
--- a/include/lara2dgs.h
+++ b/include/lara2dgs.h
@@ -8,7 +8,7 @@
 extern "C" {
 #endif
 
-#define LARA2DGS_ABI_VERSION 10
+#define LARA2DGS_ABI_VERSION 11
 
 #define LARA2DGS_OK 0
 #define LARA2DGS_E_INVALID (-1)
@@ -102,6 +102,16 @@
                                   int64_t state_stride, void *scratch, int64_t scratch_stride,
                                   const lara2dgs_subset *subset, void *stream);
 
+typedef struct lara2dgs_subset_rows {
+    const float *means3D, *opacities, *scales, *rotations, *transmat_precomp;
+} lara2dgs_subset_rows;
+int lara2dgs_forward_views_subset_checked(int32_t n_views, const lara2dgs_view *views, const float *means3D,
+                                          const float *shs, const float *colors_precomp, const float *opacities,
+                                          const float *scales, const float *rotations, const float *transmat_precomp,
+                                          float *out_color, float *out_allmap, int32_t *out_radii, void *state,
+                                          int64_t state_stride, void *scratch, int64_t scratch_stride,
+                                          const lara2dgs_subset *subset, const lara2dgs_subset_rows *coarse_rows, void *stream);
+
 typedef struct lara2dgs_grad_layout {
     int64_t means3D, means2D, shs, colors, opacities, scales, rotations, transmat, total;
 } lara2dgs_grad_layout;
diff --git a/lara_amd/csrc/abi.hip b/lara_amd/csrc/abi.hip
--- a/lara_amd/csrc/abi.hip
+++ b/lara_amd/csrc/abi.hip
@@ -261,8 +261,11 @@
                            const float *scales, const float *rotations, const float *transmat_precomp,
                            float *out_color, float *out_allmap, int32_t *out_radii, void *state,
                            int64_t state_stride, void *scratch, int64_t scratch_stride, void *stream,
-                           const lara2dgs_subset *subset) {
+                           const lara2dgs_subset *subset, const lara2dgs_subset_rows *coarse_rows = nullptr) {
     if (n_views <= 0 || !views || !state || !scratch) return LARA2DGS_E_INVALID;
+    if (coarse_rows && (!subset || !coarse_rows->means3D || !coarse_rows->opacities ||
+                        (transmat_precomp ? !coarse_rows->transmat_precomp : !coarse_rows->scales || !coarse_rows->rotations)))
+        return LARA2DGS_E_INVALID;
     if (subset) {
         if (!subset->coarse_state || !subset->inv || subset->coarse_P < views[0].P || subset->coarse_capacity < 0 ||
             subset->coarse_capacity > 0xffffffffll || subset->coarse_state_stride % 256) return LARA2DGS_E_INVALID;
@@ -296,6 +299,8 @@
             zero_strided(sc[0].tile_count, scratch_stride, SL.sub_start - SL.tile_count, n_views, caller);
     }
     int rc = LARA2DGS_OK;
+    const bool masks = subset && coarse_rows && v0.P > 0 && !v0.forward_only && !subset->coarse_forward_only;
+    const lara2dgs_subset_rows fine_rows{means3D, opacities, scales, rotations, transmat_precomp};
     for (int i0 = 0; i0 < n_views && rc == LARA2DGS_OK; i0 += L2D_MAX_VIEWS) {
         ViewBatch vb{};
         vb.n = n_views - i0 < L2D_MAX_VIEWS ? n_views - i0 : L2D_MAX_VIEWS;
@@ -308,11 +313,12 @@
             ViewDev cv = vd[i0];
             cv.P = subset->coarse_P; cv.cap = (unsigned)subset->coarse_capacity; cv.fwd_only = subset->coarse_forward_only != 0;
             const StateView cst = carve_state(cv, (char *)const_cast<void *>(subset->coarse_state) + (int64_t)i0 * subset->coarse_state_stride);
-            rc = launch_binning_subset(vd[i0], st[i0], sc[i0], caller, vb, cst, subset->coarse_state_stride, subset->inv);
+            rc = launch_binning_subset(vd[i0], st[i0], sc[i0], caller, vb, cst, subset->coarse_state_stride, subset->inv,
+                                       subset->coarse_P, coarse_rows ? &fine_rows : nullptr, coarse_rows, masks);
         }
         if (rc == LARA2DGS_OK)
             rc = launch_composite_fwd(vd[i0], st[i0], sc[i0], out_color + (int64_t)i0 * 3 * HW, out_allmap + (int64_t)i0 * 7 * HW,
-                                      caller, vb);
+                                      caller, vb, masks);
     }
     return rc;
 }
@@ -335,6 +341,17 @@
     if (!subset) return LARA2DGS_E_INVALID;
     return forward_views_impl(n_views, views, means3D, shs, colors_precomp, opacities, scales, rotations, transmat_precomp, out_color,
                               out_allmap, out_radii, state, state_stride, scratch, scratch_stride, stream, subset);
+}
+
+int lara2dgs_forward_views_subset_checked(int32_t n_views, const lara2dgs_view *views, const float *means3D,
+                                          const float *shs, const float *colors_precomp, const float *opacities,
+                                          const float *scales, const float *rotations, const float *transmat_precomp,
+                                          float *out_color, float *out_allmap, int32_t *out_radii, void *state,
+                                          int64_t state_stride, void *scratch, int64_t scratch_stride,
+                                          const lara2dgs_subset *subset, const lara2dgs_subset_rows *coarse_rows, void *stream) {
+    if (!subset || !coarse_rows) return LARA2DGS_E_INVALID;
+    return forward_views_impl(n_views, views, means3D, shs, colors_precomp, opacities, scales, rotations, transmat_precomp, out_color,
+                              out_allmap, out_radii, state, state_stride, scratch, scratch_stride, stream, subset, coarse_rows);
 }
 
 static int backward_views_impl(int32_t n_views, const lara2dgs_view *views, const float *means3D, const float *shs,
diff --git a/lara_amd/csrc/binning.hip b/lara_amd/csrc/binning.hip
--- a/lara_amd/csrc/binning.hip
+++ b/lara_amd/csrc/binning.hip
@@ -31,7 +31,8 @@
                  uint32_t *__restrict__ tile_order, uint32_t *__restrict__ block_tot,
                  uint32_t *__restrict__ seg_base, uint32_t *__restrict__ seg_cnt,
                  uint32_t *__restrict__ bwd_order, uint2 *__restrict__ bwd_items,
-                 uint32_t *__restrict__ sort_parts, uint2 *__restrict__ sort_items, const long long sst, const long long qst) {
+                 uint32_t *__restrict__ sort_parts, uint2 *__restrict__ sort_items, const long long sst, const long long qst,
+                 const uint32_t *__restrict__ subset_check = nullptr) {
     tile_count = l2d_view_ptr(tile_count, qst); sub_start = l2d_view_ptr(sub_start, qst); block_tot = l2d_view_ptr(block_tot, qst);
     sort_parts = l2d_view_ptr(sort_parts, qst); sort_items = l2d_view_ptr(sort_items, qst);
     ranges = l2d_view_ptr(ranges, sst); header = l2d_view_ptr(header, sst); tile_order = l2d_view_ptr(tile_order, sst);
@@ -127,14 +128,16 @@
         uint32_t m = 0;
         for (int w = 0; w < 16; w++) m = wave_sums[w] > m ? wave_sums[w] : m;
         const uint32_t total = carry_s;
+        const uint32_t flags = (total > v.cap ? 1u : 0u) |
+                               (subset_check && (subset_check[0] != 0u || subset_check[1] != (uint32_t)v.P) ? 2u : 0u);
         header[0] = total;
-        header[1] = total > v.cap ? 1u : 0u;
+        header[1] = flags;
         header[2] = m;
         s_max = m;
         if (v.counts_out) {
             uint32_t *c = v.counts_out + 4 * blockIdx.z;
             __hip_atomic_store(&c[0], total, __ATOMIC_RELAXED, __HIP_MEMORY_SCOPE_SYSTEM);
-            __hip_atomic_store(&c[1], total > v.cap ? 1u : 0u, __ATOMIC_RELAXED, __HIP_MEMORY_SCOPE_SYSTEM);
+            __hip_atomic_store(&c[1], flags, __ATOMIC_RELAXED, __HIP_MEMORY_SCOPE_SYSTEM);
             __hip_atomic_store(&c[2], m, __ATOMIC_RELAXED, __HIP_MEMORY_SCOPE_SYSTEM);
             __hip_atomic_store(&c[3], 1u, __ATOMIC_RELEASE, __HIP_MEMORY_SCOPE_SYSTEM);
         }
@@ -624,29 +627,70 @@
     }
 }
 
+struct SubsetRows {
+    const uint32_t *means3D, *opacities, *scales, *rotations, *transmat;
+};
 __global__ void __launch_bounds__(256)
-subset_compact_kernel(ViewDev v, const uint32_t *__restrict__ header, const uint2 *__restrict__ ranges, uint32_t *__restrict__ point_list,
-                      const uint32_t *__restrict__ pair_base, uint32_t *__restrict__ pair_pos, const long long sst,
+subset_verify_kernel(const int coarse_P, const int P, const int32_t *__restrict__ inv, const SubsetRows f, const SubsetRows c,
+                     uint32_t *__restrict__ check) {
+    const int r = blockIdx.x * 256 + threadIdx.x;
+    bool bad = false, kept = false;
+    if (r < coarse_P) {
+        const int j = inv[r];
+        kept = j >= 0;
+        if (j >= P) bad = true;
+        else if (j >= 0) {
+            for (int k = 0; k < 3; k++) bad |= f.means3D[3 * (size_t)j + k] != c.means3D[3 * (size_t)r + k];
+            bad |= f.opacities[j] != c.opacities[r];
+            if (f.transmat) {
+                for (int k = 0; k < 9; k++) bad |= f.transmat[9 * (size_t)j + k] != c.transmat[9 * (size_t)r + k];
+            } else {
+                for (int k = 0; k < 2; k++) bad |= f.scales[2 * (size_t)j + k] != c.scales[2 * (size_t)r + k];
+                for (int k = 0; k < 4; k++) bad |= f.rotations[4 * (size_t)j + k] != c.rotations[4 * (size_t)r + k];
+            }
+        }
+    }
+    const unsigned long long any_bad = __ballot(bad), n_kept = __ballot(kept);
+    if ((threadIdx.x & 63) == 0) {
+        if (any_bad) __hip_atomic_fetch_or(&check[0], 1u, __ATOMIC_RELAXED, __HIP_MEMORY_SCOPE_AGENT);
+        if (n_kept) __hip_atomic_fetch_add(&check[1], (uint32_t)__builtin_popcountll(n_kept), __ATOMIC_RELAXED, __HIP_MEMORY_SCOPE_AGENT);
+    }
+}
+
+__global__ void __launch_bounds__(256)
+subset_compact_kernel(ViewDev v, uint32_t *__restrict__ header, const uint2 *__restrict__ ranges, uint32_t *__restrict__ point_list,
+                      const uint32_t *__restrict__ pair_base, uint32_t *__restrict__ pair_pos, uint2 *__restrict__ pair_mask,
+                      uint32_t *__restrict__ tile_maxc, const long long sst,
                       const uint2 *__restrict__ c_ranges, const uint32_t *__restrict__ c_point_list, const uint32_t *__restrict__ c_pair_base,
-                      const uint32_t *__restrict__ c_pair_pos, const long long csst, const int32_t *__restrict__ inv) {
+                      const uint32_t *__restrict__ c_pair_pos, const uint2 *__restrict__ c_pair_mask,
+                      const uint32_t *__restrict__ c_tile_maxc, const long long csst, const int32_t *__restrict__ inv, const int masks) {
     header = l2d_view_ptr(header, sst); ranges = l2d_view_ptr(ranges, sst); point_list = l2d_view_ptr(point_list, sst);
-    pair_base = l2d_view_ptr(pair_base, sst); pair_pos = l2d_view_ptr(pair_pos, sst);
+    pair_base = l2d_view_ptr(pair_base, sst); pair_pos = l2d_view_ptr(pair_pos, sst); pair_mask = l2d_view_ptr(pair_mask, sst);
+    tile_maxc = l2d_view_ptr(tile_maxc, sst);
     c_ranges = l2d_view_ptr(c_ranges, csst); c_point_list = l2d_view_ptr(c_point_list, csst);
     c_pair_base = l2d_view_ptr(c_pair_base, csst); c_pair_pos = l2d_view_ptr(c_pair_pos, csst);
+    c_pair_mask = l2d_view_ptr(c_pair_mask, csst); c_tile_maxc = l2d_view_ptr(c_tile_maxc, csst);
     __shared__ uint32_t wtot[2][4];
-    if (header[1]) return;
     const int tile = blockIdx.x, tid = threadIdx.x, lane = tid & 63, wave = tid >> 6;
-    const uint2 cr = c_ranges[tile];
+    if (__hip_atomic_load(&header[1], __ATOMIC_RELAXED, __HIP_MEMORY_SCOPE_AGENT) == 0u) {
+    const uint2 cr = c_ranges[tile], rg = ranges[tile];
     const uint32_t n = cr.y - cr.x;
-    uint32_t out = ranges[tile].x;
+    uint32_t n_ok = 0;
+    if (masks) {
+        const uint32_t rounds = (c_tile_maxc[tile] + 511u) / 512u;
+        n_ok = min(n, (rounds ? rounds : 1u) * 512u);
+    }
+    uint32_t out = rg.x, n_masked = 0;
     uint32_t id_n = tid < n ? c_point_list[cr.x + tid] : 0u;
     int fid_n = tid < n ? inv[id_n] : -1;
     int buf = 0;
     for (uint32_t base = 0; base < n; base += 256, buf ^= 1) {
         const uint32_t i = base + tid, id = id_n;
-        const int fid = fid_n;
+        const int fid = fid_n < v.P ? fid_n : -1;
         uint32_t off = 0, pbf = 0;
+        uint2 cm = make_uint2(0u, 0u);
         if (fid >= 0 && !v.fwd_only) { off = c_pair_pos[cr.x + i] - c_pair_base[id]; pbf = pair_base[fid]; }
+        if (fid >= 0 && i < n_ok) cm = c_pair_mask[cr.x + i];
         if (base + 256 < n) {
             id_n = i + 256 < n ? c_point_list[cr.x + i + 256] : 0u;
             fid_n = i + 256 < n ? inv[id_n] : -1;
@@ -659,24 +703,45 @@
         for (int w = 0; w < 4; w++) { before += w < wave ? wtot[buf][w] : 0u; all += wtot[buf][w]; }
         if (fid >= 0) {
             const uint32_t pos = out + before + (uint32_t)__builtin_popcountll(kept & ((1ull << lane) - 1ull));
-            point_list[pos] = (uint32_t)fid;
-            if (!v.fwd_only) pair_pos[pos] = pbf + off;
+            if (pos < rg.y) {
+                point_list[pos] = (uint32_t)fid;
+                if (!v.fwd_only) pair_pos[pos] = pbf + off;
+                if (i < n_ok) pair_mask[pos] = cm;
+            }
         }
         out += all;
+        if (base < n_ok) n_masked = out - rg.x;
+    }
+    if (tid == 0) {
+        if (masks) tile_maxc[tile] = min(n_masked, rg.y - rg.x);
+        if (out != rg.y) __hip_atomic_fetch_or(&header[1], 2u, __ATOMIC_RELAXED, __HIP_MEMORY_SCOPE_AGENT);
+    }
     }
 }
 
 }
 
 int launch_binning_subset(const ViewDev &v, StateView st, ScratchView sc, hipStream_t s, const ViewBatch &vb, StateView cst,
-                          long long coarse_stride, const int32_t *inv) {
+                          long long coarse_stride, const int32_t *inv, int coarse_P, const lara2dgs_subset_rows *fine_rows,
+                          const lara2dgs_subset_rows *coarse_rows, bool masks) {
     const unsigned nz = (unsigned)vb.n;
     const long long sst = vb.state_stride, qst = vb.scratch_stride;
+    const uint32_t *check = coarse_rows && v.P > 0 ? sc.tile_fill : nullptr;
+    if (check) {
+        L2D_PROF("subset_verify", s);
+        auto rows = [](const lara2dgs_subset_rows *r) {
+            return SubsetRows{(const uint32_t *)r->means3D, (const uint32_t *)r->opacities, (const uint32_t *)r->scales,
+                              (const uint32_t *)r->rotations, (const uint32_t *)r->transmat_precomp};
+        };
+        hipLaunchKernelGGL(subset_verify_kernel, dim3((coarse_P + 255) / 256), dim3(256), 0, s, coarse_P, v.P, inv, rows(fine_rows),
+                           rows(coarse_rows), sc.tile_fill);
+        L2D_CHECK_LAUNCH();
+    }
     {
         L2D_PROF("tile_scan", s);
         hipLaunchKernelGGL(tile_scan_kernel, dim3(v.P > 0 ? 2 : 1, 1, nz), dim3(1024), 0, s, v, sc.tile_count, sc.sub_start,
                            st.ranges, st.header, st.tile_order, sc.block_tot, st.seg_base, st.seg_cnt, st.bwd_order,
-                           st.bwd_items, sc.sort_parts, sc.sort_items, sst, qst);
+                           st.bwd_items, sc.sort_parts, sc.sort_items, sst, qst, check);
     }
     L2D_CHECK_LAUNCH();
     if (v.P == 0) return LARA2DGS_OK;
@@ -687,7 +752,8 @@
     {
         L2D_PROF("subset_compact", s);
         hipLaunchKernelGGL(subset_compact_kernel, dim3(v.tiles, 1, nz), dim3(256), 0, s, v, st.header, st.ranges, st.point_list,
-                           st.pair_base, st.pair_pos, sst, cst.ranges, cst.point_list, cst.pair_base, cst.pair_pos, coarse_stride, inv);
+                           st.pair_base, st.pair_pos, st.pair_mask, st.tile_maxc, sst, cst.ranges, cst.point_list, cst.pair_base,
+                           cst.pair_pos, cst.pair_mask, cst.tile_maxc, coarse_stride, inv, masks ? 1 : 0);
     }
     L2D_CHECK_LAUNCH();
     return LARA2DGS_OK;
diff --git a/lara_amd/csrc/common.h b/lara_amd/csrc/common.h
--- a/lara_amd/csrc/common.h
+++ b/lara_amd/csrc/common.h
@@ -134,9 +134,10 @@
                                 const ScratchView *sc, int32_t *const *radii, hipStream_t s);
 int launch_binning(const ViewDev &v, StateView st, ScratchView sc, hipStream_t s, const ViewBatch &vb);
 int launch_binning_subset(const ViewDev &v, StateView st, ScratchView sc, hipStream_t s, const ViewBatch &vb, StateView cst,
-                          long long coarse_stride, const int32_t *inv);
+                          long long coarse_stride, const int32_t *inv, int coarse_P, const lara2dgs_subset_rows *fine_rows,
+                          const lara2dgs_subset_rows *coarse_rows, bool masks);
 int launch_composite_fwd(const ViewDev &v, StateView st, ScratchView sc, float *out_color, float *out_allmap,
-                         hipStream_t s, const ViewBatch &vb);
+                         hipStream_t s, const ViewBatch &vb, bool masks_staged = false);
 int launch_bwd_order(const ViewDev &v, StateView st, ScratchView sc, hipStream_t s, const ViewBatch &vb, void *zero_base, int64_t zero_bytes);
 int launch_composite_bwd(const ViewDev &v, StateView st, ScratchView sc, const float *dL_dcolor,
                          const float *dL_dallmap, hipStream_t s, const ViewBatch &vb);
diff --git a/lara_amd/csrc/composite.hip b/lara_amd/csrc/composite.hip
--- a/lara_amd/csrc/composite.hip
+++ b/lara_amd/csrc/composite.hip
@@ -117,7 +117,7 @@
     }
     rec[0 * CHUNK + e] = r0; rec[1 * CHUNK + e] = r1; rec[2 * CHUNK + e] = r2;
     rec[3 * CHUNK + e] = r3; rec[4 * CHUNK + e] = r4; rec[5 * CHUNK + e] = r5;
-    ids[e] = valid ? id : 0u;
+    if (ids) ids[e] = valid ? id : 0u;
 }
 
 struct Hit {
@@ -201,7 +201,7 @@
 
 };
 
-template <bool KEEP>
+template <bool KEEP, bool REUSE = false>
 __global__ void __launch_bounds__(256)
 composite_fwd_kernel(ViewDev v, const uint32_t *__restrict__ header, const uint2 *__restrict__ ranges,
                      const uint32_t *__restrict__ point_list, const float4 *__restrict__ geom,
@@ -256,6 +256,7 @@
 
     const uint2 range = ranges[tile];
     const int total = (int)(range.y - range.x);
+    const int n_masked = REUSE ? (int)tile_maxc[tile] : 0;
     const int lo = 0, hi = total;
     FwdPixel px;
     px.done = !inside;
@@ -273,14 +274,16 @@
     constexpr int SPT = CHUNK / 256;
     uint32_t id1[SPT], id2[SPT];
     float4 cb1[SPT];
+    uint2 mk1[SPT];
 #pragma unroll
     for (int q = 0; q < SPT; q++) {
         const int o = lo + q * 256 + tid;
         id1[q] = o < hi ? point_list[range.x + o] : 0u;
         id2[q] = CHUNK + o < hi ? point_list[range.x + CHUNK + o] : 0u;
-    }
-#pragma unroll
-    for (int q = 0; q < SPT; q++) cb1[q] = lo + q * 256 + tid < hi ? cullbox[id1[q]] : make_float4(0.f, 0.f, 0.f, 0.f);
+        mk1[q] = REUSE && o < n_masked ? pair_mask[range.x + o] : make_uint2(0u, 0u);
+    }
+#pragma unroll
+    for (int q = 0; q < SPT; q++) cb1[q] = lo + q * 256 + tid < hi && lo + q * 256 + tid >= n_masked ? cullbox[id1[q]] : make_float4(0.f, 0.f, 0.f, 0.f);
     if (threadIdx.x < 3) *(uint32_t *)&rec[5 * CHUNK + threadIdx.x].w = 0u;
     __syncthreads();
     for (int base = lo; base < hi; base += CHUNK) {
@@ -307,11 +310,16 @@
             const int o = q * 256 + tid;
             const uint32_t id0 = id1[q];
             const float4 cb0 = cb1[q];
+            const uint2 mk0 = mk1[q];
             id1[q] = id2[q];
             id2[q] = base + 2 * CHUNK + o < hi ? point_list[range.x + base + 2 * CHUNK + o] : 0u;
-            cb1[q] = base + CHUNK + o < hi ? cullbox[id1[q]] : make_float4(0.f, 0.f, 0.f, 0.f);
-            stage_entry<CHUNK>(geom, id0, cb0, base + o < hi, X0, Y0, rec, nullptr, o,
-                               KEEP && base + o < hi ? pair_mask + range.x + base + o : nullptr);
+            cb1[q] = base + CHUNK + o < hi && base + CHUNK + o >= n_masked ? cullbox[id1[q]] : make_float4(0.f, 0.f, 0.f, 0.f);
+            if (REUSE) mk1[q] = base + CHUNK + o < n_masked ? pair_mask[range.x + base + CHUNK + o] : make_uint2(0u, 0u);
+            if (REUSE && base + o < n_masked)
+                stage_entry_masked<CHUNK>(geom, id0, mk0, true, X0, Y0, rec, nullptr, o);
+            else
+                stage_entry<CHUNK>(geom, id0, cb0, base + o < hi, X0, Y0, rec, nullptr, o,
+                                   KEEP && base + o < hi ? pair_mask + range.x + base + o : nullptr);
         }
         __syncthreads();
         if (__ballot(!px.done) == 0ull) continue;
@@ -1058,12 +1066,13 @@
 }
 
 int launch_composite_fwd(const ViewDev &v, StateView st, ScratchView sc, float *out_color, float *out_allmap,
-                         hipStream_t s, const ViewBatch &vb) {
+                         hipStream_t s, const ViewBatch &vb, bool masks_staged) {
     (void)sc;
+    if (masks_staged && v.fwd_only) return LARA2DGS_E_INVALID;
     const unsigned nz = (unsigned)vb.n;
     {
         L2D_PROF(v.fwd_only ? "composite_fwd_only" : "composite_fwd", s);
-        auto kern = v.fwd_only ? composite_fwd_kernel<false> : composite_fwd_kernel<true>;
+        auto kern = v.fwd_only ? composite_fwd_kernel<false> : (masks_staged ? composite_fwd_kernel<true, true> : composite_fwd_kernel<true>);
         hipLaunchKernelGGL(kern, dim3(v.tiles, 1, nz), dim3(256), 0, s, v, st.header, st.ranges, st.point_list,
                            (const float4 *)st.geom, st.tile_order, (const float4 *)st.cullbox, st.final_T, st.n_contrib, st.seg_base,
                            st.seg_cnt, st.ckpt, st.pair_mask, st.tile_maxc, st.seg_cost, out_color, out_allmap, vb);
diff --git a/lara_amd/rasterizer.py b/lara_amd/rasterizer.py
--- a/lara_amd/rasterizer.py
+++ b/lara_amd/rasterizer.py
@@ -13,7 +13,7 @@
 
 _HERE = os.path.dirname(os.path.abspath(__file__))
 LIB_PATH = os.environ.get("LARA2DGS_LIB") or os.path.join(_HERE, "liblara2dgs.so")
-ABI_VERSION = 10
+ABI_VERSION = 11
 
 
 class _View(ctypes.Structure):
@@ -32,6 +32,10 @@
 class _Subset(ctypes.Structure):
     _fields_ = [("coarse_state", ctypes.c_void_p), ("coarse_state_stride", ctypes.c_int64), ("coarse_capacity", ctypes.c_int64),
                 ("coarse_P", ctypes.c_int32), ("coarse_forward_only", ctypes.c_int32), ("inv", ctypes.c_void_p)]
+
+
+class _SubsetRows(ctypes.Structure):
+    _fields_ = [(n, ctypes.c_void_p) for n in ("means3D", "opacities", "scales", "rotations", "transmat_precomp")]
 
 
 class GradLayout(ctypes.Structure):
@@ -77,6 +81,9 @@
     lib.lara2dgs_forward_views.argtypes = [i32, ctypes.POINTER(_View)] + [vp] * 11 + [i64, vp, i64, vp]
     lib.lara2dgs_forward_views_subset.restype = ctypes.c_int
     lib.lara2dgs_forward_views_subset.argtypes = [i32, ctypes.POINTER(_View)] + [vp] * 11 + [i64, vp, i64, ctypes.POINTER(_Subset), vp]
+    lib.lara2dgs_forward_views_subset_checked.restype = ctypes.c_int
+    lib.lara2dgs_forward_views_subset_checked.argtypes = [i32, ctypes.POINTER(_View)] + [vp] * 11 + [i64, vp, i64, ctypes.POINTER(_Subset),
+                                                          ctypes.POINTER(_SubsetRows), vp]
     lib.lara2dgs_backward_views.restype = ctypes.c_int
     lib.lara2dgs_backward_views.argtypes = [i32, ctypes.POINTER(_View)] + [vp] * 10 + [i64, vp, i64, vp, vp]
     lib.lara2dgs_get_grad_layout.restype = ctypes.c_int
@@ -196,6 +203,19 @@
     return c
 
 
+class _SubsetMismatch(Exception):
+    """A `subset_of` call whose surfels turned out not to be rows of the earlier call (the library's flag, bit 1)."""
+
+
+_OVERFLOW, _MISMATCH = 1, 2
+
+
+def _record_event():
+    done = torch.cuda.Event()
+    done.record()
+    return done
+
+
 def _wait_counts(c: _Counts, n: int, done: torch.cuda.Event, headers):
     global _counts_fallbacks
     ready = c.np[:n, 3]
@@ -206,9 +226,10 @@
             if done.query() and not ready.all():
                 _counts_fallbacks += 1
                 h = headers().cpu().numpy().view("uint32").reshape(n, -1)
-                return int(h[:, 0].max()), bool(h[:, 1].any())
+                return int(h[:, 0].max()), int(h[:, 1].max() | (2 if (h[:, 1] & 2).any() else 0))
             time.sleep(0)
-    return int(c.np[:n, 0].max()), bool(c.np[:n, 1].any())
+    flags = c.np[:n, 1]
+    return int(c.np[:n, 0].max()), (_OVERFLOW if (flags & _OVERFLOW).any() else 0) | (_MISMATCH if (flags & _MISMATCH).any() else 0)
 
 
 def _run_forward(bucket, n, enqueue, debug=False):
@@ -218,9 +239,11 @@
     while True:
         c.np[:n, 3] = 0
         state, headers, extra = enqueue(cap, c.ptr)
-        done = torch.cuda.Event()
-        done.record()
-        D, overflow = _wait_counts(c, n, done, headers)
+        done = _record_event()
+        D, flags = _wait_counts(c, n, done, headers)
+        if flags & _MISMATCH:
+            raise _SubsetMismatch()
+        overflow = bool(flags & _OVERFLOW)
         note_pair_count(bucket, D)
         if bool(c.np[:n, 3].all()):
             _longest[bucket] = max(_longest.get(bucket, 0), int(c.np[:n, 2].max()))
@@ -397,12 +420,12 @@
         radii = torch.empty(lead + (P,), dtype=torch.int32, device=device)
         sub = None
         if subset is not None and P > 0:
-            c_state, c_sb, c_cap, c_P, idx = subset
+            c_state, c_sb, c_cap, c_P, idx, c_rows = subset
             if idx.numel() != P or idx.device != device or c_P < P:
                 raise RuntimeError("lara_amd: `subset_of` needs one index per surfel of this call, on its device")
             inv = torch.full((c_P,), -1, dtype=torch.int32, device=device)
             inv[idx] = torch.arange(P, dtype=torch.int32, device=device)
-            sub = _Subset(c_state.data_ptr(), c_sb, c_cap, c_P, 0, inv.data_ptr())
+            sub = (_Subset(c_state.data_ptr(), c_sb, c_cap, c_P, 0, inv.data_ptr()), _SubsetRows(*(_ptr(t) for t in c_rows)))
 
         def enqueue(cap, counts_ptr):
             for i in range(n):
@@ -415,16 +438,45 @@
             scratch = _get_scratch(device, n * qb)
             args = (n, views, _ptr(means3D_c), _ptr(sh_c), _ptr(col_c), _ptr(opa_c), _ptr(sc_c), _ptr(rot_c), _ptr(tm_c),
                     color.data_ptr(), allmap.data_ptr(), radii.data_ptr(), state.data_ptr(), sb, scratch.data_ptr(), qb)
-            if sub is None:
+            if use[0] is None:
                 rc = lib.lara2dgs_forward_views(*args, torch.cuda.current_stream(device).cuda_stream)
             else:
-                rc = lib.lara2dgs_forward_views_subset(*args, ctypes.byref(sub), torch.cuda.current_stream(device).cuda_stream)
+                rc = lib.lara2dgs_forward_views_subset_checked(*args, ctypes.byref(use[0][0]), ctypes.byref(use[0][1]),
+                                                               torch.cuda.current_stream(device).cuda_stream)
             _check(rc, "lara2dgs_forward_views")
             return state, (lambda: state.view(n, sb)[:, :64].contiguous().view(torch.int32)), (sb, qb)
 
-        state, cap, (sb, qb), D = _run_forward(_bucket(device, P, H, W), n, enqueue, any(rs.debug for rs in settings))
+        use = [sub]
+
+        def run(with_subset):
+            use[0] = sub if with_subset else None
+            return _run_forward(_bucket(device, P, H, W), n, enqueue, any(rs.debug for rs in settings))
+
+        state, cap, (sb, qb), D = _with_subset_fallback(run, sub is not None)
     return dict(color=color, radii=radii, allmap=allmap, state=state, cap=cap, strides=(sb, qb), D=D, M=M, keep=keep,
-                inputs=(means3D_c, sh_c, col_c, sc_c, rot_c, tm_c))
+                inputs=(means3D_c, sh_c, col_c, sc_c, rot_c, tm_c), opacities=opa_c)
+
+
+def _with_subset_fallback(run, has_subset):
+    if not has_subset:
+        return run(False)
+    try:
+        return run(True)
+    except _SubsetMismatch:
+        warnings.warn("lara_amd: `subset_of` names a call whose surfels, cameras or settings are not this call's (rows that "
+                      "differ, indices that repeat or do not ascend); the call was repeated without it", RuntimeWarning,
+                      stacklevel=2)
+        return run(False)
+
+
+def _check_subset_settings(earlier, earlier_bits, settings, bits):
+    if earlier_bits != bits:
+        raise RuntimeError("lara_amd: `subset_of` names a call with another `prefiltered` / cull-transparent setting")
+    for a, b in zip(earlier, settings):
+        if (a.image_height, a.image_width, a.tanfovx, a.tanfovy, float(a.scale_modifier)) != \
+                (b.image_height, b.image_width, b.tanfovx, b.tanfovy, float(b.scale_modifier)) or \
+                a.viewmatrix.data_ptr() != b.viewmatrix.data_ptr() or a.projmatrix.data_ptr() != b.projmatrix.data_ptr():
+            raise RuntimeError("lara_amd: `subset_of` names a call with other cameras")
 
 
 class _RasterizeViews(torch.autograd.Function):
@@ -439,6 +491,7 @@
         color, radii, allmap, M, keep = r["color"], r["radii"], r["allmap"], r["M"], r["keep"]
         means3D_c, sh_c, col_c, sc_c, rot_c, tm_c = r["inputs"]
         ctx.state, ctx.cap, ctx.strides, ctx.D = r["state"], r["cap"], r["strides"], r["D"]
+        ctx.opacities = r["opacities"]
         ctx.settings = settings
         ctx.M = M
         ctx.prefiltered_bits = int(bool(rs0.prefiltered)) | (2 if _cull_transparent else 0)
@@ -520,13 +573,14 @@
     if subset_of is not None:
         coarse_color, idx = subset_of
         node = getattr(coarse_color, "grad_fn", None)
-        if node is not None and hasattr(node, "strides") and hasattr(node, "state") and len(node.settings) == len(settings):
-            for a, b in zip(node.settings, settings):
-                if (a.image_height, a.image_width, a.tanfovx, a.tanfovy, float(a.scale_modifier)) != \
-                        (b.image_height, b.image_width, b.tanfovx, b.tanfovy, float(b.scale_modifier)) or \
-                        a.viewmatrix.data_ptr() != b.viewmatrix.data_ptr() or a.projmatrix.data_ptr() != b.projmatrix.data_ptr():
-                    raise RuntimeError("lara_amd: `subset_of` names a call with other cameras")
-            subset = (node.state, node.strides[0], node.cap, node.saved_tensors[0].shape[0], idx.contiguous())
+        if node is not None and hasattr(node, "strides") and hasattr(node, "state") and len(node.settings) == len(settings) and \
+                node.flags[2:] == (scales is not None, cov3D_precomp is not None):
+            _check_subset_settings(node.settings, node.prefiltered_bits, settings,
+                                   int(bool(settings[0].prefiltered)) | (2 if _cull_transparent else 0))
+            c_means, _, _, c_sc, c_rot, c_tm = node.saved_tensors[:6]
+            rows = (c_means, node.opacities, c_sc if node.flags[2] else None, c_rot if node.flags[2] else None,
+                    c_tm if node.flags[3] else None)
+            subset = (node.state, node.strides[0], node.cap, c_means.shape[0], idx.contiguous(), rows)
     return _RasterizeViews.apply(means3D, means2D, shs, colors_precomp, opacities, scales, rotations, cov3D_precomp,
                                  tuple(settings), subset)
 
```

After: 932.8, median of 5. +1.4%, better.
